# OFA-Sys/OFASys

Measured on AMD Instinct MI355X. Metric: multimodal tokens/sec (enc+dec train step), higher is better.
Workload: dtype bf16

## Files before the change

include/ofasys_amd.h:

```cpp
#ifndef OFASYS_AMD_H
#define OFASYS_AMD_H

#include <stdint.h>

#ifdef __cplusplus
extern "C" {
#endif

typedef enum { OFA_F32 = 0, OFA_BF16 = 1, OFA_F16 = 2 } ofa_dtype;

enum {
  OFA_OK = 0,
  OFA_ERR_INVALID = 1,
  OFA_ERR_UNSUPPORTED = 2,
  OFA_ERR_LAUNCH = 3
};

enum {
  OFA_GEMM_BIAS_COL = 1,
  OFA_GEMM_BIAS_ROW = 2,
  OFA_GEMM_ACCUM = 4,
  OFA_GEMM_FORCE_SIMPLE = 8,
  OFA_GEMM_OUT_F32 = 16,
  OFA_GEMM_A_KPAD_ZERO = 32,
  OFA_GEMM_NO_LDS_DMA = 64,
  OFA_GEMM_DEFER_REDUCE = 128
};

int ofa_version(void);
const char* ofa_last_error(void);

int ofa_layernorm_fwd(const void* x, const void* gamma, const void* beta, void* y, float* mean, float* rstd,
                      int64_t rows, int cols, float eps, int dtype, void* stream);
int ofa_layernorm_bwd_ws_rows(void);
int ofa_layernorm_bwd(const void* dy, const void* x, const void* gamma, const float* mean, const float* rstd,
                      const void* dres, void* dx, void* dgamma, void* dbeta, float* ws, int64_t rows, int cols,
                      int accumulate, int dtype, void* stream);
int ofa_gelu_layernorm_fwd(const void* h, const void* gamma, const void* beta, void* y, float* mean, float* rstd,
                           int64_t rows, int cols, float eps, int dtype, void* stream);
int ofa_gelu_layernorm_bwd(const void* dy, const void* h, const void* gamma, const float* mean, const float* rstd,
                           void* dh, void* dgamma, void* dbeta, void* dbias, float* ws, int64_t rows, int cols,
                           int accumulate, int dtype, void* stream);

int64_t ofa_join_keep_bytes(int64_t rows, int cols, int dtype);
int ofa_join_fwd(const void* x, const void* residual, const void* gamma_a, const void* beta_a, const void* gamma_b,
                 const void* beta_b, void* y, void* z, float* stats, uint8_t* keep_bits, int64_t rows, int cols, float eps, float p,
                 uint64_t seed, uint64_t offset, const int64_t* offset_base, int dtype, void* stream);
int ofa_join_bwd_slots(int64_t rows, int cols, int dtype);
int ofa_join_bwd(const void* dy, const void* dz, const void* x, const void* y, const void* gamma_a, const void* gamma_b,
                 const float* stats, const uint8_t* keep_bits, void* dres, void* dx, float* ws, int64_t rows, int cols, float p,
                 uint64_t seed, uint64_t offset, const int64_t* offset_base, int want_dx_colsum, int dtype, void* stream);

int ofa_gemm(const void* A, const void* B, void* C, const void* bias, int M, int N, int K, int transA, int transB,
             int64_t lda, int64_t ldb, int64_t ldc, int batch, int64_t strideA, int64_t strideB, int64_t strideC,
             int batch_inner, int64_t strideA2, int64_t strideB2, int64_t strideC2,
             float alpha, int flags, int dtype, void* ws, int64_t ws_bytes, void* stream);

int ofa_gemm_colstat(const void* A, const void* B, void* C, const void* bias, int M, int N, int K, int transA, int transB,
                     int64_t lda, int64_t ldb, int64_t ldc, float alpha, int flags, int dtype, void* ws, int64_t ws_bytes,
                     double* partial, int max_groups, int* groups, void* stream);

typedef struct ofa_gemm_group_item {
  const void* a;
  const void* b;
  float* slabs;
  int64_t lda, ldb;
  int32_t m, n, k;
  int32_t splits;
  void* out;
  int64_t ldo;
  float out_alpha;
} ofa_gemm_group_item;
int ofa_gemm_group_plan(ofa_gemm_group_item* items, int n, int dtype);
int ofa_gemm_group_tn(const ofa_gemm_group_item* items, int n, int dtype, void* stream);

int ofa_scaled_softmax_fwd(const void* x, void* y, float scale, int b, int np, int sq, int sk, int dtype, void* stream);
int ofa_scaled_softmax_bwd(const void* dy, const void* y, void* dx, float scale, int b, int np, int sq, int sk,
                           int dtype, void* stream);
int ofa_scaled_masked_softmax_fwd(const void* x, const uint8_t* mask, void* y, float scale, int b, int np, int sq,
                                  int sk, int mask_b, int dtype, void* stream);
int ofa_scaled_masked_softmax_bwd(const void* dy, const void* y, void* dx, float scale, int b, int np, int sq, int sk,
                                  int dtype, void* stream);
int ofa_scaled_upper_triang_masked_softmax_fwd(const void* x, void* y, float scale, int attn_batches, int sq,
                                               int dtype, void* stream);
int ofa_scaled_upper_triang_masked_softmax_bwd(const void* dy, const void* y, void* dx, float scale, int attn_batches,
                                               int sq, int dtype, void* stream);
int ofa_get_batch_per_block(int sq, int sk, int b, int np);

int ofa_attn_softmax_fwd(const void* x, const void* bias, const uint8_t* kpm, void* p, float scale, int BA, int heads,
                         int T, int S, int causal, int dtype, void* stream);

typedef struct ofa_attn_call {
  const void *q, *k, *v, *dout;
  void* out;
  float *lse, *delta;
  void *dq, *dk, *dv;
  const void *bias, *bias_swz_row, *bias_swz_col;
  void* dbias;
  float* ws;
  const uint8_t* kpm;
  const void* c_attn;
  const int32_t* seg;
  float *cs_q, *cs_k, *cs_v, *cs_c;
  int64_t ldq, ldk, ldo, ws_bytes, cs_ldq, cs_ldk;
  int32_t B, heads, T, S, Tpad, Tb, Sb;
  int32_t causal, rows_q, rows_k;
  int32_t dtype, c_attn_dtype, dbias_dtype;
  float scale;
} ofa_attn_call;
int ofa_attn_fwd(const ofa_attn_call* c, void* stream);
int ofa_attn_bwd(const ofa_attn_call* c, void* stream);
int ofa_attn_bwd_prep(const void* dout, const void* out, float* delta, int B, int heads, int T, int Tpad, int64_t ldo,
                      int dtype, void* stream);
int ofa_attn_cs_slots(int B, int rows);
int ofa_attn_sbias_chunks(int B, int heads, int Tb, int Sb);
int ofa_c_attn_grad(const float* delta, const void* c_attn, void* dc, int B, int heads, int T, int64_t ld, int accumulate,
                    int c_attn_dtype, void* stream);
int ofa_attn_decode(const void* q, const void* k, const void* v, const void* bias, const uint8_t* kpm, const void* c_attn,
                    int c_attn_dtype, void* out, void* probs, int B, int heads, int head_dim, int S, int64_t ldk,
                    int64_t k_batch_stride, int64_t kpm_ld, float scale, int dtype, void* stream);
int ofa_mean_heads(const void* p, void* out, int B, int heads, int64_t n, int dtype, void* stream);
int ofa_transpose_heads(const void* x, void* xt, int B, int T, int C, int Tpad, int64_t ld, int dtype, void* stream);

int ofa_gather_rows(const void* src, const int64_t* index, void* out, int64_t n, int D, int64_t src_rows, int dtype,
                    void* stream);
int ofa_gather_rows_parts(const void* const* srcs, const int* lens, int nparts, const int64_t* index, void* out, int64_t n, int D,
                          int64_t batch, int dtype, void* stream);
int ofa_scatter_rows_part(const void* src, const int64_t* inverse, void* out, int64_t batch, int nk, int Ttot, int start, int D,
                          int64_t src_rows, int dtype, void* stream);
int ofa_embedding_fwd(const void* weight, const int64_t* ids, void* out, int64_t n, int D, int64_t V, uint8_t* is_pad, int64_t pad_id,
                      int dtype, void* stream);
int ofa_segment_rowsum(const void* dout, const int32_t* order, const int32_t* seg_off, const int32_t* seg_row, void* dweight, int nseg,
                       int D, int accumulate, int dtype, void* stream);
int ofa_embedding_bwd_slices(int64_t V, int D);
int ofa_embedding_bwd(const void* dout, const int64_t* ids, void* dweight, int64_t n, int D, int64_t V,
                      int64_t padding_idx, uint8_t* present_ws, float* slice_ws, int dtype, void* stream);
#define OFA_EMBEDDING_IDS_MAX 15360
int ofa_embedding_bwd_ids_ok(int64_t n, int D, int64_t V, int dtype);
int ofa_embedding_bwd_ids(const void* dout, const int64_t* ids, void* dweight, int64_t n, int D, int64_t V, int64_t padding_idx,
                          int slices, int dtype, void* stream);
int ofa_embedding_range_bwd(const void* dout, void* dweight, int batch, int64_t T, int D, int64_t V, int64_t r0, int dtype, void* stream);
enum { OFA_EDGE_POS_RANGE = 0, OFA_EDGE_TOKEN_BWD = 1, OFA_EDGE_COLSUM_FOLD = 2, OFA_EDGE_IM2COL = 3 };
int ofa_step_edges_old(int item);

int ofa_gelu_fwd(const void* x, void* y, int64_t n, int dtype, void* stream);
int ofa_gelu_bwd(const void* dy, const void* x, void* dx, int64_t n, int dtype, void* stream);
int ofa_dropout_add_fwd(const void* x, const void* residual, void* y, int64_t n, float p, uint64_t seed,
                        uint64_t offset, const int64_t* offset_base, int dtype, void* stream);
int ofa_dropout_bwd(const void* dy, void* dx, int64_t n, float p, uint64_t seed, uint64_t offset,
                    const int64_t* offset_base, int dtype, void* stream);
int ofa_add_rowvec_mask(const void* a, const void* b, const void* vec, const uint8_t* rowmask, void* y, int64_t rows,
                        int cols, int64_t b_period, int dtype, void* stream);
int ofa_batch_sum(const void* x, void* out, int batch, int64_t n, int accumulate, int dtype, void* stream);

int ofa_colsum_ws_floats(int cols);
int ofa_colsum(const void* x, void* out, float* ws, int64_t rows, int cols, int64_t ld, float alpha, int accumulate,
               int dtype, int out_dtype, void* stream);

int ofa_add_n(const void* const* inputs, int n, void* out, int64_t numel, int dtype, void* stream);
int ofa_mul(const void* a, const void* b, void* y, int64_t rows, int cols, int b_rowvec, int dtype, void* stream);
int ofa_scale_row_groups(const void* x, const float* scale, void* y, int64_t rows, int cols, int64_t group, int dtype,
                         void* stream);
int ofa_reduce_sum_f32(const float* x, float* out, int64_t n, void* stream);
int ofa_head_sum_f32(const float* x, float* out, int B, int heads, int T, int ld, void* stream);

typedef struct ofa_bias_slots {
  const void* values[8];
  const void* values2[8];
  int32_t start[8];
  int32_t n[8];
  int32_t inner[8];
  int32_t count;
} ofa_bias_slots;
int64_t ofa_bias_swz_elems(int heads, int Tb, int Sb);
int ofa_bias_build(const void* abs_bias, const ofa_bias_slots* slots, void* out, void* swz_row, void* swz_col, int heads, int Tb,
                   int Sb, int dtype, void* stream);
int ofa_bias_outer_grad(const void* dbias, void* d_frames, void* d_patches, int heads, int T, int start, int F, int P, int dtype,
                        void* stream);
int ofa_bias_block_add(void* bias, const void* values, int B, int A, int T, int start, int n, int dtype, void* stream);
int ofa_bias_block_grad(const void* dbias, void* dvalues, int B, int A, int T, int start, int n, int dtype, void* stream);
int ofa_bias_block_add_batch(void* bias, const void* values, int B, int A, int T, int start, int n, int dtype, void* stream);
int ofa_bias_block_slice(const void* dbias, void* dvalues, int B, int A, int T, int start, int n, int dtype, void* stream);

int ofa_im2col_patch(const void* img, void* col, int B, int C, int H, int W, int p, int Kpad, int lead, int dtype, void* stream);

int ofa_cross_entropy_fwd(const void* logits, const int64_t* target, float* lse, float* row_loss, int64_t rows,
                          int64_t V, int64_t ld, int64_t ignore_index, int dtype, void* stream);
int ofa_cross_entropy_fwd_grad_ok(int64_t V, int64_t ld, int dtype);
int ofa_cross_entropy_fwd_grad(const void* logits, const int64_t* target, const float* grad_scale, float* lse, float* row_loss,
                               void* dlogits, int64_t rows, int64_t V, int64_t ld, int64_t ignore_index, int dtype, void* stream);
int ofa_cross_entropy_bwd(const void* logits, const int64_t* target, const float* lse, const float* grad_scale,
                          void* dlogits, int64_t rows, int64_t V, int64_t ld, int64_t ignore_index, int dtype,
                          void* stream);

int ofa_ls_cross_entropy_fwd(const void* logits, const int64_t* target, float* lse, float* row_loss, float* row_nll,
                             float* row_cnt, int64_t rows, int64_t V, int64_t ld, int64_t ignore_index, float eps,
                             int64_t cstart, int64_t cend, const uint8_t* cmask, int dtype, void* stream);
int ofa_ls_cross_entropy_bwd(const void* logits, const int64_t* target, const float* lse, const float* row_cnt,
                             const float* row_w, const float* grad_scale, void* dlogits, int64_t rows, int64_t V, int64_t ld,
                             int64_t ignore_index, float eps, int64_t cstart, int64_t cend, const uint8_t* cmask, int dtype,
                             void* stream);
int ofa_scst_loss_fwd_grad(const void* logits, const int64_t* target, const float* reward, const int32_t* row_seq,
                           int64_t rows_per_seq, const float* grad_scale, float* lse, float* row_loss, void* dlogits, int64_t rows,
                           int64_t nseq, int64_t V, int64_t ld, int64_t ignore_index, int64_t cstart, int64_t cend, int dtype,
                           void* stream);
int ofa_probs_fwd(const void* logits, float* out, int64_t rows, int64_t V, int64_t ld, int log_probs, int dtype,
                  void* stream);
int ofa_probs_bwd(const float* dy, const float* y, void* dlogits, int64_t rows, int64_t V, int64_t ld, int log_probs,
                  int dtype, void* stream);

int ofa_sumsq_ws_floats(void);
int ofa_sumsq(const void* x, float* out , float* ws ,
              int64_t n, int dtype, void* stream);
int ofa_step_schedule(const float* gsq, const double* sample_size, double* step, const double* lr, float* sched,
                      float* gnorm, float clip_norm, double beta1, double beta2, void* stream);
int ofa_step_stats_add(double* stats, const float* loss, const int64_t* target, int64_t n, int64_t pad, void* stream);
int ofa_step_schedule_scaled(const float* gsq, const double* sample_size, double* step, const double* lr, float* sched,
                             float* gnorm, double* loss_scaler, float clip_norm, double beta1, double beta2, double scale_factor,
                             double scale_window, double tolerance, double threshold, double min_loss_scale, void* stream);
int ofa_adam_step(float* master, float* exp_avg, float* exp_avg_sq, const void* grad, void* model_param,
                  const float* coef, int64_t n, float lr, float beta1, float beta2, float eps, float weight_decay,
                  int step, int dtype, void* stream);
int ofa_ema_step(void* state, const void* p, void* shadow, int64_t n, const double* step, const float* sched, double decay,
                 int64_t start_update, int64_t update_freq, int dtype, int state_dtype, int max_blocks, void* stream);
int ofa_ema_segments_step(void* state, const void* segments, void* shadow, int64_t n, int64_t state_numel, int64_t max_len,
                          const double* step, const float* sched, double decay, int64_t start_update, int64_t update_freq,
                          int dtype, int state_dtype, int max_blocks, void* stream);

int ofa_conv_out_size(int in, int k, int stride, int pad);
int ofa_im2col(const void* x, void* col, int B, int H, int W, int C, int KH, int KW, int stride, int pad, int Kpad,
               int x_nchw, int dtype, void* stream);
int ofa_col2im(const void* dcol, void* dx, int B, int H, int W, int C, int KH, int KW, int stride, int pad, int Kpad,
               int dtype, void* stream);
int ofa_batchnorm_ws_floats(int C);
int ofa_batchnorm_fwd(const void* x, const void* gamma, const void* beta, const void* residual, void* y, float* mean,
                      float* rstd, float* running_mean, float* running_var, float* ws, int64_t rows, int C, float eps,
                      float momentum, int use_running, int relu, int dtype, void* stream);
int ofa_batchnorm_bwd(const void* dy, const void* y, const void* x, const void* gamma, const float* mean, const float* rstd,
                      void* dx, void* dres, void* dgamma, void* dbeta, float* ws, int64_t rows, int C, int batch_stats,
                      int relu, int accumulate, const void* beta, int dtype, void* stream);
int ofa_batchnorm_fwd_stats(const void* x, double* sums, float* ws, int64_t rows, int C, int dtype, void* stream);
int ofa_batchnorm_fwd_apply(const void* x, const void* gamma, const void* beta, const void* residual, void* y, float* mean,
                            float* rstd, float* running_mean, float* running_var, const double* sums, int groups, int64_t rows,
                            int C, float eps, float momentum, int relu, int dtype, void* stream);
int ofa_batchnorm_bwd_stats(const void* dy, const void* y, const void* x, const void* gamma, const float* mean, const float* rstd,
                            float* sums, void* dgamma, void* dbeta, float* ws, int64_t rows, int C, int relu, int accumulate,
                            const void* beta, int dtype, void* stream);
int ofa_batchnorm_bwd_dx(const void* dy, const void* y, const void* x, const void* gamma, const float* mean, const float* rstd,
                         const float* sums, void* dx, void* dres, int64_t rows, const double* total_rows, int C, int relu,
                         const void* beta, int dtype, void* stream);
int ofa_maxpool_fwd(const void* x, void* y, uint8_t* arg, int B, int H, int W, int C, int K, int stride, int pad, int dtype,
                    void* stream);
int ofa_maxpool_bwd(const void* dy, const uint8_t* arg, void* dx, int B, int H, int W, int C, int K, int stride, int pad,
                    int dtype, void* stream);
int ofa_relu(const void* x, const void* gate, void* y, int64_t n, int dtype, void* stream);

typedef struct ofa_fold_job {
  const float* part;
  void* out;
  int64_t cols;
  int64_t stride;
  int32_t nslots;
  int32_t accumulate;
  float alpha;
  int32_t out_dtype;
} ofa_fold_job;
#define OFA_FOLD_LANES16 4
int ofa_fold_batched(const ofa_fold_job* jobs, int njobs, void* stream);
typedef struct ofa_copy_job {
  const void* src;
  void* dst;
  int64_t bytes;
} ofa_copy_job;
int ofa_copy_batched(const ofa_copy_job* jobs, int njobs, void* stream);
#define OFA_DEFER_FOLD 2
int ofa_layernorm_bwd_slots(int64_t rows, int cols, int dtype, int gelu);
int ofa_colsum_slots(int64_t rows);
int ofa_gemm_splits(int M, int N, int K, int transA, int transB, int batch, int flags, int dtype, int64_t ws_bytes);
enum {
  OFA_GEMM_PLAN_KERNEL = 0,
  OFA_GEMM_PLAN_SIMPLE_WHY,
  OFA_GEMM_PLAN_WAVES_M,
  OFA_GEMM_PLAN_WAVES_N,
  OFA_GEMM_PLAN_WAVE_TM,
  OFA_GEMM_PLAN_WAVE_TN,
  OFA_GEMM_PLAN_TILE_M,
  OFA_GEMM_PLAN_TILE_N,
  OFA_GEMM_PLAN_SPLITS,
  OFA_GEMM_PLAN_KSPLIT,
  OFA_GEMM_PLAN_K,
  OFA_GEMM_PLAN_MIXED_TALL,
  OFA_GEMM_PLAN_MIXED_SHORT,
  OFA_GEMM_PLAN_COLSTAT_ROWS,
  OFA_GEMM_PLAN_REDUCE,
  OFA_GEMM_PLAN_LEN
};
enum {
  OFA_GEMM_KERNEL_SIMPLE = 0,
  OFA_GEMM_KERNEL_REG = 1,
  OFA_GEMM_KERNEL_LDS_DMA = 2,
  OFA_GEMM_KERNEL_RING = 3,
  OFA_GEMM_KERNEL_BIG = 4,
  OFA_GEMM_KERNEL_PP = 5,
  OFA_GEMM_KERNEL_MIXED = 6
};
int ofa_gemm_plan(int M, int N, int K, int transA, int transB, int batch, int flags, int dtype, int64_t ws_bytes, int* plan);

typedef struct ofa_gen_policy {
  float temperature;
  int32_t cstart, cend;
  int32_t step, min_len, max_len;
  int32_t pad, unk, eos;
  float unk_penalty;
  int32_t ngram;
  const int64_t* tokens;
  int64_t tok_ld;
  const int32_t* done;
} ofa_gen_policy;

typedef struct ofa_gen_state {
  int64_t* tokens;
  int64_t tok_ld;
  int32_t tok_cap;
  float* scores;
  int64_t score_ld;
  int32_t *ignore, *done, *nfin;
  int64_t* reorder;
// ... 55 lines not shown
```

ofasys_amd/csrc/elementwise.hip:

```cpp
#include "common.h"

namespace ofa {

template <typename T> __device__ __forceinline__ float round_to(float v);
template <> __device__ __forceinline__ float round_to<float>(float v) { return v; }
template <> __device__ __forceinline__ float round_to<bf16_t>(float v) { return bf2f(f2bf(v)); }
template <> __device__ __forceinline__ float round_to<f16_t>(float v) { return (float)(f16_t)v; }

template <typename T, bool BWD>
__global__ __launch_bounds__(256) void gelu_kernel(const T* __restrict__ dy, const T* __restrict__ x, T* __restrict__ y,
                                                   int64_t nvec, int64_t n) {
  constexpr int N = Vec<T>::N;
  for (int64_t v = (int64_t)blockIdx.x * 256 + threadIdx.x; v < nvec; v += (int64_t)gridDim.x * 256) {
    float a[N], g[N], o[N];
    load_vec<T>(x + v * N, a);
    if (BWD) load_vec<T>(dy + v * N, g);
#pragma unroll
    for (int j = 0; j < N; ++j) o[j] = BWD ? g[j] * gelu_grad_f(a[j]) : gelu_f(a[j]);
    store_vec<T>(y + v * N, o);
  }
  if (blockIdx.x == 0) {
    for (int64_t e = nvec * N + threadIdx.x; e < n; e += 256) {
      const float a = ld1<T>(x + e);
      st1<T>(y + e, BWD ? ld1<T>(dy + e) * gelu_grad_f(a) : gelu_f(a));
// ... 728 lines not shown
  return check_launch("segment_rowsum");
}

extern "C" int ofa_embedding_bwd(const void* dout, const int64_t* ids, void* dweight, int64_t n, int D, int64_t V,
                                 int64_t padding_idx, uint8_t* present_ws, float* slice_ws, int dtype, void* stream) {
  OFA_DT_CHECK("embedding_bwd");
  OFA_REQUIRE(n >= 0 && D > 0 && V > 0 && dout && ids && dweight, OFA_ERR_INVALID, "embedding_bwd: bad argument");
  const int vecn = dt_vecn(dtype);
  OFA_REQUIRE(D <= 2048, OFA_ERR_UNSUPPORTED, "embedding_bwd: D=%d exceeds 2048", D);
  const bool vec_ok = D % vecn == 0 && D <= 64 * vecn * 4 && (((uintptr_t)dout | (uintptr_t)dweight) & 15) == 0;
  if (n == 0) return 0;
  hipStream_t st = (hipStream_t)stream;
  if (present_ws) {
    (void)hipMemsetAsync(present_ws, 0, (size_t)V, st);
    hipLaunchKernelGGL(embedding_mark_kernel, dim3(grid_for(n)), dim3(256), 0, st, ids, present_ws, n, V);
  }
  const int S = slice_ws ? ofa_embedding_bwd_slices(V, D) : 1;
  const int nv = cdiv(D, 64 * vecn);
  dim3 grid((unsigned)((V + 3) / 4), S), block(256);
#define EMB_LAUNCH(T, NV)                                                                                               \
  hipLaunchKernelGGL((embedding_bwd_kernel<T, NV>), grid, block, 0, st, (const T*)dout, ids, (T*)dweight, slice_ws, n, D, V, \
                     padding_idx, (const uint8_t*)present_ws, S)
  if (!vec_ok)
    dispatch_dtype(dtype, [&](auto tag) {
      using T = typename decltype(tag)::type;
      hipLaunchKernelGGL((embedding_bwd_scalar_kernel<T>), grid, block, 0, st, (const T*)dout, ids, (T*)dweight, slice_ws, n, D, V,
                         padding_idx, (const uint8_t*)present_ws, S);
    });
  else
    dispatch_dtype(dtype, [&](auto tag) {
      using T = typename decltype(tag)::type;
      if (nv <= 1) EMB_LAUNCH(T, 1);
      else if (nv <= 2) EMB_LAUNCH(T, 2);
      else EMB_LAUNCH(T, 4);
    });
#undef EMB_LAUNCH
  int rc = check_launch("embedding_bwd");
  if (rc || S == 1) return rc;
  dispatch_dtype(dtype, [&](auto tag) {
    using T = typename decltype(tag)::type;
    hipLaunchKernelGGL((embedding_fold_kernel<T>), dim3((unsigned)V), dim3(256), 0, st, slice_ws, (T*)dweight, D, V, padding_idx,
                       (const uint8_t*)present_ws, S);
  });
  return check_launch("embedding_fold");
}

extern "C" int ofa_step_edges_old(int item) {
#ifdef OFA_DEBUG_SWITCHES
  if (const char* e = getenv("OFA_STEP_EDGES_OLD")) return (atoi(e) >> item) & 1;
#endif
  return 0;
}

extern "C" int ofa_embedding_bwd_ids_ok(int64_t n, int D, int64_t V, int dtype) {
  const int vecn = dt_vecn(dtype);
  return OFA_DT_OK(dtype) && n >= 0 && n <= OFA_EMBEDDING_IDS_MAX && V > 0 && V < ((int64_t)1 << 31) && D > 0 && D % vecn == 0 &&
         D <= 64 * vecn * 4;
}

extern "C" int ofa_embedding_bwd_ids(const void* dout, const int64_t* ids, void* dweight, int64_t n, int D, int64_t V,
                                     int64_t padding_idx, int slices, int dtype, void* stream) {
  OFA_DT_CHECK("embedding_bwd_ids");
  OFA_REQUIRE(n >= 0 && D > 0 && V > 0 && slices >= 1 && dout && ids && dweight, OFA_ERR_INVALID, "embedding_bwd_ids: bad argument");
  OFA_REQUIRE(ofa_embedding_bwd_ids_ok(n, D, V, dtype), OFA_ERR_UNSUPPORTED,
              "embedding_bwd_ids: n=%lld ids (at most %d), D=%d (whole 16-byte vectors, at most 256 of them): use ofa_embedding_bwd",
              (long long)n, OFA_EMBEDDING_IDS_MAX, D);
  OFA_REQUIRE((((uintptr_t)dout | (uintptr_t)dweight) & 15) == 0, OFA_ERR_UNSUPPORTED, "embedding_bwd_ids: buffers not 16-byte aligned");
  if (n == 0) return 0;
  hipStream_t st = (hipStream_t)stream;
  const int vecn = dt_vecn(dtype);
  const int nv = cdiv(D, 64 * vecn);
  const int per = (int)(((n + slices - 1) / slices + 63) / 64 * 64);
  const int blocks = cdiv(n, EMB_IDS_WAVES) < 1024 ? cdiv(n, EMB_IDS_WAVES) : 1024;
  const size_t lds = (size_t)((n + 63) / 64 * 64 + EMB_IDS_WAVES * 64) * sizeof(int);
#define EMB_LAUNCH(T, NV, SL)                                                                                       \
  hipLaunchKernelGGL((embedding_bwd_ids_kernel<T, NV, SL>), dim3(blocks), dim3(EMB_IDS_WAVES * 64), lds, st, (const T*)dout, ids, \
                     (T*)dweight, (int)n, D, V, padding_idx, per)
  if (slices > 1)
    dispatch_dtype(dtype, [&](auto tag) {
      using T = typename decltype(tag)::type;
      if (nv <= 1) EMB_LAUNCH(T, 1, true);
      else if (nv <= 2) EMB_LAUNCH(T, 2, true);
      else EMB_LAUNCH(T, 4, true);
    });
  else
    dispatch_dtype(dtype, [&](auto tag) {
      using T = typename decltype(tag)::type;
      if (nv <= 1) EMB_LAUNCH(T, 1, false);
      else if (nv <= 2) EMB_LAUNCH(T, 2, false);
      else EMB_LAUNCH(T, 4, false);
    });
#undef EMB_LAUNCH
  return check_launch("embedding_bwd_ids");
}

extern "C" int ofa_embedding_range_bwd(const void* dout, void* dweight, int batch, int64_t T, int D, int64_t V, int64_t r0, int dtype,
                                       void* stream) {
  OFA_DT_CHECK("embedding_range_bwd");
  OFA_REQUIRE(dout && dweight && batch >= 1 && T >= 0 && D > 0 && V > 0 && r0 >= 0 && r0 + T <= V, OFA_ERR_INVALID,
              "embedding_range_bwd: bad argument (rows %lld .. %lld of %lld)", (long long)r0, (long long)(r0 + T), (long long)V);
  OFA_REQUIRE(D % dt_vecn(dtype) == 0 && (((uintptr_t)dout | (uintptr_t)dweight) & 15) == 0, OFA_ERR_UNSUPPORTED,
              "embedding_range_bwd: D=%d / buffers not whole 16-byte vectors: use ofa_embedding_bwd", D);
  if (T == 0) return 0;
  hipStream_t st = (hipStream_t)stream;
  const int64_t n = T * D;
  dispatch_dtype(dtype, [&](auto tag) {
// ... 235 lines not shown
```

ofasys_amd/csrc/fold.hip:

```cpp
#include "common.h"

namespace ofa {

constexpr int FOLD_MAX_JOBS = 56;

struct FoldJobs {
  const float* part[FOLD_MAX_JOBS];
  void* out[FOLD_MAX_JOBS];
  int64_t cols[FOLD_MAX_JOBS];
  int64_t stride[FOLD_MAX_JOBS];
  float alpha[FOLD_MAX_JOBS];
  int nslots[FOLD_MAX_JOBS];
  unsigned block0[FOLD_MAX_JOBS + 1];
  unsigned char flags[FOLD_MAX_JOBS];
  int njobs;
};

__device__ __forceinline__ void fold_store(const FoldJobs& J, int j, int64_t c, int64_t cols, const float (&t)[4]) {
  const float alpha = J.alpha[j];
  const bool acc = J.flags[j] & 1, f32 = J.flags[j] & 2, f16 = J.flags[j] & 8;
  if (c + 4 <= cols && (cols & 3) == 0) {
    if (f32) {
      float4* o = reinterpret_cast<float4*>((float*)J.out[j] + c);
      float4 v = make_float4(t[0] * alpha, t[1] * alpha, t[2] * alpha, t[3] * alpha);
// ... 126 lines not shown
      for (; s + 24 < ns; s += 32) {
        const float4 v0 = *reinterpret_cast<const float4*>(r + (int64_t)s * stride);
        const float4 v1 = *reinterpret_cast<const float4*>(r + (int64_t)(s + 8) * stride);
        const float4 v2 = *reinterpret_cast<const float4*>(r + (int64_t)(s + 16) * stride);
        const float4 v3 = *reinterpret_cast<const float4*>(r + (int64_t)(s + 24) * stride);
        a.x = (((a.x + v0.x) + v1.x) + v2.x) + v3.x;
        a.y = (((a.y + v0.y) + v1.y) + v2.y) + v3.y;
        a.z = (((a.z + v0.z) + v1.z) + v2.z) + v3.z;
        a.w = (((a.w + v0.w) + v1.w) + v2.w) + v3.w;
      }
      for (; s < ns; s += 8) {
        const float4 v = *reinterpret_cast<const float4*>(r + (int64_t)s * stride);
        a.x += v.x; a.y += v.y; a.z += v.z; a.w += v.w;
      }
    } else {
      for (int s = sl; s < ns; s += 8) {
        const float* r = p + (int64_t)s * stride + c;
        a.x += r[0];
        if (c + 1 < cols) a.y += r[1];
        if (c + 2 < cols) a.z += r[2];
        if (c + 3 < cols) a.w += r[3];
      }
    }
  }
  red[sl][q] = a;
  if (l16) red[sl + 8][q] = a2;
  __syncthreads();
  if (sl == 0 && c < cols) {
    float t[4] = {0.f, 0.f, 0.f, 0.f};
#pragma unroll
    for (int r = 0; r < 8; ++r) {
      t[0] += red[r][q].x; t[1] += red[r][q].y; t[2] += red[r][q].z; t[3] += red[r][q].w;
    }
    if (l16) {
#pragma unroll
      for (int r = 8; r < 16; ++r) {
        t[0] += red[r][q].x; t[1] += red[r][q].y; t[2] += red[r][q].z; t[3] += red[r][q].w;
      }
    }
    fold_store(J, j, c, cols, t);
  }
}

constexpr int COPY_MAX_JOBS = 96;
constexpr int COPY_CHUNK = 32768;
struct CopyJobs {
  const unsigned char* src[COPY_MAX_JOBS];
  unsigned char* dst[COPY_MAX_JOBS];
  int64_t bytes[COPY_MAX_JOBS];
  unsigned block0[COPY_MAX_JOBS + 1];
  int njobs;
};

__global__ __launch_bounds__(256) void copy_batched_kernel(CopyJobs J) {
  int lo = 0, hi = J.njobs - 1;
  while (lo < hi) {
    const int mid = (lo + hi + 1) >> 1;
    if (J.block0[mid] <= blockIdx.x) lo = mid; else hi = mid - 1;
  }
  const int64_t off = (int64_t)(blockIdx.x - J.block0[lo]) * COPY_CHUNK;
  const int64_t left = J.bytes[lo] - off;
  const int n = (int)(left < COPY_CHUNK ? left : COPY_CHUNK);
  const unsigned char* s = J.src[lo] + off;
  unsigned char* d = J.dst[lo] + off;
  if ((((uintptr_t)s | (uintptr_t)d) & 15) == 0) {
    const int nv = n >> 4;
    for (int i = threadIdx.x; i < nv; i += 256) reinterpret_cast<uint4*>(d)[i] = reinterpret_cast<const uint4*>(s)[i];
    for (int i = (nv << 4) + threadIdx.x; i < n; i += 256) d[i] = s[i];
  } else {
    for (int i = threadIdx.x; i < n; i += 256) d[i] = s[i];
  }
}

}
using namespace ofa;

extern "C" int ofa_copy_batched(const ofa_copy_job* jobs, int njobs, void* stream) {
  OFA_REQUIRE(njobs >= 0 && (njobs == 0 || jobs), OFA_ERR_INVALID, "copy_batched: bad argument");
  hipStream_t st = (hipStream_t)stream;
  for (int base = 0; base < njobs; base += COPY_MAX_JOBS) {
    CopyJobs J;
    const int n = njobs - base < COPY_MAX_JOBS ? njobs - base : COPY_MAX_JOBS;
    int m = 0;
    unsigned blocks = 0;
    for (int i = 0; i < n; ++i) {
      const ofa_copy_job& b = jobs[base + i];
      OFA_REQUIRE(b.bytes >= 0 && (b.bytes == 0 || (b.src && b.dst)), OFA_ERR_INVALID, "copy_batched: bad job %d", base + i);
      if (b.bytes == 0) continue;
      J.src[m] = (const unsigned char*)b.src; J.dst[m] = (unsigned char*)b.dst; J.bytes[m] = b.bytes;
      J.block0[m] = blocks;
      blocks += (unsigned)((b.bytes + COPY_CHUNK - 1) / COPY_CHUNK);
      ++m;
    }
    if (m == 0) continue;
    J.block0[m] = blocks;
    J.njobs = m;
    hipLaunchKernelGGL(copy_batched_kernel, dim3(blocks), dim3(256), 0, st, J);
    int rc = check_launch("copy_batched");
    if (rc) return rc;
  }
  return 0;
}

extern "C" int ofa_fold_batched(const ofa_fold_job* jobs, int njobs, void* stream) {
  OFA_REQUIRE(njobs >= 0 && (njobs == 0 || jobs), OFA_ERR_INVALID, "fold_batched: bad argument");
  hipStream_t st = (hipStream_t)stream;
  for (int base = 0; base < njobs; base += FOLD_MAX_JOBS) {
    FoldJobs J;
    const int n = njobs - base < FOLD_MAX_JOBS ? njobs - base : FOLD_MAX_JOBS;
    J.njobs = n;
    unsigned blocks = 0;
    for (int i = 0; i < n; ++i) {
      const ofa_fold_job& b = jobs[base + i];
      OFA_REQUIRE(b.part && b.out && b.cols > 0 && b.nslots > 0 && b.stride >= b.cols, OFA_ERR_INVALID, "fold_batched: bad job %d", base + i);
      OFA_REQUIRE(OFA_DT_OK(b.out_dtype), OFA_ERR_INVALID, "fold_batched: bad out dtype %d", b.out_dtype);
      J.part[i] = b.part; J.out[i] = b.out; J.cols[i] = b.cols; J.stride[i] = b.stride; J.alpha[i] = b.alpha;
      J.nslots[i] = b.nslots;
      const bool wide = b.nslots <= 16;
      J.flags[i] = (unsigned char)(((b.accumulate & ~OFA_FOLD_LANES16) ? 1 : 0) | (b.out_dtype == OFA_F32 ? 2 : 0) | (wide ? 4 : 0) |
                                   (b.out_dtype == OFA_F16 ? 8 : 0) | ((b.accumulate & OFA_FOLD_LANES16) ? 16 : 0));
      J.block0[i] = blocks;
      blocks += (unsigned)(wide ? (b.cols + 1023) / 1024 : (b.cols + 127) / 128);
    }
    J.block0[n] = blocks;
    if (blocks == 0) continue;
    hipLaunchKernelGGL(fold_batched_kernel, dim3(blocks), dim3(256), 0, st, J);
    int rc = check_launch("fold_batched");
    if (rc) return rc;
  }
  return 0;
}
```

ofasys_amd/csrc/gemm_core.h:

```cpp
#pragma once
#include <stdlib.h>

#include <type_traits>

#include "gemm.h"

namespace ofa {

typedef __attribute__((ext_vector_type(8))) short bf16x8;
template <bool F16> __device__ __forceinline__ float lo16(uint32_t w) {
  if constexpr (F16) return (float)__builtin_bit_cast(f16x2_t, w)[0];
  else return __uint_as_float(w << 16);
}
template <bool F16> __device__ __forceinline__ float hi16(uint32_t w) {
  if constexpr (F16) return (float)__builtin_bit_cast(f16x2_t, w)[1];
  else return __uint_as_float(w & 0xffff0000u);
}
template <bool F16> __device__ __forceinline__ uint32_t enc2(float lo, float hi) {
  if constexpr (F16) return pack_f16x2(lo, hi);
  else return pack_bf16x2(lo, hi);
}
template <bool F16> __device__ __forceinline__ float dec1(uint16_t u) {
  if constexpr (F16) return (float)__builtin_bit_cast(f16_t, u);
  else return bf2f(u);
// ... 405 lines not shown
      for (int j = 0; j < 8; ++j) {
        ps[j] = (double)cs[j];
        ps[g.N + j] = (double)cq[j];
      }
    }
  }
}

template <int I, int N, typename F> __device__ __forceinline__ void static_for(F&& f) {
  if constexpr (I < N) {
    f(std::integral_constant<int, I>{});
    static_for<I + 1, N>(f);
  }
}

template <int R, bool KMAJ> struct BigAddr {
  uint32_t a[4];
  __device__ __forceinline__ void init(uint32_t op0, int rbase, int lane) {
    if (KMAJ) {
      const int row = rbase + (lane & 31), hi = lane >> 5;
#pragma unroll
      for (int kk = 0; kk < 4; ++kk) a[kk] = op0 + (uint32_t)(row * 64 + swz<R, true>(row, kk * 2 + hi) * 8) * 2u;
    } else {
      const int g = lane >> 4, q = lane & 15;
      const int k = (g >> 1) * 8 + (q >> 2);
#pragma unroll
      for (int ti = 0; ti < 4; ++ti) {
        const int col = rbase + ti * 32 + (g & 1) * 16 + 4 * (q & 3);
        a[ti] = op0 + (uint32_t)(k * R + swz<R, false>(k, col >> 3) * 8 + (col & 7)) * 2u;
      }
    }
  }
};

template <int R, bool KMAJ, int KK, int TI, int BUFOFF>
__device__ __forceinline__ void big_frag(u64x2& d, const BigAddr<R, KMAJ>& fa) {
  if constexpr (KMAJ) {
    asm volatile("ds_read_b128 %0, %1 offset:%2" : "=v"(d) : "v"(fa.a[KK]), "i"(BUFOFF + TI * 32 * 128));
  } else {
    unsigned long long lo, hi;
    asm volatile("ds_read_b64_tr_b16 %0, %1 offset:%2" : "=v"(lo) : "v"(fa.a[TI]), "i"(BUFOFF + KK * 16 * R * 2));
    asm volatile("ds_read_b64_tr_b16 %0, %1 offset:%2" : "=v"(hi) : "v"(fa.a[TI]), "i"(BUFOFF + KK * 16 * R * 2 + 4 * R * 2));
    d[0] = lo;
    d[1] = hi;
  }
}

__host__ __device__ constexpr int big_read_after(int t, int nr) { return t < nr ? t : -1; }

constexpr int GROUP_MAX = 16;
struct GroupItem {
  const void* A; const void* B; float* ws;
  void* out; int64_t ldo; float alpha;
  int64_t lda, ldb;
  int M, N, K, krows, ksplit, splits, tiles_m, tiles_n, first;
};
struct GroupArgs { GroupItem it[GROUP_MAX]; int n, total; };

__device__ __forceinline__ const GroupItem* group_enter(const GroupArgs& ga, GemmArgs& g, int& t, int& ks) {
  const int id = xcd_remap((int)blockIdx.x, ga.total);
  int p = 0;
  for (int q = 1; q < ga.n; ++q)
    if (id >= ga.it[q].first) p = q;
  const GroupItem& it = ga.it[p];
  g.A = it.A; g.B = it.B; g.C = it.out; g.bias = nullptr;
  g.M = it.M; g.N = it.N; g.K = it.K; g.transA = 1; g.transB = 0;
  g.lda = it.lda; g.ldb = it.ldb; g.ldc = it.ldo; g.strideA = g.strideB = g.strideC = 0;
  g.alpha = it.out ? it.alpha : 1.f; g.flags = it.out ? OFA_GEMM_ACCUM : 0; g.batch_inner = 1; g.strideA2 = g.strideB2 = g.strideC2 = 0; g.a_krows = g.b_krows = it.krows;
  g.colstat = nullptr; g.colstat_rows = 0;
  const int ntiles = it.tiles_m * it.tiles_n, local = id - it.first;
  ks = local / ntiles;
  t = local - ks * ntiles;
  return &it;
}

bool gemm_group_pp_launch(int variant, const GroupArgs& ga, bool f16, hipStream_t st);

}
```

ofasys_amd/csrc/gemm_mfma.hip:

```cpp
#include <mutex>
#include <utility>
#include <vector>

#include "gemm_core.h"

namespace ofa {


#ifdef OFA_GEMM_TIMELINE
#define OFA_TL(i) do { if (threadIdx.x == 0 && (i) < 24) tl[i] = __builtin_amdgcn_s_memtime(); } while (0)
#define OFA_TL_BEGIN                                                                                                           \
  unsigned long long* tl = (unsigned long long*)ws + 32 * (blockIdx.x + gridDim.x * (blockIdx.y + gridDim.y * blockIdx.z));   \
  int tlk = 8;                                                                                                                 \
  if (threadIdx.x == 0) {                                                                                                      \
    tl[5] = __builtin_amdgcn_s_getreg((31 << 11) | 4);                                                                         \
    tl[6] = __builtin_amdgcn_s_getreg((31 << 11) | 20);                                                                        \
    tl[7] = __builtin_amdgcn_s_memrealtime();                                                                                  \
  }                                                                                                                            \
  OFA_TL(0)
#define OFA_TL_STEP do { OFA_TL(tlk); ++tlk; } while (0)
#define OFA_TL_END                                                        \
  do {                                                                    \
    OFA_TL(3);                                                            \
    asm volatile("s_waitcnt vmcnt(0)" ::: "memory");                      \
// ... 990 lines not shown
  }
  if (len < 0) {
    len = group_plan_len(items, n);
    std::lock_guard<std::mutex> lk(mu);
    if (cache.size() < 512) cache.push_back({key, len});
  }
  for (int p = 0; p < n; ++p) {
    int sp = cdiv(items[p].k, len);
    sp = sp > 32 ? 32 : sp;
    const int ksplit = cdiv(cdiv(items[p].k, BK), sp) * BK;
    items[p].splits = cdiv(items[p].k, ksplit);
  }
}

static int group_plan_len(const ofa_gemm_group_item* items, int n) {
  int kmax = 0;
  for (int p = 0; p < n; ++p) kmax = items[p].k > kmax ? items[p].k : kmax;
  const int tiles = cdiv(kmax, BK);
  int len = tiles * BK;
  double best = group_time_us(items, n, len);
  for (int sp = 2; sp <= 32 && cdiv(tiles, sp) >= 4; ++sp) {
    const int l = cdiv(tiles, sp) * BK;
    const double t = group_time_us(items, n, l);
    if (t < best * 0.97) { best = t; len = l; }
  }
  return len;
}

extern "C" int ofa_gemm_group_plan(ofa_gemm_group_item* items, int n, int dtype) {
  OFA_REQUIRE(dtype == OFA_BF16 || dtype == OFA_F16, OFA_ERR_INVALID, "gemm_group: 16-bit operands only (dtype %d)", dtype);
  OFA_REQUIRE(items && n >= 1 && n <= GROUP_MAX, OFA_ERR_INVALID, "gemm_group: 1..%d products per launch (got %d)", GROUP_MAX, n);
  for (int p = 0; p < n; ++p)
    OFA_REQUIRE(group_item_ok(items[p]), OFA_ERR_INVALID,
                "gemm_group: product %d (m=%d n=%d k=%d lda=%lld ldb=%lld) needs m, n, lda, ldb %% 8 == 0 and 16-byte aligned operands",
                p, items[p].m, items[p].n, items[p].k, (long long)items[p].lda, (long long)items[p].ldb);
  group_plan(items, n);
  return 0;
}

extern "C" int ofa_gemm_group_tn(const ofa_gemm_group_item* items, int n, int dtype, void* stream) {
  OFA_REQUIRE(dtype == OFA_BF16 || dtype == OFA_F16, OFA_ERR_INVALID, "gemm_group: 16-bit operands only (dtype %d)", dtype);
  OFA_REQUIRE(items && n >= 1 && n <= GROUP_MAX, OFA_ERR_INVALID, "gemm_group: 1..%d products per launch (got %d)", GROUP_MAX, n);
  GroupArgs ga;
  int first = 0;
  for (int p = 0; p < n; ++p) {
    const ofa_gemm_group_item& it = items[p];
    const bool direct = it.out != nullptr && it.splits == 1;
    OFA_REQUIRE(group_item_ok(it) && (direct || (it.slabs && !((uintptr_t)it.slabs & 15))), OFA_ERR_INVALID, "gemm_group: product %d is not eligible", p);
    OFA_REQUIRE(!direct || (!((uintptr_t)it.out & 15) && it.ldo >= it.n && !(it.ldo & 7)), OFA_ERR_INVALID,
                "gemm_group: product %d: out must be 16-byte aligned with a row stride that is a multiple of 8 elements", p);
    OFA_REQUIRE(it.splits >= 1 && it.splits <= 32, OFA_ERR_INVALID, "gemm_group: product %d: splits %d (run ofa_gemm_group_plan)", p, it.splits);
    GroupItem& d = ga.it[p];
    d.A = it.a; d.B = it.b; d.ws = it.slabs; d.lda = it.lda; d.ldb = it.ldb;
    d.out = direct ? it.out : nullptr; d.ldo = it.ldo; d.alpha = it.out_alpha;
    d.M = it.m; d.N = it.n; d.K = cdiv(it.k, BK) * BK; d.krows = it.k;
    d.ksplit = cdiv(cdiv(it.k, BK), it.splits) * BK;
    d.splits = it.splits;
    OFA_REQUIRE(cdiv(it.k, d.ksplit) == it.splits, OFA_ERR_INVALID, "gemm_group: product %d: %d slices leave an empty one", p, it.splits);
    d.tiles_m = cdiv(it.m, 256); d.tiles_n = cdiv(it.n, 256);
    d.first = first;
    first += d.tiles_m * d.tiles_n * d.splits;
  }
  for (int p = n; p < GROUP_MAX; ++p) ga.it[p] = ga.it[0];
  ga.n = n; ga.total = first;
  hipStream_t st = (hipStream_t)stream;
  if (const int v = pp_variant(plan_knobs(), true, false, 0)) {
    if (gemm_group_pp_launch(v, ga, dtype == OFA_F16, st)) return check_launch("gemm_group_tn_pp");
  }
  auto kern = dtype == OFA_F16 ? gemm_group_tn_kernel<true> : gemm_group_tn_kernel<false>;
  static uint64_t attr_done[2] = {0, 0};
  (void)gemm_lds_attr((const void*)kern, BIG_LDS, attr_done[dtype == OFA_F16]);
  hipLaunchKernelGGL(kern, dim3(ga.total), dim3(512), BIG_LDS, st, ga);
  return check_launch("gemm_group_tn");
}

extern "C" int ofa_gemm(const void* A, const void* B, void* C, const void* bias, int M, int N, int K, int transA,
                        int transB, int64_t lda, int64_t ldb, int64_t ldc, int batch, int64_t strideA, int64_t strideB,
                        int64_t strideC, int batch_inner, int64_t strideA2, int64_t strideB2, int64_t strideC2,
                        float alpha, int flags, int dtype, void* ws, int64_t ws_bytes, void* stream) {
  OFA_REQUIRE(OFA_DT_OK(dtype), OFA_ERR_INVALID, "gemm: bad dtype %d", dtype);
  OFA_REQUIRE(M >= 0 && N >= 0 && K >= 0 && batch >= 0, OFA_ERR_INVALID, "gemm: negative size");
  if (M == 0 || N == 0 || batch == 0) return 0;
  OFA_REQUIRE(A && B && C, OFA_ERR_INVALID, "gemm: null pointer");
  OFA_REQUIRE(!(flags & (OFA_GEMM_BIAS_COL | OFA_GEMM_BIAS_ROW)) || bias, OFA_ERR_INVALID, "gemm: bias flag without bias");
  OFA_REQUIRE(lda >= (transA ? M : K) && ldb >= (transB ? K : N) && ldc >= N, OFA_ERR_INVALID,
              "gemm: leading dimension too small (lda=%lld ldb=%lld ldc=%lld)", (long long)lda, (long long)ldb,
              (long long)ldc);
  OFA_REQUIRE(!(dtype == OFA_F32 && (flags & OFA_GEMM_OUT_F32)), OFA_ERR_INVALID, "gemm: OUT_F32 is for 16-bit inputs");
  if (batch_inner <= 0 || batch_inner >= batch) { batch_inner = batch; strideA2 = strideB2 = strideC2 = 0; }
  GemmArgs g{A, B, C, bias, M, N, K, transA, transB, lda, ldb, ldc, strideA, strideB, strideC, alpha, flags,
             batch_inner, strideA2, strideB2, strideC2};
  hipStream_t st = (hipStream_t)stream;
  if (dtype != OFA_F32 && !(flags & OFA_GEMM_FORCE_SIMPLE) && K > 0 && gemm_mfma_supported(g))
    return gemm_mfma_launch(g, batch, ws, ws_bytes, st, dtype == OFA_F16);
  return gemm_simple_launch(g, batch, dtype, st);
}

extern "C" int ofa_gemm_colstat(const void* A, const void* B, void* C, const void* bias, int M, int N, int K, int transA, int transB,
                                int64_t lda, int64_t ldb, int64_t ldc, float alpha, int flags, int dtype, void* ws, int64_t ws_bytes,
                                double* partial, int max_groups, int* groups, void* stream) {
  OFA_REQUIRE(groups, OFA_ERR_INVALID, "gemm_colstat: groups must not be NULL");
  *groups = 0;
  OFA_REQUIRE(OFA_DT_OK(dtype), OFA_ERR_INVALID, "gemm_colstat: bad dtype %d", dtype);
  OFA_REQUIRE(M > 0 && N > 0 && K > 0 && A && B && C, OFA_ERR_INVALID, "gemm_colstat: bad argument");
  OFA_REQUIRE(!(flags & (OFA_GEMM_BIAS_COL | OFA_GEMM_BIAS_ROW)) || bias, OFA_ERR_INVALID, "gemm_colstat: bias flag without bias");
  OFA_REQUIRE(lda >= (transA ? M : K) && ldb >= (transB ? K : N) && ldc >= N, OFA_ERR_INVALID, "gemm_colstat: leading dimension too small");
  GemmArgs g{A, B, C, bias, M, N, K, transA, transB, lda, ldb, ldc, 0, 0, 0, alpha, flags, 1, 0, 0, 0};
// ... 12 lines not shown
```

ofasys_amd/csrc/loss_optim.hip:

```cpp
#include "common.h"

namespace ofa {

__device__ __forceinline__ void online_merge(float& m, float& s, float m2, float s2) {
  const float mm = fmaxf(m, m2);
  if (mm == -INFINITY) { m = mm; s = 0.f; return; }
  s = s * expf(m - mm) + s2 * expf(m2 - mm);
  m = mm;
}

struct ExpLib {
  float c;
  __device__ __forceinline__ explicit ExpLib(float centre) : c(centre) {}
  __device__ __forceinline__ float operator()(float v) const { return expf(v - c); }
};
constexpr float L2E = 1.4426950408889634f;
__device__ __forceinline__ float ex2(float v) { return __builtin_amdgcn_exp2f(v); }
struct Exp2Fma {
  float k;
  __device__ __forceinline__ explicit Exp2Fma(float centre) : k(-centre * L2E) {}
  __device__ __forceinline__ float operator()(float v) const { return ex2(fmaf(v, L2E, k)); }
};
template <typename Exp, int N>
__device__ __forceinline__ void vec_merge(float& m, float& s, const float (&a)[N]) {
// ... 26 lines not shown

template <typename T>
__global__ __launch_bounds__(256) void ce_fwd_kernel(const T* __restrict__ logits, const int64_t* __restrict__ target,
                                                     float* __restrict__ lse, float* __restrict__ row_loss, int64_t V,
                                                     int64_t ld, int64_t ignore_index) {
  constexpr int N = Vec<T>::N;
  const int64_t row = blockIdx.x;
  const T* x = logits + row * ld;
  float m = -INFINITY, s = 0.f;
  const int64_t nvec = V / N;
  for (int64_t v = threadIdx.x; v < nvec; v += 256) {
    float a[N];
    load_vec<T>(x + v * N, a);
    vec_merge<ExpLib>(m, s, a);
  }
  for (int64_t e = nvec * N + threadIdx.x; e < V; e += 256) online_merge(m, s, ld1<T>(x + e), 1.f);
  block256_lse(m, s, [&](float l) {
    lse[row] = l;
    const int64_t t = target[row];
    row_loss[row] = (t == ignore_index) ? 0.f : l - ld1<T>(x + t);
  });
}

template <typename T>
__global__ __launch_bounds__(256) void ce_bwd_kernel(const T* __restrict__ logits, const int64_t* __restrict__ target,
                                                     const float* __restrict__ lse, const float* __restrict__ gscale,
                                                     T* __restrict__ dlogits, int64_t V, int64_t ld, int64_t ignore_index) {
  constexpr int N = Vec<T>::N;
  const int64_t row = blockIdx.x;
  const T* x = logits + row * ld;
  T* dx = dlogits + row * ld;
  const int64_t t = target[row];
  const bool ignored = t == ignore_index;
  const float g = gscale ? gscale[0] : 1.0f;
  const float l = lse[row];
  const int64_t nvec = ld / N;
  for (int64_t v = threadIdx.x; v < nvec; v += 256) {
    float a[N], o[N];
    load_vec<T>(x + v * N, a);
#pragma unroll
    for (int j = 0; j < N; ++j) {
      const int64_t c = v * N + j;
      float d = 0.f;
      if (!ignored && c < V) d = (expf(a[j] - l) - (c == t ? 1.f : 0.f)) * g;
      o[j] = d;
    }
    store_vec<T>(dx + v * N, o);
  }
}

template <typename T, int NV>
__global__ __launch_bounds__(1024) __attribute__((amdgpu_waves_per_eu(8))) void ce_fwd_grad_kernel(
    const T* __restrict__ logits, const int64_t* __restrict__ target, const float* __restrict__ gscale, float* __restrict__ lse,
    float* __restrict__ row_loss, T* __restrict__ dlogits, int V, int ld, int64_t ignore_index) {
  constexpr int N = Vec<T>::N;
  static_assert(N == 8, "16-bit element types");
  __shared__ float sm[16], ss[16];
  const int64_t row = blockIdx.x;
  const char* xb = reinterpret_cast<const char*>(logits + row * ld);
  char* db = reinterpret_cast<char*>(dlogits + row * ld);
  const int nvec = ld / N;
  const int tid = threadIdx.x;
  uint4 raw[NV];
#pragma unroll
  for (int i = 0; i < NV; ++i) {
    const int v = tid + i * 1024;
    raw[i] = v < nvec ? *reinterpret_cast<const uint4*>(xb + (uint32_t)v * 16u) : make_uint4(0, 0, 0, 0);
  }
  float m = -INFINITY, s = 0.f;
#pragma unroll
  for (int i = 0; i < NV; ++i) {
    const int c0 = (tid + i * 1024) * N;
    if (c0 >= V) continue;
    float a[N];
    unpack16<T>(raw[i], a);
    if (c0 + N <= V) {
      vec_merge<Exp2Fma>(m, s, a);
    } else {
#pragma unroll
      for (int j = 0; j < N; ++j)
        if (c0 + j < V) online_merge(m, s, a[j], 1.f);
    }
  }
  const float mw = wave_max(m);
  const float sw = wave_sum(mw == -INFINITY ? 0.f : s * ex2((m - mw) * L2E));
  const int wave = tid >> 6;
  if ((tid & 63) == 0) { sm[wave] = mw; ss[wave] = sw; }
  __syncthreads();
  float M = sm[0];
#pragma unroll
  for (int w = 1; w < 16; ++w) M = fmaxf(M, sm[w]);
  float S = 0.f;
#pragma unroll
  for (int w = 0; w < 16; ++w) S += ss[w] * ex2((sm[w] - M) * L2E);
  const float l = M + logf(S);
  const int64_t t64 = target[row];
  const bool ignored = t64 == ignore_index;
  const int t = (t64 >= 0 && t64 < V) ? (int)t64 : -1;
  const bool dead = ignored || t < 0;
  if (tid == 0) {
    lse[row] = l;
    row_loss[row] = ignored ? 0.f : t < 0 ? INFINITY : l - ld1<T>(reinterpret_cast<const T*>(xb) + t);
  }
  const float g = dead ? 0.f : (gscale ? gscale[0] : 1.0f);
  const Exp2Fma prob(l);
#pragma unroll
  for (int i = 0; i < NV; ++i) {
    const int v = tid + i * 1024;
    if (v >= nvec) continue;
    float a[N], o[N];
    unpack16<T>(raw[i], a);
    const int c0 = v * N;
#pragma unroll
    for (int j = 0; j < N; ++j) {
      float d = 0.f;
      if (!dead && c0 + j < V) d = (prob(a[j]) - (c0 + j == t ? 1.f : 0.f)) * g;
      o[j] = d;
    }
    uint4 w;
    w.x = pack2<T>(o[0], o[1]); w.y = pack2<T>(o[2], o[3]); w.z = pack2<T>(o[4], o[5]); w.w = pack2<T>(o[6], o[7]);
    *reinterpret_cast<uint4*>(db + (uint32_t)v * 16u) = w;
  }
}

struct LsCfg { float eps; int64_t cstart, cend; const uint8_t* cmask; };
__device__ __forceinline__ bool ls_allowed(const LsCfg& c, int64_t row, int64_t v, int64_t V) {
  bool ok = c.cstart < 0 || v < 4 || (v >= c.cstart && v < c.cend);
  if (ok && c.cmask) ok = c.cmask[row * V + v] != 0;
  return ok;
}

template <typename T>
__global__ __launch_bounds__(256) void lsce_fwd_kernel(const T* __restrict__ logits, const int64_t* __restrict__ target,
                                                       float* __restrict__ lse, float* __restrict__ row_loss,
                                                       float* __restrict__ row_nll, float* __restrict__ row_cnt, int64_t V,
                                                       int64_t ld, int64_t ignore_index, LsCfg cfg) {
  __shared__ float sx[4], sc[4];
  const int64_t row = blockIdx.x;
  const T* x = logits + row * ld;
  float m = -INFINITY, s = 0.f, sumx = 0.f, cnt = 0.f;
  for (int64_t v = threadIdx.x; v < V; v += 256) {
    if (!ls_allowed(cfg, row, v, V)) continue;
    const float a = ld1<T>(x + v);
    online_merge(m, s, a, 1.f);
    sumx += a;
    cnt += 1.f;
  }
  sumx = wave_sum(sumx);
  cnt = wave_sum(cnt);
  if ((threadIdx.x & 63) == 0) { sx[threadIdx.x >> 6] = sumx; sc[threadIdx.x >> 6] = cnt; }
  block256_lse(m, s, [&](float l) {
    const float X = sx[0] + sx[1] + sx[2] + sx[3], C = sc[0] + sc[1] + sc[2] + sc[3];
    lse[row] = l;
    row_cnt[row] = C;
    const int64_t t = target[row];
    if (t == ignore_index) {
      row_loss[row] = 0.f;
      row_nll[row] = 0.f;
    } else {
      const float nll = l - ld1<T>(x + t);
      const float smooth = C * l - X;
      const float eps_i = cfg.eps / (cfg.cstart < 0 && !cfg.cmask ? (C - 1.f) : (C - 1.f + 1e-6f));
      row_nll[row] = nll;
      row_loss[row] = (1.f - cfg.eps - eps_i) * nll + eps_i * smooth;
    }
  });
}

template <typename T>
__global__ __launch_bounds__(256) void lsce_bwd_kernel(const T* __restrict__ logits, const int64_t* __restrict__ target,
                                                       const float* __restrict__ lse, const float* __restrict__ row_cnt,
                                                       const float* __restrict__ row_w, const float* __restrict__ gscale,
                                                       T* __restrict__ dlogits, int64_t V, int64_t ld, int64_t ignore_index,
                                                       LsCfg cfg) {
// ... 410 lines not shown
        for (int j = 0; j < 4; ++j) e[j] = ema_one<S>(e[j], x[j], d, a);
        if constexpr (S32) {
          const f4v eo = {e[0], e[1], e[2], e[3]};
          __builtin_nontemporal_store(eo, reinterpret_cast<f4v*>(state + i));
        } else {
          u2v o;
          o.x = pack2<S>(e[0], e[1]);
          o.y = pack2<S>(e[2], e[3]);
          *reinterpret_cast<u2v*>(state + i) = o;
        }
        if (shadow) {
          if constexpr (T32) {
            const f4v so = {e[0], e[1], e[2], e[3]};
            *reinterpret_cast<f4v*>(shadow + i) = so;
          } else {
            u2v o;
            o.x = pack2<T>(e[0], e[1]);
            o.y = pack2<T>(e[2], e[3]);
            *reinterpret_cast<u2v*>(shadow + i) = o;
          }
        }
      }
    }
  }
  if (blockIdx.x == 0 && threadIdx.x < (n & 3)) {
    const int64_t i = (nq << 2) + threadIdx.x;
    const float e = ema_one<S>(ld1<S>(state + i), ld1<T>(p + i), d, a);
    st1<S>(state + i, e);
    if (shadow) st1<T>(shadow + i, e);
  }
}

struct EmaSegment {
  const void* src;
  int64_t off, len;
};
template <typename T, typename S>
__global__ __launch_bounds__(256) void ema_segments_kernel(S* __restrict__ state, const EmaSegment* __restrict__ segs,
                                                           T* __restrict__ shadow, int64_t state_numel,
                                                           const double* __restrict__ step, const float* __restrict__ sched,
                                                           EmaRule rule) {
  float d, a;
  if (!ema_decide(step, sched, rule, d, a)) return;
  const EmaSegment sg = segs[blockIdx.y];
  if (sg.off < 0 || sg.len < 0 || sg.off > state_numel - sg.len) return;
  const T* src = static_cast<const T*>(sg.src);
  for (int64_t i = (int64_t)blockIdx.x * 256 + threadIdx.x; i < sg.len; i += (int64_t)gridDim.x * 256) {
    const float e = ema_one<S>(ld1<S>(state + sg.off + i), ld1<T>(src + i), d, a);
    st1<S>(state + sg.off + i, e);
    if (shadow) st1<T>(shadow + sg.off + i, e);
  }
}

__global__ void step_schedule_kernel(const float* __restrict__ gsq, const double* __restrict__ sample_size,
                                     double* __restrict__ step, const double* __restrict__ lr, float* __restrict__ sched,
                                     float* __restrict__ gnorm, float clip_norm, double beta1, double beta2) {
  if (threadIdx.x || blockIdx.x) return;
  const double n = sample_size[0];
  const float inv_n = n > 0.0 ? (float)(1.0 / n) : 0.f;
  const float gn = sqrtf(gsq[0]) * inv_n;
  gnorm[0] = n > 0.0 ? gn : __builtin_nanf("");
  if (!(n > 0.0) || !isfinite(gn)) {
    sched[0] = 0.f;
    sched[1] = 0.f;
    sched[2] = (float)lr[0];
    sched[3] = 1.f;
    sched[4] += 1.f;
    return;
  }
  sched[3] = 0.f;
  float coef = inv_n;
  if (clip_norm > 0.f) coef *= fminf(clip_norm / (gn + 1e-6f), 1.0f);
  const double t = step[0] + 1.0;
  step[0] = t;
  const double bc1 = 1.0 - pow(beta1, t), bc2 = 1.0 - pow(beta2, t);
  sched[0] = coef;
  sched[1] = (float)(lr[0] * sqrt(bc2) / bc1);
  sched[2] = (float)lr[0];
  gnorm[0] = gn;
}

__global__ void step_schedule_scaled_kernel(const float* __restrict__ gsq, const double* __restrict__ sample_size,
                                            double* __restrict__ step, const double* __restrict__ lr, float* __restrict__ sched,
                                            float* __restrict__ gnorm, double* __restrict__ ls, float clip_norm, double beta1,
                                            double beta2, double scale_factor, double scale_window, double tolerance,
                                            double threshold, double min_loss_scale) {
  if (threadIdx.x || blockIdx.x) return;
  const double n = sample_size[0];
  const double scale = ls[0];
  double mf = n > 0.0 ? 1.0 / (scale * n) : 0.0;
  const float gn = (float)(mf * sqrt((double)gsq[0]));
  gnorm[0] = n > 0.0 ? gn : __builtin_nanf("");
  if (!(n > 0.0)) {
    sched[0] = 0.f;
    sched[1] = 0.f;
    sched[2] = (float)lr[0];
    sched[3] = 1.f;
    sched[4] += 1.f;
    return;
  }
  if (!isfinite(gn)) {
    const double it = ls[1];
    const double since = it - ls[3];
    ls[2] = it;
    ls[4] += 1.0;
    const double pct = ls[4] / since;
    if (since <= 0.0 || pct >= tolerance) {
      double dec = scale / scale_factor;
      if (threshold > 0.0 && dec < threshold) dec = threshold;
      ls[0] = dec;
      ls[3] = it;
      ls[4] = 0.0;
    }
    if (ls[0] <= min_loss_scale) {
      ls[0] = scale;
      ls[5] = 1.0;
    } else {
      ls[1] = it + 1.0;
    }
    sched[0] = 0.f;
    sched[1] = 0.f;
    sched[2] = (float)lr[0];
    sched[3] = 1.f;
    sched[4] += 1.f;
    return;
  }
  sched[3] = 0.f;
  if (clip_norm > 0.f && gn > clip_norm) mf *= (double)clip_norm / (double)gn;
  const double t = step[0] + 1.0;
  step[0] = t;
  const double bc1 = 1.0 - pow(beta1, t), bc2 = 1.0 - pow(beta2, t);
  sched[0] = (float)mf;
  sched[1] = (float)(lr[0] * sqrt(bc2) / bc1);
  sched[2] = (float)lr[0];
  const double it = ls[1];
  if (fmod(it - ls[2], scale_window) == 0.0) {
    ls[0] = scale * scale_factor;
    ls[3] = it;
  }
  ls[1] = it + 1.0;
}
}
using namespace ofa;

extern "C" int ofa_cross_entropy_fwd(const void* logits, const int64_t* target, float* lse, float* row_loss, int64_t rows,
                                     int64_t V, int64_t ld, int64_t ignore_index, int dtype, void* stream) {
  OFA_REQUIRE(OFA_DT_OK(dtype), OFA_ERR_INVALID, "cross_entropy_fwd: bad dtype %d", dtype);
  OFA_REQUIRE(rows >= 0 && V > 0 && ld >= V && logits && target && lse && row_loss, OFA_ERR_INVALID, "cross_entropy_fwd: bad argument");
  OFA_REQUIRE(ld % dt_vecn(dtype) == 0, OFA_ERR_INVALID, "cross_entropy_fwd: ld=%lld must be a multiple of the 16-byte vector width", (long long)ld);
  if (rows == 0) return 0;
  hipStream_t st = (hipStream_t)stream;
  dispatch_dtype(dtype, [&](auto tag) {
    using T = typename decltype(tag)::type;
    hipLaunchKernelGGL((ce_fwd_kernel<T>), dim3((unsigned)rows), dim3(256), 0, st, (const T*)logits, target, lse, row_loss, V, ld, ignore_index);
  });
  return check_launch("cross_entropy_fwd");
}

template <typename T>
static bool ce_fwd_grad_launch(const T* logits, const int64_t* target, const float* gs, float* lse, float* row_loss, T* dlogits,
                               int64_t rows, int64_t V, int64_t ld, int64_t ignore_index, hipStream_t st) {
  const int64_t per_thread = (ld / 8 + 1023) / 1024;
#define CE_FG(NV) hipLaunchKernelGGL((ce_fwd_grad_kernel<T, NV>), dim3((unsigned)rows), dim3(1024), 0, st, logits, target, gs, lse, row_loss, dlogits, (int)V, (int)ld, ignore_index)
  if (per_thread <= 1) CE_FG(1);
  else if (per_thread <= 2) CE_FG(2);
  else if (per_thread <= 4) CE_FG(4);
  else if (per_thread <= 7) CE_FG(7);
  else if (per_thread <= 8) CE_FG(8);
  else return false;
#undef CE_FG
  return true;
}

extern "C" int ofa_cross_entropy_fwd_grad_ok(int64_t V, int64_t ld, int dtype) {
  return (dtype == OFA_BF16 || dtype == OFA_F16) && V > 0 && ld >= V && ld % 8 == 0 && ld <= 8 * 1024 * 8;
}

extern "C" int ofa_cross_entropy_fwd_grad(const void* logits, const int64_t* target, const float* grad_scale, float* lse,
                                          float* row_loss, void* dlogits, int64_t rows, int64_t V, int64_t ld, int64_t ignore_index,
                                          int dtype, void* stream) {
  OFA_REQUIRE(ofa_cross_entropy_fwd_grad_ok(V, ld, dtype), OFA_ERR_UNSUPPORTED,
              "cross_entropy_fwd_grad: 16-bit logits of at most 65536 (padded) columns, ld a multiple of 8 (V=%lld ld=%lld dtype=%d)", (long long)V, (long long)ld, dtype);
  OFA_REQUIRE(rows >= 0 && logits && target && lse && row_loss && dlogits, OFA_ERR_INVALID, "cross_entropy_fwd_grad: bad argument");
  if (rows == 0) return 0;
  hipStream_t st = (hipStream_t)stream;
  const bool ok = dispatch_dtype16(dtype, [&](auto tag) {
    using T = typename decltype(tag)::type;
    return ce_fwd_grad_launch<T>((const T*)logits, target, grad_scale, lse, row_loss, (T*)dlogits, rows, V, ld, ignore_index, st);
  });
  OFA_REQUIRE(ok, OFA_ERR_UNSUPPORTED, "cross_entropy_fwd_grad: row too long");
  return check_launch("cross_entropy_fwd_grad");
}

extern "C" int ofa_cross_entropy_bwd(const void* logits, const int64_t* target, const float* lse, const float* grad_scale,
                                     void* dlogits, int64_t rows, int64_t V, int64_t ld, int64_t ignore_index, int dtype,
                                     void* stream) {
  OFA_REQUIRE(OFA_DT_OK(dtype), OFA_ERR_INVALID, "cross_entropy_bwd: bad dtype %d", dtype);
  OFA_REQUIRE(rows >= 0 && V > 0 && ld >= V && logits && target && lse && dlogits, OFA_ERR_INVALID, "cross_entropy_bwd: bad argument");
  OFA_REQUIRE(ld % dt_vecn(dtype) == 0, OFA_ERR_INVALID, "cross_entropy_bwd: ld must be a multiple of the 16-byte vector width");
  if (rows == 0) return 0;
  hipStream_t st = (hipStream_t)stream;
  dispatch_dtype(dtype, [&](auto tag) {
    using T = typename decltype(tag)::type;
    hipLaunchKernelGGL((ce_bwd_kernel<T>), dim3((unsigned)rows), dim3(256), 0, st, (const T*)logits, target, lse, grad_scale, (T*)dlogits, V, ld, ignore_index);
  });
  return check_launch("cross_entropy_bwd");
}

extern "C" int ofa_ls_cross_entropy_fwd(const void* logits, const int64_t* target, float* lse, float* row_loss, float* row_nll,
                                        float* row_cnt, int64_t rows, int64_t V, int64_t ld, int64_t ignore_index, float eps,
                                        int64_t cstart, int64_t cend, const uint8_t* cmask, int dtype, void* stream) {
  OFA_REQUIRE(OFA_DT_OK(dtype), OFA_ERR_INVALID, "ls_cross_entropy_fwd: bad dtype %d", dtype);
  OFA_REQUIRE(rows >= 0 && V > 1 && ld >= V && logits && target && lse && row_loss && row_nll && row_cnt, OFA_ERR_INVALID,
              "ls_cross_entropy_fwd: bad argument");
  OFA_REQUIRE(eps >= 0.f && eps < 1.f && (cstart < 0 || (cstart >= 4 && cend > cstart && cend <= V)), OFA_ERR_INVALID,
              "ls_cross_entropy_fwd: bad eps / constraint range [%lld, %lld)", (long long)cstart, (long long)cend);
  if (rows == 0) return 0;
  hipStream_t st = (hipStream_t)stream;
  const LsCfg cfg{eps, cstart, cend, cmask};
  dispatch_dtype(dtype, [&](auto tag) {
    using T = typename decltype(tag)::type;
    hipLaunchKernelGGL((lsce_fwd_kernel<T>), dim3((unsigned)rows), dim3(256), 0, st, (const T*)logits, target, lse, row_loss, row_nll, row_cnt, V, ld, ignore_index, cfg);
  });
  return check_launch("ls_cross_entropy_fwd");
}

extern "C" int ofa_ls_cross_entropy_bwd(const void* logits, const int64_t* target, const float* lse, const float* row_cnt,
                                        const float* row_w, const float* grad_scale, void* dlogits, int64_t rows, int64_t V,
                                        int64_t ld, int64_t ignore_index, float eps, int64_t cstart, int64_t cend,
                                        const uint8_t* cmask, int dtype, void* stream) {
  OFA_REQUIRE(OFA_DT_OK(dtype), OFA_ERR_INVALID, "ls_cross_entropy_bwd: bad dtype %d", dtype);
  OFA_REQUIRE(rows >= 0 && V > 1 && ld >= V && logits && target && lse && row_cnt && dlogits, OFA_ERR_INVALID,
              "ls_cross_entropy_bwd: bad argument");
  if (rows == 0) return 0;
  hipStream_t st = (hipStream_t)stream;
  const LsCfg cfg{eps, cstart, cend, cmask};
  dispatch_dtype(dtype, [&](auto tag) {
    using T = typename decltype(tag)::type;
    hipLaunchKernelGGL((lsce_bwd_kernel<T>), dim3((unsigned)rows), dim3(256), 0, st, (const T*)logits, target, lse, row_cnt, row_w, grad_scale, (T*)dlogits, V, ld, ignore_index, cfg);
  });
  return check_launch("ls_cross_entropy_bwd");
}

template <typename T>
// ... 31 lines not shown
  hipStream_t st = (hipStream_t)stream;
  dispatch_dtype(dtype, [&](auto tag) {
    using T = typename decltype(tag)::type;
    scst_launch<T>((const T*)logits, target, reward, row_seq, row_seq ? 1 : rows_per_seq, grad_scale, lse, row_loss, (T*)dlogits, rows, nseq,
                   V, ld, ignore_index, cstart < 0 ? 0 : cstart, cstart < 0 ? V : cend, st);
  });
  return check_launch("scst_loss_fwd_grad");
}

extern "C" int ofa_probs_fwd(const void* logits, float* out, int64_t rows, int64_t V, int64_t ld, int log_probs, int dtype,
                             void* stream) {
  OFA_REQUIRE(OFA_DT_OK(dtype), OFA_ERR_INVALID, "probs_fwd: bad dtype %d", dtype);
  OFA_REQUIRE(rows >= 0 && V > 0 && ld >= V && logits && out, OFA_ERR_INVALID, "probs_fwd: bad argument");
  if (rows == 0) return 0;
  hipStream_t st = (hipStream_t)stream;
  dispatch_dtype(dtype, [&](auto tag) {
    using T = typename decltype(tag)::type;
    hipLaunchKernelGGL((probs_fwd_kernel<T>), dim3((unsigned)rows), dim3(256), 0, st, (const T*)logits, out, V, ld, log_probs);
  });
  return check_launch("probs_fwd");
}

extern "C" int ofa_probs_bwd(const float* dy, const float* y, void* dlogits, int64_t rows, int64_t V, int64_t ld,
                             int log_probs, int dtype, void* stream) {
  OFA_REQUIRE(OFA_DT_OK(dtype), OFA_ERR_INVALID, "probs_bwd: bad dtype %d", dtype);
  OFA_REQUIRE(rows >= 0 && V > 0 && ld >= V && dy && y && dlogits, OFA_ERR_INVALID, "probs_bwd: bad argument");
  if (rows == 0) return 0;
  hipStream_t st = (hipStream_t)stream;
  dispatch_dtype(dtype, [&](auto tag) {
    using T = typename decltype(tag)::type;
    hipLaunchKernelGGL((probs_bwd_kernel<T>), dim3((unsigned)rows), dim3(256), 0, st, dy, y, (T*)dlogits, V, ld, log_probs);
  });
  return check_launch("probs_bwd");
}

extern "C" int ofa_sumsq_ws_floats(void) { return 1024; }

extern "C" int ofa_sumsq(const void* x, float* out, float* ws, int64_t n, int dtype, void* stream) {
  OFA_REQUIRE(OFA_DT_OK(dtype), OFA_ERR_INVALID, "sumsq: bad dtype %d", dtype);
  OFA_REQUIRE(n >= 0 && out && ws && (n == 0 || x), OFA_ERR_INVALID, "sumsq: bad argument");
  if (n == 0) return 0;
  hipStream_t st = (hipStream_t)stream;
  const int vecw = dt_vecn(dtype);
  int64_t nbl = (n / vecw + 255) / 256;
  const int nb = (int)(nbl < 1 ? 1 : (nbl > 1024 ? 1024 : nbl));
  dispatch_dtype(dtype, [&](auto tag) {
    using T = typename decltype(tag)::type;
    hipLaunchKernelGGL((sumsq_kernel<T>), dim3(nb), dim3(256), 0, st, (const T*)x, ws, n);
  });
  int rc = check_launch("sumsq");
  if (rc) return rc;
  hipLaunchKernelGGL(sumsq_final_kernel, dim3(1), dim3(256), 0, st, (const float*)ws, out, nb);
  return check_launch("sumsq_final");
}

extern "C" int ofa_adam_step(float* master, float* exp_avg, float* exp_avg_sq, const void* grad, void* model_param,
                             const float* coef, int64_t n, float lr, float beta1, float beta2, float eps,
                             float weight_decay, int step, int dtype, void* stream) {
  OFA_REQUIRE(OFA_DT_OK(dtype), OFA_ERR_INVALID, "adam_step: bad dtype %d", dtype);
  OFA_REQUIRE(n >= 0 && step >= 0 && master && exp_avg && exp_avg_sq && grad && model_param, OFA_ERR_INVALID, "adam_step: bad argument");
  OFA_REQUIRE(step >= 1 || coef, OFA_ERR_INVALID, "adam_step: step == 0 takes the step size and lr from coef[1], coef[2]");
  if (n == 0) return 0;
  const int dev_sched = step == 0;
  const double bc1 = 1.0 - pow((double)beta1, step), bc2 = 1.0 - pow((double)beta2, step);
  const float step_size = dev_sched ? 0.f : (float)(lr * sqrt(bc2) / bc1);
  hipStream_t st = (hipStream_t)stream;
  OFA_REQUIRE(!(((uintptr_t)master | (uintptr_t)exp_avg | (uintptr_t)exp_avg_sq) & 15) && !(((uintptr_t)grad | (uintptr_t)model_param) & 7),
              OFA_ERR_INVALID, "adam_step: arenas must be 16-byte (fp32 state) / 8-byte (grad, model copy) aligned");
  int64_t nbl = (n + 255) / 256;
  const int nb = (int)(nbl > 65536 ? 65536 : nbl);
  dispatch_dtype(dtype, [&](auto tag) {
    using T = typename decltype(tag)::type;
    hipLaunchKernelGGL((adam_kernel<T>), dim3(nb), dim3(256), 0, st, master, exp_avg, exp_avg_sq, (const T*)grad, (T*)model_param, coef, n, lr, beta1, beta2, eps, weight_decay, step_size, dev_sched);
  });
  return check_launch("adam_step");
}

static int ema_rule(const char* who, const void* state, const void* p, const double* step, const float* sched, double decay,
                    int64_t start_update, int64_t update_freq, int dtype, int state_dtype, int max_blocks, EmaRule* rule) {
  OFA_REQUIRE(OFA_DT_OK(dtype), OFA_ERR_INVALID, "%s: bad dtype %d", who, dtype);
  OFA_REQUIRE(state_dtype == OFA_F32 || state_dtype == dtype, OFA_ERR_INVALID,
              "%s: the state is fp32 or of the model dtype (dtype %d, state dtype %d)", who, dtype, state_dtype);
  OFA_REQUIRE(state && p && step && sched && max_blocks >= 0, OFA_ERR_INVALID, "%s: bad argument", who);
  OFA_REQUIRE(decay >= 0.0 && decay <= 1.0 && start_update >= 0 && update_freq >= 1, OFA_ERR_INVALID,
              "%s: decay in [0, 1], start_update >= 0, update_freq >= 1 (got %g, %lld, %lld)", who, decay, (long long)start_update,
              (long long)update_freq);
  float a = (float)(1.0 - decay);
  if (state_dtype == OFA_F16) a = (float)(_Float16)a;
  if (state_dtype == OFA_BF16) {
    uint32_t u;
    memcpy(&u, &a, 4);
    u = (u + 0x7fffu + ((u >> 16) & 1u)) & 0xffff0000u;
    memcpy(&a, &u, 4);
  }
  *rule = EmaRule{(float)decay, a, (double)start_update, update_freq};
  return 0;
}

extern "C" int ofa_ema_step(void* state, const void* p, void* shadow, int64_t n, const double* step, const float* sched,
                            double decay, int64_t start_update, int64_t update_freq, int dtype, int state_dtype, int max_blocks,
                            void* stream) {
  EmaRule rule;
  if (int rc = ema_rule("ema_step", state, p, step, sched, decay, start_update, update_freq, dtype, state_dtype, max_blocks, &rule)) return rc;
  OFA_REQUIRE(n >= 0, OFA_ERR_INVALID, "ema_step: bad argument");
  if (n == 0) return 0;
  const uintptr_t sa = state_dtype == OFA_F32 ? 15 : 7, ta = dtype == OFA_F32 ? 15 : 7;
// ... 78 lines not shown
```

ofasys_amd/kernels.py:

```python
import contextlib
import ctypes

import torch

from .lib import (BF16, F32, GEMM_ACCUM, GEMM_BIAS_COL, GEMM_BIAS_ROW, GEMM_FORCE_SIMPLE, GEMM_OUT_F32, OfaError,
                  dptr, dtype_code, lib, ptr, stream)

_ws_cache = {}


def workspace(nbytes, device, tag="ws"):
    key = (tag, device, torch.cuda.current_stream().cuda_stream if device.type == "cuda" else 0)
    buf = _ws_cache.get(key)
    n = (nbytes + 3) // 4
    if buf is None or buf.numel() < n:
        buf = torch.empty(max(n, 1 << 20), dtype=torch.float32, device=device)
        _ws_cache[key] = buf
    return buf


@contextlib.contextmanager
def capture_workspaces(cache):
    global _ws_cache
    saved, _ws_cache = _ws_cache, dict(cache)
    added = {}
    try:
        yield added
    finally:
        added.update({k: v for k, v in _ws_cache.items() if cache.get(k) is not v})
        cache.update(added)
        _ws_cache = saved


class _FoldJob(ctypes.Structure):
    _fields_ = [("part", ctypes.c_void_p), ("out", ctypes.c_void_p), ("cols", ctypes.c_int64), ("stride", ctypes.c_int64),
                ("nslots", ctypes.c_int32), ("accumulate", ctypes.c_int32), ("alpha", ctypes.c_float),
                ("out_dtype", ctypes.c_int32)]


class _CopyJob(ctypes.Structure):
    _fields_ = [("src", ctypes.c_void_p), ("dst", ctypes.c_void_p), ("bytes", ctypes.c_int64)]


def copy_batched(pairs):
    jobs = []
    for dst, src in pairs:
        if (src.dtype == dst.dtype and src.shape == dst.shape and src.device == dst.device and dst.is_cuda
                and src.is_contiguous() and dst.is_contiguous()):
            jobs.append((dptr(src), dptr(dst), src.numel() * src.element_size()))
        else:
            dst.copy_(src, non_blocking=True)
    if jobs:
        arr = (_CopyJob * len(jobs))()
        for it, (s_, d_, n) in zip(arr, jobs):
            it.src, it.dst, it.bytes = s_, d_, n
        lib().call("ofa_copy_batched", ctypes.addressof(arr), len(jobs), stream())


DEFER_FOLD = 2
FOLD_LANES16 = 4
GEMM_DEFER_REDUCE = 128


class FoldQueue:

    MAX_PENDING_BYTES = 48 << 20

    def __init__(self):
        self.jobs, self.keep, self.bytes, self.outs, self.want_flush = [], [], 0, set(), False

    def add(self, part, part_off, out, cols, stride, nslots, alpha=1.0, accumulate=True, flush_ok=True, lanes16=False):
        assert part.dtype == torch.float32 and out.is_contiguous()
        if out.data_ptr() in self.outs:
            self.flush()
        self.outs.add(out.data_ptr())
        self.jobs.append(_FoldJob(dptr(part) + part_off * 4, dptr(out), cols, stride, nslots,
                                  int(bool(accumulate)) | (FOLD_LANES16 if lanes16 else 0), float(alpha), dtype_code(out)))
        self.keep.append((part, out))
        self.bytes += nslots * stride * 4
        self.want_flush = self.bytes > self.MAX_PENDING_BYTES

    def flush_if_large(self):
        if getattr(self, "want_flush", False):
            self.flush()

    def flush(self):
        if not self.jobs:
            return
        arr = (_FoldJob * len(self.jobs))(*self.jobs)
        lib().call("ofa_fold_batched", ctypes.addressof(arr), len(self.jobs), stream())
        self.jobs, self.keep, self.bytes, self.want_flush = [], [], 0, False
        self.outs = set()


class ImmediateFold:

    def add(self, part, part_off, out, cols, stride, nslots, alpha=1.0, accumulate=True, flush_ok=True, lanes16=False):
        assert part.dtype == torch.float32 and out.is_contiguous()
        job = (_FoldJob * 1)(_FoldJob(dptr(part) + part_off * 4, dptr(out), cols, stride, nslots,
                                      int(bool(accumulate)) | (FOLD_LANES16 if lanes16 else 0), float(alpha), dtype_code(out)))
        lib().call("ofa_fold_batched", ctypes.addressof(job), 1, stream())

    def flush_if_large(self):
        pass


def _u8(mask):
    mask = mask.contiguous()
    return mask.view(torch.uint8) if mask.dtype == torch.bool else mask.to(torch.uint8)


def _rows_cols(x):
    cols = x.shape[-1]
    return x.numel() // cols, cols


def layernorm_fwd(x, gamma, beta, eps=1e-5, fuse_gelu=False):
    x = x.contiguous()
    rows, cols = _rows_cols(x)
    y = torch.empty_like(x)
    mean = torch.empty(rows, dtype=torch.float32, device=x.device)
    rstd = torch.empty(rows, dtype=torch.float32, device=x.device)
    lib().call("ofa_gelu_layernorm_fwd" if fuse_gelu else "ofa_layernorm_fwd", ptr(x), ptr(gamma), ptr(beta), ptr(y),
               ptr(mean), ptr(rstd), rows, cols, eps, dtype_code(x), stream())
    return y, mean, rstd


def layernorm_bwd(dy, x, gamma, mean, rstd, fuse_gelu=False, dgamma=None, dbeta=None, dbias=None, want_dbias=False,
                  fold=None, dres=None):
    dy = dy.contiguous()
    x = x.contiguous()
    rows, cols = _rows_cols(x)
    dx = torch.empty_like(x)
    acc = dgamma is not None
    if not acc:
        dgamma = torch.empty(cols, dtype=gamma.dtype, device=x.device)
        dbeta = torch.empty(cols, dtype=gamma.dtype, device=x.device)
        if want_dbias:
            dbias = torch.empty(cols, dtype=gamma.dtype, device=x.device)
    assert dgamma.dtype == x.dtype and dbeta.dtype == x.dtype and (dbias is None or dbias.dtype == x.dtype)
    wsr = lib().cdll.ofa_layernorm_bwd_ws_rows()
    if fold is not None and acc:
        ns = lib().cdll.ofa_layernorm_bwd_slots(rows, cols, dtype_code(x), int(fuse_gelu))
        nq = 3 if (fuse_gelu and dbias is not None) else 2
        ws = torch.empty(nq * ns * cols, dtype=torch.float32, device=x.device)
        for q, o in enumerate((dgamma, dbeta, dbias)[:nq]):
            fold.add(ws, q * ns * cols, o, cols, cols, ns)
        acc = DEFER_FOLD
    else:
        ws = workspace(wsr * cols * 4, x.device, "ln")
    if fuse_gelu:
        lib().call("ofa_gelu_layernorm_bwd", ptr(dy), ptr(x), ptr(gamma), ptr(mean), ptr(rstd), ptr(dx), ptr(dgamma),
                   ptr(dbeta), ptr(dbias), ptr(ws), rows, cols, int(acc), dtype_code(x), stream())
    else:
        if dres is not None:
            dres = dres.contiguous()
            assert dres.shape == x.shape and dres.dtype == x.dtype
        lib().call("ofa_layernorm_bwd", ptr(dy), ptr(x), ptr(gamma), ptr(mean), ptr(rstd), ptr(dres), ptr(dx), ptr(dgamma),
                   ptr(dbeta), ptr(ws), rows, cols, int(acc), dtype_code(x), stream())
    if acc == DEFER_FOLD:
        fold.flush_if_large()
    return dx, dgamma, dbeta, (dbias if fuse_gelu else None)


def gemm(a, b, trans_a=False, trans_b=False, bias=None, bias_row=False, alpha=1.0, out=None, accumulate=False,
         out_f32=False, force_simple=False, a_kpad_zero=False, fold=None):
    assert a.dim() == b.dim() and a.dim() in (2, 3)
    batched = a.dim() == 3
    if a.stride(-1) != 1:
        a = a.contiguous()
    if b.stride(-1) != 1:
        b = b.contiguous()
    batch = a.shape[0] if batched else 1
    ar, ac = a.shape[-2], a.shape[-1]
    br, bc = b.shape[-2], b.shape[-1]
    M, K = (ac, ar) if trans_a else (ar, ac)
    N, Kb = (br, bc) if trans_b else (bc, br)
    if K != Kb:
        raise OfaError(f"gemm: inner dimensions differ ({K} vs {Kb})")
    dt = dtype_code(a)
    if b.dtype != a.dtype:
        raise OfaError("gemm: operand dtypes differ")
    if out is None:
        odt = torch.float32 if (out_f32 or a.dtype == torch.float32) else a.dtype
        out = torch.empty((batch, M, N) if batched else (M, N), dtype=odt, device=a.device)
    flags = 0
    if bias is not None:
        flags |= GEMM_BIAS_ROW if bias_row else GEMM_BIAS_COL
    if accumulate:
        flags |= GEMM_ACCUM
    if force_simple:
        flags |= GEMM_FORCE_SIMPLE
    if dt != F32 and out.dtype == torch.float32:
        flags |= GEMM_OUT_F32
    if a_kpad_zero:
        flags |= 32
    lda, ldb, ldc = a.stride(-2), b.stride(-2), out.stride(-2)
    sa = a.stride(0) if batched else 0
    sb = b.stride(0) if batched else 0
    sc = out.stride(0) if batched else 0
    ws = None
    if fold is not None and bias is None and not batched and ldc == N and N % 4 == 0 and _prof is None:
        nsp = lib().cdll.ofa_gemm_splits(M, N, K, int(trans_a), int(trans_b), 1, flags, dt, 256 << 20)
        if nsp > 1:
            ws = torch.empty(nsp * M * N, dtype=torch.float32, device=a.device)
            fold.add(ws, 0, out, M * N, M * N, nsp, alpha, accumulate)
            flags |= GEMM_DEFER_REDUCE
            ws_bytes = 256 << 20
    if ws is None:
        ws = workspace(256 << 20, a.device, "gemm")
        ws_bytes = ws.numel() * 4
    args = ("ofa_gemm", ptr(a), ptr(b), ptr(out), ptr(bias), M, N, K, int(trans_a), int(trans_b), lda, ldb, ldc, batch,
            sa, sb, sc, 0, 0, 0, 0, float(alpha), flags, dt, ptr(ws), ws_bytes, stream())
    if _prof is not None:
        e0 = torch.cuda.Event(enable_timing=True)
        e1 = torch.cuda.Event(enable_timing=True)
        e0.record()
        lib().call(*args)
        e1.record()
        _prof.append((2.0 * M * N * K * batch, e0, e1, batch * ((M * K + K * N) * a.element_size() + M * N * out.element_size())))
    else:
        lib().call(*args)
    if flags & GEMM_DEFER_REDUCE:
        fold.flush_if_large()
    return out


def gemm_colstat(a, b, bias=None, max_groups=512):
    assert a.dim() == 2 and b.dim() == 2 and a.shape[1] == b.shape[1] and a.dtype == b.dtype
    if a.stride(-1) != 1:
        a = a.contiguous()
    if b.stride(-1) != 1:
        b = b.contiguous()
    M, Kd, N = a.shape[0], a.shape[1], b.shape[0]
    out = torch.empty(M, N, dtype=a.dtype, device=a.device)
    if a.dtype == torch.float32 or N % 8:
        return gemm(a, b, False, True, bias=bias, out=out), None
    flags = GEMM_BIAS_COL if bias is not None else 0
    ws = workspace(256 << 20, a.device, "gemm")
    cap = min(max_groups, (M + 31) // 32)
    partial = torch.empty(cap, 2, N, dtype=torch.float64, device=a.device)
    groups = ctypes.c_int(0)
    args = ("ofa_gemm_colstat", ptr(a), ptr(b), ptr(out), ptr(bias), M, N, Kd, 0, 1, a.stride(0), b.stride(0), out.stride(0), 1.0,
            flags, dtype_code(a), ptr(ws), ws.numel() * 4, ptr(partial), cap, ctypes.addressof(groups), stream())
    if _prof is not None:
        e0 = torch.cuda.Event(enable_timing=True)
        e1 = torch.cuda.Event(enable_timing=True)
        e0.record()
        lib().call(*args)
        e1.record()
        _prof.append((2.0 * M * N * Kd, e0, e1, (M * Kd + Kd * N + M * N) * a.element_size()))
    else:
        lib().call(*args)
    return out, (partial[:groups.value] if groups.value > 0 else None)


class _GroupItem(ctypes.Structure):
    _fields_ = [("a", ctypes.c_void_p), ("b", ctypes.c_void_p), ("slabs", ctypes.c_void_p), ("lda", ctypes.c_int64),
                ("ldb", ctypes.c_int64), ("m", ctypes.c_int32), ("n", ctypes.c_int32), ("k", ctypes.c_int32),
                ("splits", ctypes.c_int32), ("out", ctypes.c_void_p), ("ldo", ctypes.c_int64), ("out_alpha", ctypes.c_float)]


GROUP_MAX = 16
GROUP_DIRECT = True


def gemm_group_ok(dy, x, out):
    return (dy.dim() == 2 and x.dim() == 2 and dy.dtype in (torch.bfloat16, torch.float16) and x.dtype == dy.dtype
            and dy.stride(1) == 1 and x.stride(1) == 1 and dy.shape[0] == x.shape[0] and dy.shape[0] >= 1
            and dy.shape[1] % 8 == 0 and x.shape[1] % 8 == 0 and dy.stride(0) % 8 == 0 and x.stride(0) % 8 == 0
            and dy.data_ptr() % 16 == 0 and x.data_ptr() % 16 == 0 and out.is_contiguous())


def gemm_group_tn(products, fold):
    assert 1 <= len(products) <= GROUP_MAX
    arr = (_GroupItem * len(products))()
    for it, (dy, x, out, alpha) in zip(arr, products):
        it.a, it.b, it.lda, it.ldb = dptr(dy), dptr(x), dy.stride(0), x.stride(0)
        it.m, it.n, it.k = dy.shape[1], x.shape[1], dy.shape[0]
    dt = dtype_code(products[0][0])
    lib().call("ofa_gemm_group_plan", ctypes.addressof(arr), len(products), dt)
    slabs, direct_outs = [], set()
    for it, (dy, x, out, alpha) in zip(arr, products):
        direct = (GROUP_DIRECT and it.splits == 1 and out.dtype == dy.dtype and out.dim() == 2 and out.stride(1) == 1 and out.stride(0) % 8 == 0
                  and out.data_ptr() % 16 == 0 and out.data_ptr() not in direct_outs)
        if direct:
            direct_outs.add(out.data_ptr())
            it.out, it.ldo, it.out_alpha = dptr(out), out.stride(0), float(alpha)
            slabs.append(None)
        else:
            sl = torch.empty(it.splits * it.m * it.n, dtype=torch.float32, device=dy.device)
            it.slabs = dptr(sl)
            slabs.append(sl)
    if _prof is not None:
        e0 = torch.cuda.Event(enable_timing=True)
        e1 = torch.cuda.Event(enable_timing=True)
        e0.record()
        lib().call("ofa_gemm_group_tn", ctypes.addressof(arr), len(products), dt, stream())
        e1.record()
        es = products[0][0].element_size()
        _prof.append((sum(2.0 * it.m * it.n * it.k for it in arr), e0, e1,
                      sum((it.m + it.n) * it.k * es + (it.splits * it.m * it.n * 4 if sl is not None else 2 * it.m * it.n * es)
                          for it, sl in zip(arr, slabs))))
    else:
        lib().call("ofa_gemm_group_tn", ctypes.addressof(arr), len(products), dt, stream())
    for it, sl, (dy, x, out, alpha) in zip(arr, slabs, products):
        if sl is not None:
            fold.add(sl, 0, out, it.m * it.n, it.m * it.n, it.splits, alpha, True)


_prof = None
_PROF_REPS = 1


def gemm_profile_begin():
    global _prof
    _prof = []


def gemm_profile_end():
    global _prof
    torch.cuda.synchronize()
    rec, _prof = _prof, None
    return {"launches": len(rec), "flops": sum(r[0] for r in rec), "bytes": sum(r[3] for r in rec),
            "time_ms": sum(r[1].elapsed_time(r[2]) for r in rec) / _PROF_REPS, "reps": _PROF_REPS}


def gemm_heads(a, b, out, M, N, K, trans_a, trans_b, lda, ldb, ldc, B, heads, sa, sa2, sb, sb2, sc, sc2, alpha=1.0,
               accumulate=False):
    dt = dtype_code(a)
    flags = GEMM_ACCUM if accumulate else 0
    if dt != F32 and out.dtype == torch.float32:
        flags |= GEMM_OUT_F32
    ws = workspace(256 << 20, a.device, "gemm")
    lib().call("ofa_gemm", ptr(a), ptr(b), ptr(out), None, M, N, K, int(trans_a), int(trans_b), lda, ldb, ldc, B * heads,
               sa, sb, sc, heads, sa2, sb2, sc2, float(alpha), flags, dt, ptr(ws), ws.numel() * 4, stream())
    return out


def scaled_softmax(x, scale):
    x = x.contiguous()
# ... 55 lines not shown

def attn_softmax(x, bias, kpm, scale, heads, causal):
    x = x.contiguous()
    BA, T, S = x.shape
    if bias is not None:
        bias = bias.contiguous()
    if kpm is not None:
        kpm = _u8(kpm)
    p = torch.empty_like(x)
    lib().call("ofa_attn_softmax_fwd", ptr(x), ptr(bias), ptr(kpm), ptr(p), float(scale), BA, heads, T, S, int(causal),
               dtype_code(x), stream())
    return p


def pad32(n):
    return (n + 31) // 32 * 32


def transpose_heads(x, T_pad):
    B, T, C = x.shape
    if x.stride(-1) != 1 or x.stride(0) != T * x.stride(1):
        x = x.contiguous()
    xt = torch.empty(B, C, T_pad, dtype=x.dtype, device=x.device)
    lib().call("ofa_transpose_heads", ptr(x), ptr(xt), B, T, C, T_pad, x.stride(1), dtype_code(x), stream())
    return xt


def _rows3(x):
    if x.stride(-1) != 1 or x.stride(0) != x.shape[1] * x.stride(1):
        x = x.contiguous()
    return x, x.stride(1)


def _same_ld(k, v):
    k, ldk = _rows3(k)
    v, ldv = _rows3(v)
    if ldv != ldk:
        k, v = k.contiguous(), v.contiguous()
        ldk = k.stride(1)
    return k, v, ldk


def _c_dtype(c_attn):
    if c_attn is None:
        return dtype_code(torch.empty(0, dtype=torch.float32))
    assert c_attn.is_contiguous()
    return dtype_code(c_attn)


def c_attn_grad(delta, c_attn, B, heads, T, out=None, accumulate=False):
    if out is None:
        out = torch.empty_like(c_attn)
        accumulate = False
    lib().call("ofa_c_attn_grad", ptr(delta), ptr(c_attn), ptr(out), B, heads, T, delta.stride(0), int(accumulate),
               dtype_code(c_attn), stream())
    return out


def _shared_bias(bias, heads, q):
    assert bias.dim() == 3 and bias.shape[0] == heads, (tuple(bias.shape), heads)
    if bias.dtype != q.dtype:
        bias = bias.to(q.dtype)
    return bias.contiguous()


class _BiasSlots(ctypes.Structure):
    _fields_ = [("values", ctypes.c_void_p * 8), ("values2", ctypes.c_void_p * 8), ("start", ctypes.c_int32 * 8), ("n", ctypes.c_int32 * 8),
                ("inner", ctypes.c_int32 * 8), ("count", ctypes.c_int32)]


def bias_build(abs_bias, starts=(), values=(), heads=None, want_out=True):
    live = [(s, v) for s, v in zip(starts, values) if v is not None]
    ref = abs_bias if abs_bias is not None else (live[0][1][0] if isinstance(live[0][1], tuple) else live[0][1])
    slots = _BiasSlots()
    assert len(live) <= 8, "at most 8 slots per bias"
    keep, ends = [], []
    for i, (s, v) in enumerate(live):
        if isinstance(v, tuple):
            vf, vi = (t.to(ref.dtype).contiguous() for t in v)
            keep += [vf, vi]
            n = vf.shape[0] * vi.shape[0]
            slots.values[i], slots.values2[i], slots.inner[i] = dptr(vf), dptr(vi), vi.shape[0]
        else:
            v = v.to(ref.dtype).contiguous()
            keep.append(v)
            n = v.shape[0]
            slots.values[i], slots.values2[i], slots.inner[i] = dptr(v), None, 0
        slots.start[i], slots.n[i] = int(s), n
        ends.append(int(s) + n)
    slots.count = len(live)
    if abs_bias is not None:
        abs_bias = abs_bias.contiguous()
        A, Tb, Sb = abs_bias.shape
    else:
        A = heads
        Tb = Sb = max(ends)
    n = lib().cdll.ofa_bias_swz_elems(A, Tb, Sb)
    swz = torch.empty(2, n, dtype=ref.dtype, device=ref.device)
    out = torch.empty(A, Tb, Sb, dtype=ref.dtype, device=ref.device) if want_out else None
    lib().call("ofa_bias_build", ptr(abs_bias), ctypes.addressof(slots), ptr(out), ptr(swz[0]), ptr(swz[1]), A, Tb, Sb,
               dtype_code(ref), stream())
    return out, (swz[0], swz[1])


def _shared_swz(bias, bias_shared):
    if isinstance(bias_shared, tuple):
        return bias_shared
# ... 133 lines not shown
    y = torch.empty_like(x)
    lib().call("ofa_gelu_fwd", ptr(x), ptr(y), x.numel(), dtype_code(x), stream())
    return y


def gelu_bwd(dy, x):
    dy, x = dy.contiguous(), x.contiguous()
    dx = torch.empty_like(x)
    lib().call("ofa_gelu_bwd", ptr(dy), ptr(x), ptr(dx), x.numel(), dtype_code(x), stream())
    return dx


def dropout_add(x, residual, p, seed, offset, offset_base=None):
    x = x.contiguous()
    if residual is not None:
        residual = residual.contiguous()
    y = torch.empty_like(x)
    lib().call("ofa_dropout_add_fwd", ptr(x), ptr(residual), ptr(y), x.numel(), float(p), seed, offset, ptr(offset_base),
               dtype_code(x), stream())
    return y


def dropout_bwd(dy, p, seed, offset, offset_base=None):
    dy = dy.contiguous()
    dx = torch.empty_like(dy)
    lib().call("ofa_dropout_bwd", ptr(dy), ptr(dx), dy.numel(), float(p), seed, offset, ptr(offset_base), dtype_code(dy),
               stream())
    return dx


def add_rowvec_mask(a, b=None, vec=None, rowmask=None):
    a = a.contiguous()
    rows, cols = _rows_cols(a)
    period = 0
    if b is not None:
        b = b.contiguous()
        brows = b.numel() // cols
        if brows != rows:
            assert brows > 0 and rows % brows == 0, (rows, brows)
            period = brows
    if rowmask is not None:
        rowmask = _u8(rowmask)
    y = torch.empty_like(a)
    lib().call("ofa_add_rowvec_mask", ptr(a), ptr(b), ptr(vec), ptr(rowmask), ptr(y), rows, cols, period, dtype_code(a), stream())
    return y


def batch_sum(x, batch, out=None, accumulate=False):
    x = x.contiguous()
    n = x.numel() // batch
    if out is None:
        out = torch.empty(n, dtype=x.dtype, device=x.device)
        accumulate = False
    lib().call("ofa_batch_sum", ptr(x), ptr(out), int(batch), n, int(bool(accumulate)), dtype_code(x), stream())
    return out


def embedding_fwd(weight, ids, pad_mask_of=None):
    ids = ids.contiguous()
    V, D = weight.shape
    out = torch.empty(*ids.shape, D, dtype=weight.dtype, device=weight.device)
    mask = None
    if pad_mask_of is not None and D % (4 if weight.dtype == torch.float32 else 8) == 0:
        mask = torch.empty(ids.shape, dtype=torch.bool, device=weight.device)
    lib().call("ofa_embedding_fwd", ptr(weight), ptr(ids), ptr(out), ids.numel(), D, V, ptr(mask), int(pad_mask_of) if mask is not None else 0,
               dtype_code(weight), stream())
    if pad_mask_of is None:
        return out
    return out, (mask if mask is not None else ids.eq(pad_mask_of))


def gather_rows(src2d, index):
    assert src2d.dim() == 2 and src2d.is_contiguous() and index.dtype == torch.int64 and index.is_contiguous()
    out = torch.empty(index.numel(), src2d.shape[1], dtype=src2d.dtype, device=src2d.device)
    lib().call("ofa_gather_rows", ptr(src2d), ptr(index), ptr(out), index.numel(), src2d.shape[1], src2d.shape[0],
               dtype_code(src2d), stream())
    return out


def gather_rows_parts(parts, index):
    assert 1 <= len(parts) <= 8 and index.dtype == torch.int64 and index.is_contiguous()
    B, D = parts[0].shape[0], parts[0].shape[2]
    assert all(t.dim() == 3 and t.is_contiguous() and t.shape[0] == B and t.shape[2] == D and t.dtype == parts[0].dtype for t in parts)
    out = torch.empty(index.numel(), D, dtype=parts[0].dtype, device=parts[0].device)
    srcs = (ctypes.c_void_p * len(parts))(*[dptr(t) for t in parts])
    lens = (ctypes.c_int * len(parts))(*[int(t.shape[1]) for t in parts])
    lib().call("ofa_gather_rows_parts", ctypes.addressof(srcs), ctypes.addressof(lens), len(parts), ptr(index), ptr(out), index.numel(), D, B,
               dtype_code(parts[0]), stream())
    return out


def scatter_rows_part(dpacked, inverse, B, nk, Ttot, start):
    assert dpacked.dim() == 2 and dpacked.is_contiguous() and inverse.dtype == torch.int64 and inverse.is_contiguous()
    D = dpacked.shape[1]
    out = torch.empty(B, nk, D, dtype=dpacked.dtype, device=dpacked.device)
    lib().call("ofa_scatter_rows_part", ptr(dpacked), ptr(inverse), ptr(out), B, nk, Ttot, start, D, dpacked.shape[0], dtype_code(dpacked), stream())
    return out


EDGE_POS_RANGE, EDGE_TOKEN_BWD, EDGE_COLSUM_FOLD, EDGE_IM2COL = 0, 1, 2, 3


def edge_old(item):
    return bool(lib().cdll.ofa_step_edges_old(int(item)))


def embedding_bwd(dout, ids, V, padding_idx=-1, dweight=None, id_major=None):
    dout = dout.contiguous()
    ids = ids.contiguous()
    D = dout.shape[-1]
    if dweight is None:
        dweight = torch.zeros(V, D, dtype=dout.dtype, device=dout.device)
    S = lib().cdll.ofa_embedding_bwd_slices(V, D)
    pad = -1 if padding_idx is None else padding_idx
    if id_major is None:
        id_major = S == 1 and not edge_old(EDGE_TOKEN_BWD)
    if (id_major and lib().cdll.ofa_embedding_bwd_ids_ok(ids.numel(), D, V, dtype_code(dout))
            and (dout.data_ptr() | dweight.data_ptr()) % 16 == 0):
        lib().call("ofa_embedding_bwd_ids", ptr(dout), ptr(ids), ptr(dweight), ids.numel(), D, V, pad, S, dtype_code(dout), stream())
        return dweight
    present = workspace(V, dout.device, "embed_present") if V > 4096 else None
    slices = workspace(S * V * D * 4, dout.device, "embed_slices") if S > 1 else None
    lib().call("ofa_embedding_bwd", ptr(dout), ptr(ids), ptr(dweight), ids.numel(), D, V,
               pad, ptr(present), ptr(slices), dtype_code(dout), stream())
    return dweight


def embedding_range_ok(x):
    return x.shape[-1] % (4 if x.dtype == torch.float32 else 8) == 0 and not edge_old(EDGE_POS_RANGE)


def embedding_range_bwd(dout, dweight, r0, T):
    dout = dout.contiguous()
    V, D = dweight.shape
    batch = dout.numel() // (T * D)
    assert dweight.is_contiguous() and dweight.dtype == dout.dtype and batch * T * D == dout.numel()
    lib().call("ofa_embedding_range_bwd", ptr(dout), ptr(dweight), batch, T, D, V, int(r0), dtype_code(dout), stream())
    return dweight


def segment_rowsum(dout2d, plan, dweight, accumulate):
    assert dout2d.dim() == 2 and dout2d.is_contiguous() and dweight.is_contiguous() and dout2d.dtype == dweight.dtype
    lib().call("ofa_segment_rowsum", ptr(dout2d), ptr(plan.order), ptr(plan.seg_off), ptr(plan.seg_row), ptr(dweight), plan.nseg,
               dout2d.shape[1], int(accumulate), dtype_code(dout2d), stream())
    return dweight


def im2col_patch(img, p, Kpad, lead=0):
    img = img.contiguous()
    B, C, H, W = img.shape
    col = torch.empty(B * (lead + (H // p) * (W // p)), Kpad, dtype=img.dtype, device=img.device)
    lib().call("ofa_im2col_patch", ptr(img), ptr(col), B, C, H, W, p, Kpad, int(lead), dtype_code(img), stream())
    return col


def step_stats_add(stats, loss, target, pad):
    assert stats.dtype == torch.float64 and stats.numel() >= 3 and loss.dtype == torch.float32 and loss.numel() == 1
    t = target.reshape(-1)
    assert t.dtype == torch.int64 and t.is_contiguous()
    lib().call("ofa_step_stats_add", ptr(stats), ptr(loss), ptr(t), t.numel(), int(pad), stream())


def cross_entropy_fwd(logits2d, target, V, ignore_index):
    rows, ld = logits2d.shape[0], logits2d.stride(0)
    lse = torch.empty(rows, dtype=torch.float32, device=logits2d.device)
    row_loss = torch.empty(rows, dtype=torch.float32, device=logits2d.device)
    lib().call("ofa_cross_entropy_fwd", ptr(logits2d), ptr(target), ptr(lse), ptr(row_loss), rows, V, ld, ignore_index,
               dtype_code(logits2d), stream())
    return lse, row_loss


def cross_entropy_fwd_grad_ok(logits2d, V):
    return logits2d.is_cuda and bool(lib().cdll.ofa_cross_entropy_fwd_grad_ok(int(V), int(logits2d.stride(0)), dtype_code(logits2d)))


def cross_entropy_fwd_grad(logits2d, target, grad_scale, V, ignore_index):
    rows, ld = logits2d.shape[0], logits2d.stride(0)
    lse = torch.empty(rows, dtype=torch.float32, device=logits2d.device)
    row_loss = torch.empty(rows, dtype=torch.float32, device=logits2d.device)
    dlogits = torch.empty(rows, ld, dtype=logits2d.dtype, device=logits2d.device)
    lib().call("ofa_cross_entropy_fwd_grad", ptr(logits2d), ptr(target), ptr(grad_scale), ptr(lse), ptr(row_loss), ptr(dlogits), rows, V,
               ld, ignore_index, dtype_code(logits2d), stream())
    return lse, row_loss, dlogits


def cross_entropy_bwd(logits2d, target, lse, grad_scale, V, ignore_index, dlogits=None):
    rows, ld = logits2d.shape[0], logits2d.stride(0)
    if dlogits is None:
        dlogits = torch.empty(rows, ld, dtype=logits2d.dtype, device=logits2d.device)
    lib().call("ofa_cross_entropy_bwd", ptr(logits2d), ptr(target), ptr(lse), ptr(grad_scale), ptr(dlogits), rows, V, ld,
               ignore_index, dtype_code(logits2d), stream())
    return dlogits


def ls_cross_entropy_fwd(logits2d, target, V, ignore_index, eps, cstart=-1, cend=-1, cmask=None):
    rows, ld = logits2d.shape[0], logits2d.stride(0)
    out = [torch.empty(rows, dtype=torch.float32, device=logits2d.device) for _ in range(4)]
    if cmask is not None:
        cmask = _u8(cmask)
    lib().call("ofa_ls_cross_entropy_fwd", ptr(logits2d), ptr(target), *[ptr(o) for o in out], rows, V, ld, ignore_index,
               float(eps), int(cstart), int(cend), ptr(cmask), dtype_code(logits2d), stream())
    return out


def ls_cross_entropy_bwd(logits2d, target, lse, row_cnt, row_w, grad_scale, V, ignore_index, eps, cstart=-1, cend=-1,
                         cmask=None):
    rows, ld = logits2d.shape[0], logits2d.stride(0)
    dlogits = torch.empty(rows, ld, dtype=logits2d.dtype, device=logits2d.device)
    if cmask is not None:
        cmask = _u8(cmask)
    lib().call("ofa_ls_cross_entropy_bwd", ptr(logits2d), ptr(target), ptr(lse), ptr(row_cnt), ptr(row_w), ptr(grad_scale),
               ptr(dlogits), rows, V, ld, ignore_index, float(eps), int(cstart), int(cend), ptr(cmask),
               dtype_code(logits2d), stream())
    return dlogits


def scst_loss_fwd_grad(logits2d, target, reward, grad_scale, V, ignore_index, rows_per_seq=1, row_seq=None, cstart=-1, cend=-1,
                       dlogits=None):
    rows, ld = logits2d.shape[0], logits2d.stride(0)
    assert reward.dtype == torch.float32 and reward.is_contiguous() and target.dtype == torch.int64 and target.is_contiguous()
    assert target.numel() == rows, (target.shape, rows)
    if row_seq is not None:
        assert row_seq.dtype == torch.int32 and row_seq.is_contiguous() and row_seq.numel() == rows, (row_seq.dtype, row_seq.shape)
    else:
        assert rows <= reward.numel() * int(rows_per_seq), (rows, reward.numel(), rows_per_seq)
    lse = torch.empty(rows, dtype=torch.float32, device=logits2d.device)
    row_loss = torch.empty(rows, dtype=torch.float32, device=logits2d.device)
    if dlogits is None:
        dlogits = torch.empty(rows, ld, dtype=logits2d.dtype, device=logits2d.device)
    lib().call("ofa_scst_loss_fwd_grad", ptr(logits2d), ptr(target), ptr(reward), ptr(row_seq), int(rows_per_seq), ptr(grad_scale),
               ptr(lse), ptr(row_loss), ptr(dlogits), rows, reward.numel(), V, ld, ignore_index, int(cstart), int(cend),
               dtype_code(logits2d), stream())
    return lse, row_loss, dlogits


def probs_fwd(logits2d, V, ld, log_probs):
    rows = logits2d.shape[0]
    y = torch.empty(rows, V, dtype=torch.float32, device=logits2d.device)
    lib().call("ofa_probs_fwd", ptr(logits2d), ptr(y), rows, V, ld, int(log_probs), dtype_code(logits2d), stream())
    return y


def probs_bwd(dy, y, V, dtype, log_probs):
    rows = y.shape[0]
    ld = (V + 7) // 8 * 8
    d = torch.empty(rows, ld, dtype=dtype, device=y.device)
    lib().call("ofa_probs_bwd", ptr(dy), ptr(y), ptr(d), rows, V, ld, int(log_probs), dtype_code(d), stream())
    return d


def sumsq(x, out):
    x = x.contiguous()
    ws = workspace(lib().cdll.ofa_sumsq_ws_floats() * 4, x.device, "sumsq")
    lib().call("ofa_sumsq", ptr(x), ptr(out), ptr(ws), x.numel(), dtype_code(x), stream())
    return out


def step_schedule(gsq, sample_size, step, lr, sched, gnorm, clip_norm, beta1, beta2):
    lib().call("ofa_step_schedule", ptr(gsq), ptr(sample_size), ptr(step), ptr(lr), ptr(sched), ptr(gnorm), float(clip_norm),
               float(beta1), float(beta2), stream())


def step_schedule_scaled(gsq, sample_size, step, lr, sched, gnorm, loss_scaler, clip_norm, beta1, beta2, scale_factor=2.0,
                         scale_window=2000, tolerance=0.0, threshold=None, min_loss_scale=1e-4):
    lib().call("ofa_step_schedule_scaled", ptr(gsq), ptr(sample_size), ptr(step), ptr(lr), ptr(sched), ptr(gnorm), ptr(loss_scaler),
               float(clip_norm), float(beta1), float(beta2), float(scale_factor), float(scale_window), float(tolerance),
               float(threshold or 0.0), float(min_loss_scale), stream())


def adam_step(master, exp_avg, exp_avg_sq, grad, model_param, coef, lr, beta1, beta2, eps, weight_decay, step):
    lib().call("ofa_adam_step", ptr(master), ptr(exp_avg), ptr(exp_avg_sq), ptr(grad), ptr(model_param), ptr(coef),
               master.numel(), float(lr), float(beta1), float(beta2), float(eps), float(weight_decay), int(step),
               dtype_code(grad), stream())


class _EmaSegment(ctypes.Structure):
    _fields_ = [("src", ctypes.c_void_p), ("off", ctypes.c_int64), ("len", ctypes.c_int64)]


def ema_step(state, p, shadow, step, sched, decay, start_update=0, update_freq=1, max_blocks=0):
    assert state.is_contiguous() and p.is_contiguous() and state.numel() == p.numel() and step.dtype == torch.float64
    assert shadow is None or (shadow.is_contiguous() and shadow.dtype == p.dtype and shadow.numel() == p.numel())
    lib().call("ofa_ema_step", ptr(state), ptr(p), ptr(shadow), p.numel(), ptr(step), ptr(sched), float(decay), int(start_update),
               int(update_freq), dtype_code(p), dtype_code(state), int(max_blocks), stream())


def ema_segment_table(sources, offsets, device):
    arr = (_EmaSegment * max(len(sources), 1))()
    for it, s, o in zip(arr, sources, offsets):
        assert s.is_contiguous()
        it.src, it.off, it.len = dptr(s), int(o), s.numel()
    raw = torch.frombuffer(bytearray(bytes(arr)), dtype=torch.int64).clone()
    return raw.to(device), max([s.numel() for s in sources], default=0)


def ema_segments_step(state, table, nseg, max_len, shadow, model_dtype, step, sched, decay, start_update=0, update_freq=1,
                      max_blocks=0):
    code = dtype_code(torch.empty(0, dtype=model_dtype))
    assert state.is_contiguous() and step.dtype == torch.float64 and table.dtype == torch.int64 and table.numel() >= 3 * nseg
    assert shadow is None or (shadow.is_contiguous() and shadow.numel() == state.numel() and shadow.dtype == model_dtype)
    lib().call("ofa_ema_segments_step", ptr(state), ptr(table), ptr(shadow), int(nseg), state.numel(), int(max_len), ptr(step),
               ptr(sched), float(decay), int(start_update), int(update_freq), code, dtype_code(state), int(max_blocks), stream())


def colsum(x, alpha=1.0, out=None, accumulate=False, out_dtype=torch.float32, fold=None, same_bits=False):
    if x.stride(-1) != 1:
        x = x.contiguous()
    rows, cols = x.shape
    if out is None:
        out = torch.empty(cols, dtype=out_dtype, device=x.device)
        fold = None
    if fold is not None and out.is_contiguous():
        ns = lib().cdll.ofa_colsum_slots(rows)
        ws = torch.empty(ns * cols, dtype=torch.float32, device=x.device)
        fold.add(ws, 0, out, cols, cols, ns, alpha, accumulate, lanes16=same_bits)
        lib().call("ofa_colsum", ptr(x), ptr(out), ptr(ws), rows, cols, x.stride(0), float(alpha), DEFER_FOLD,
                   dtype_code(x), dtype_code(out), stream())
        fold.flush_if_large()
        return out
    ws = workspace(lib().cdll.ofa_colsum_ws_floats(cols) * 4, x.device, "colsum")
    lib().call("ofa_colsum", ptr(x), ptr(out), ptr(ws), rows, cols, x.stride(0), float(alpha), int(accumulate),
               dtype_code(x), dtype_code(out), stream())
    return out


def mul(a, b):
    a, b = a.contiguous(), b.contiguous()
    rows, cols = _rows_cols(a)
    y = torch.empty_like(a)
    lib().call("ofa_mul", ptr(a), ptr(b), ptr(y), rows, cols, 0, dtype_code(a), stream())
    return y


def add_n(tensors):
    ts = [t.contiguous() for t in tensors]
    assert 1 <= len(ts) <= 16 and all(t.shape == ts[0].shape and t.dtype == ts[0].dtype for t in ts)
    if len(ts) == 1:
        return ts[0]
    out = torch.empty_like(ts[0])
    arr = (ctypes.c_void_p * len(ts))(*[dptr(t) for t in ts])
    lib().call("ofa_add_n", ctypes.addressof(arr), len(ts), ptr(out), out.numel(), dtype_code(out), stream())
    return out


def mul_rowvec(a, vec):
    a, vec = a.contiguous(), vec.contiguous()
    rows, cols = _rows_cols(a)
    y = torch.empty_like(a)
    lib().call("ofa_mul", ptr(a), ptr(vec), ptr(y), rows, cols, 1, dtype_code(a), stream())
    return y


def scale_row_groups(x, scale, group):
    x = x.contiguous()
    rows, cols = _rows_cols(x)
    assert scale.dtype == torch.float32 and scale.numel() * group == rows
    y = torch.empty_like(x)
    lib().call("ofa_scale_row_groups", ptr(x), ptr(scale.contiguous()), ptr(y), rows, cols, group, dtype_code(x), stream())
    return y


def sum_f32(x):
    x = x.contiguous()
    out = torch.empty((), dtype=torch.float32, device=x.device)
    lib().call("ofa_reduce_sum_f32", ptr(x), ptr(out), x.numel(), stream())
    return out


def bias_block_add_(bias, values, start):
    B, A, T, _ = bias.shape
    n = values.shape[0]
    values = values.contiguous()
    assert bias.is_contiguous() and values.dtype == bias.dtype
    lib().call("ofa_bias_block_add", ptr(bias), ptr(values), B, A, T, start, n, dtype_code(bias), stream())
    return bias
# ... 44 lines not shown

def head_sum(x, B, heads, T):
    out = torch.empty(heads, dtype=torch.float32, device=x.device)
    lib().call("ofa_head_sum_f32", ptr(x), ptr(out), B, heads, T, x.stride(0), stream())
    return out


def conv_out_size(n, k, stride, pad):
    return (n + 2 * pad - k) // stride + 1


def im2col(x, B, H, W, C, kh, kw, stride, pad, nchw=False):
    x = x.contiguous()
    Ho, Wo = conv_out_size(H, kh, stride, pad), conv_out_size(W, kw, stride, pad)
    K = kh * kw * C
    Kpad = (K + 7) // 8 * 8
    col = torch.empty(B * Ho * Wo, Kpad, dtype=x.dtype, device=x.device)
    lib().call("ofa_im2col", ptr(x), ptr(col), B, H, W, C, kh, kw, stride, pad, Kpad, int(nchw), dtype_code(x), stream())
    return col, Ho, Wo


def col2im(dcol, B, H, W, C, kh, kw, stride, pad):
    dcol = dcol.contiguous()
    dx = torch.empty(B * H * W, C, dtype=dcol.dtype, device=dcol.device)
    lib().call("ofa_col2im", ptr(dcol), ptr(dx), B, H, W, C, kh, kw, stride, pad, dcol.shape[1], dtype_code(dcol), stream())
    return dx


def batchnorm_fwd(x, gamma, beta, running_mean, running_var, training, momentum, eps, relu=False, residual=None):
    x = x.contiguous()
    rows, C = x.shape
    y = torch.empty_like(x)
    mean = torch.empty(C, dtype=torch.float32, device=x.device)
    rstd = torch.empty(C, dtype=torch.float32, device=x.device)
    ws = workspace(lib().cdll.ofa_batchnorm_ws_floats(C) * 4, x.device, "bn")
    if residual is not None:
        residual = residual.contiguous()
    lib().call("ofa_batchnorm_fwd", ptr(x), ptr(gamma), ptr(beta), ptr(residual), ptr(y), ptr(mean), ptr(rstd),
               ptr(running_mean), ptr(running_var), ptr(ws), rows, C, float(eps), float(momentum), int(not training),
               int(relu), dtype_code(x), stream())
    return y, mean, rstd


def batchnorm_bwd(dy, y, x, gamma, mean, rstd, batch_stats, relu, want_dres=False, dgamma=None, dbeta=None, beta=None):
    dy = dy.contiguous()
    rows, C = x.shape
    dx = torch.empty_like(x)
    dres = torch.empty_like(x) if want_dres else None
    acc = dgamma is not None
    if not acc:
        dgamma = torch.empty(C, dtype=gamma.dtype, device=x.device)
        dbeta = torch.empty(C, dtype=gamma.dtype, device=x.device)
    ws = workspace(lib().cdll.ofa_batchnorm_ws_floats(C) * 4, x.device, "bn")
    lib().call("ofa_batchnorm_bwd", ptr(dy), ptr(y), ptr(x), ptr(gamma), ptr(mean), ptr(rstd), ptr(dx), ptr(dres), ptr(dgamma),
               ptr(dbeta), ptr(ws), rows, C, int(batch_stats), int(relu), int(acc), ptr(beta) if (relu and not want_dres) else None,
               dtype_code(x), stream())
    return dx, dres, dgamma, dbeta


def batchnorm_fwd_stats(x):
    x = x.contiguous()
    rows, C = x.shape
    sums = torch.empty(2 * C + 1, dtype=torch.float64, device=x.device)
    ws = workspace(lib().cdll.ofa_batchnorm_ws_floats(C) * 4, x.device, "bn")
    lib().call("ofa_batchnorm_fwd_stats", ptr(x), ptr(sums), ptr(ws), rows, C, dtype_code(x), stream())
    return sums


def batchnorm_fwd_apply(x, gamma, beta, running_mean, running_var, sums, momentum, eps, relu=False, residual=None, groups=0):
    x = x.contiguous()
    rows, C = x.shape
    y = torch.empty_like(x)
    mean = torch.empty(C, dtype=torch.float32, device=x.device)
    rstd = torch.empty(C, dtype=torch.float32, device=x.device)
    if residual is not None:
        residual = residual.contiguous()
    lib().call("ofa_batchnorm_fwd_apply", ptr(x), ptr(gamma), ptr(beta), ptr(residual), ptr(y), ptr(mean), ptr(rstd),
               ptr(running_mean), ptr(running_var), ptr(sums), int(groups), rows, C, float(eps), float(momentum), int(relu),
               dtype_code(x), stream())
    return y, mean, rstd


def batchnorm_bwd_stats(dy, y, x, gamma, mean, rstd, relu, regate_beta=None, dgamma=None, dbeta=None):
    dy = dy.contiguous()
    rows, C = x.shape
    acc = dgamma is not None
    if not acc:
        dgamma = torch.empty(C, dtype=gamma.dtype, device=x.device)
        dbeta = torch.empty(C, dtype=gamma.dtype, device=x.device)
    sums = torch.empty(2, C, dtype=torch.float32, device=x.device)
    ws = workspace(lib().cdll.ofa_batchnorm_ws_floats(C) * 4, x.device, "bn")
    lib().call("ofa_batchnorm_bwd_stats", ptr(dy), ptr(y), ptr(x), ptr(gamma), ptr(mean), ptr(rstd), ptr(sums), ptr(dgamma), ptr(dbeta),
               ptr(ws), rows, C, int(relu), int(acc), ptr(regate_beta), dtype_code(x), stream())
    return sums, dgamma, dbeta


def batchnorm_bwd_dx(dy, y, x, gamma, mean, rstd, sums, total_rows, relu, want_dres=False, regate_beta=None):
    dy = dy.contiguous()
    rows, C = x.shape
    dx = torch.empty_like(x)
    dres = torch.empty_like(x) if want_dres else None
    assert total_rows.dtype == torch.float64 and total_rows.numel() == 1
    lib().call("ofa_batchnorm_bwd_dx", ptr(dy), ptr(y), ptr(x), ptr(gamma), ptr(mean), ptr(rstd), ptr(sums), ptr(dx), ptr(dres), rows,
               ptr(total_rows), C, int(relu), ptr(regate_beta), dtype_code(x), stream())
    return dx, dres


def maxpool_fwd(x, B, H, W, C, k, stride, pad):
    x = x.contiguous()
    Ho, Wo = conv_out_size(H, k, stride, pad), conv_out_size(W, k, stride, pad)
    y = torch.empty(B * Ho * Wo, C, dtype=x.dtype, device=x.device)
    arg = torch.empty(B * Ho * Wo, C, dtype=torch.uint8, device=x.device)
    lib().call("ofa_maxpool_fwd", ptr(x), ptr(y), ptr(arg), B, H, W, C, k, stride, pad, dtype_code(x), stream())
    return y, arg, Ho, Wo


def maxpool_bwd(dy, arg, B, H, W, C, k, stride, pad):
    dy = dy.contiguous()
    dx = torch.empty(B * H * W, C, dtype=dy.dtype, device=dy.device)
    lib().call("ofa_maxpool_bwd", ptr(dy), ptr(arg), ptr(dx), B, H, W, C, k, stride, pad, dtype_code(dy), stream())
    return dx


def relu(x, gate=None):
    x = x.contiguous()
    y = torch.empty_like(x)
    lib().call("ofa_relu", ptr(x), ptr(gate), ptr(y), x.numel(), dtype_code(x), stream())
    return y


def join_fwd(x, residual, ln_a, ln_b, eps, p, seed, offset, offset_base):
    x = x.contiguous()
    residual = residual.contiguous() if residual is not None else None
    rows, cols = _rows_cols(x)
    y = torch.empty_like(x)
    z = torch.empty_like(x) if ln_b is not None else None
    stats = torch.empty(4, rows, dtype=torch.float32, device=x.device)
    nkeep = lib().cdll.ofa_join_keep_bytes(rows, cols, dtype_code(x)) if p > 0 else 0
    keep = torch.empty(nkeep, dtype=torch.uint8, device=x.device) if nkeep else None
    ga, ba = ln_a if ln_a is not None else (None, None)
    gb, bb = ln_b if ln_b is not None else (None, None)
    lib().call("ofa_join_fwd", ptr(x), ptr(residual), ptr(ga), ptr(ba), ptr(gb), ptr(bb), ptr(y), ptr(z), ptr(stats), ptr(keep), rows, cols,
               float(eps), float(p), seed, offset, ptr(offset_base), dtype_code(x), stream())
    return y, z, stats, keep
# ... 204 lines not shown
```

ofasys_amd/ops.py:

```python

import weakref

import torch

from . import kernels as K
from .lib import OfaError


def rows_view(x):
    C = x.shape[-1]
    if x.is_contiguous():
        lead = x.shape[:-1]
        return x.view(-1, C), lambda y: y.view(*lead, y.shape[-1])
    if x.dim() == 3:
        xt = x.transpose(0, 1)
        if xt.is_contiguous():
            b, t = xt.shape[0], xt.shape[1]
            return xt.view(-1, C), lambda y: y.view(b, t, y.shape[-1]).transpose(0, 1)
    xc = x.contiguous()
    lead = xc.shape[:-1]
    return xc.view(-1, C), lambda y: y.view(*lead, y.shape[-1])


def like_layout(x, ref):
    if x.dim() != 3 or x.shape != ref.shape:
        return x
    ref_bm = ref.transpose(0, 1).is_contiguous() and not ref.is_contiguous()
    x_bm = x.transpose(0, 1).is_contiguous() and not x.is_contiguous()
    if ref_bm == x_bm and (x_bm or x.is_contiguous() == ref.is_contiguous()):
        return x
    if ref_bm:
        return x.transpose(0, 1).contiguous().transpose(0, 1)
    return x.contiguous()


def batch_major(x):
    xt = x.transpose(0, 1)
    return xt if xt.is_contiguous() else xt.contiguous()


class _Rng:
    seed = 0x5EED0FA
    offset = 0
    base = {}

    @classmethod
    def manual_seed(cls, seed):
        cls.seed, cls.offset = int(seed) & (2 ** 63 - 1), 0
        for b in cls.base.values():
            b.zero_()

    @classmethod
    def reserve(cls, n, device):
        o = cls.offset
        cls.offset += (n + 3) // 4 + 1
        b = cls.base.get(device)
        if b is None:
            b = cls.base[device] = torch.zeros(1, dtype=torch.int64, device=device)
        return cls.seed, o, b

    @classmethod
    def advance(cls):
        if cls.offset:
            for b in cls.base.values():
                b.add_(cls.offset)
            cls.offset = 0


manual_seed = _Rng.manual_seed
rng_advance = _Rng.advance


def _sink(param):
    return getattr(param, "_ofa_grad", None) if param is not None else None


def _sink_done(param):
    cb = getattr(param, "_ofa_grad_ready", None)
    if cb is not None:
        cb()


class _Fold:
    queue = None
    queued = False


def defer_reductions(flag):
    if flag and _Fold.queue is None:
        _Fold.queue = K.FoldQueue()
    elif not flag and _Fold.queue is not None:
        flush_folds()
        _Fold.queue = None


def drop_pending():
    _Wgrads.items, _Wgrads.fillers, _Wgrads.queued, _Fold.queued = [], [], False, False
    if _Fold.queue is not None:
        _Fold.queue.__init__()


def flush_folds():
    flush_wgrads()
    _Fold.queued = False
    if _Fold.queue is not None:
        _Fold.queue.flush()


def _fold():
    q = _Fold.queue
    if q is not None and not _Fold.queued:
        try:
            torch.autograd.Variable._execution_engine.queue_callback(flush_folds)
            _Fold.queued = True
        except RuntimeError:
            return None
    return q


def _edge_fold():
    return None if K.edge_old(K.EDGE_COLSUM_FOLD) else _fold()


class _Wgrads:
    enabled = True
    items = []
    fillers = []
    queued = False
    FLUSH_TILES = 128
    FILLER_TILES = 40
    use_fillers = True


# ... 1383 lines not shown
                    K.colsum(first, alpha=-1.0, out=gb, accumulate=True, fold=_edge_fold(), same_bits=True)
                _sink_done(bias)
            else:
                db = K.colsum(d2, out_dtype=dout.dtype)
                if lead:
                    db = db - K.colsum(first, out_dtype=dout.dtype)
        return None, dw, db, dcls, None


def patch_embed(img, weight, bias, p, cls_token=None):
    return PatchEmbedFn.apply(img, weight, bias, cls_token, p)


def _ce_rows(logits):
    V = logits.shape[-1]
    if logits.is_contiguous():
        l2d = logits.reshape(-1, V)
    else:
        try:
            l2d = logits.view(-1, V)
        except RuntimeError:
            l2d = logits.contiguous().view(-1, V)
    if l2d.stride(1) != 1 or l2d.stride(0) % (4 if l2d.dtype == torch.float32 else 8) != 0:
        pad = (-V) % 8
        store = torch.zeros(l2d.shape[0], V + pad, dtype=l2d.dtype, device=l2d.device)
        store[:, :V].copy_(l2d)
        l2d = store[:, :V]
    return l2d


class _SeededGrad:

    @staticmethod
    def usable(seed, device):
        return seed is not None and seed.dtype == torch.float32 and seed.numel() == 1 and seed.device == device

    def __init__(self, seed=None, pre=None):
        self.seed, self.version, self.pre = seed, None if seed is None else seed._version, pre

    def take(self, dloss):
        seed = self.seed
        if self.pre is None or dloss.data_ptr() != seed.data_ptr() or dloss.dtype != seed.dtype or seed._version != self.version:
            return None
        return self.spare()

    def spare(self):
        d, self.pre = self.pre, None
        return d


class CrossEntropyFn(torch.autograd.Function):

    @staticmethod
    def forward(ctx, logits, target, ignore_index, seed=None):
        V = logits.shape[-1]
        l2d = _ce_rows(logits)
        t = target.reshape(-1).contiguous()
        ctx.ignore_index, ctx.shape = ignore_index, logits.shape
        ctx.seeded = _SeededGrad()
        if ctx.needs_input_grad[0] and _SeededGrad.usable(seed, l2d.device) and K.cross_entropy_fwd_grad_ok(l2d, V):
            lse, row_loss, d = K.cross_entropy_fwd_grad(l2d, t, seed, V, ignore_index)
            ctx.seeded = _SeededGrad(seed, d)
        else:
            lse, row_loss = K.cross_entropy_fwd(l2d, t, V, ignore_index)
        ctx.save_for_backward(l2d, t, lse)
        return K.sum_f32(row_loss)

    @staticmethod
    def backward(ctx, dloss):
        l2d, t, lse = ctx.saved_tensors
        V = l2d.shape[1]
        d = ctx.seeded.take(dloss)
        if d is None:
            gs = dloss.reshape(1).float().contiguous()
            d = K.cross_entropy_bwd(l2d, t, lse, gs, V, ctx.ignore_index, dlogits=ctx.seeded.spare())
        return d[:, :V].view(ctx.shape), None, None, None


def cross_entropy_sum(logits, target, ignore_index, seed=None):
    return CrossEntropyFn.apply(logits, target, ignore_index, seed)


class LabelSmoothedCrossEntropyFn(torch.autograd.Function):

    @staticmethod
    def forward(ctx, logits, target, ignore_index, eps, constraint_range, constraint_masks, drop_worst_ratio):
        V = logits.shape[-1]
        l2d = _ce_rows(logits)
        t = target.reshape(-1).contiguous()
        cs, ce = constraint_range if constraint_range is not None else (-1, -1)
        cm = constraint_masks.reshape(-1, V).contiguous() if constraint_masks is not None else None
        lse, row_loss, row_nll, row_cnt = K.ls_cross_entropy_fwd(l2d, t, V, ignore_index, eps, cs, ce, cm)
        valid = t.ne(ignore_index)
        row_w = None
        if drop_worst_ratio > 0:
            n = valid.sum()
            k = (n.double() * (1 - drop_worst_ratio)).floor().long()
            key = torch.where(valid, row_loss, torch.full_like(row_loss, float("inf")))
            order = torch.argsort(key, stable=True)
            rank = torch.empty_like(order)
            rank[order] = torch.arange(order.numel(), device=order.device)
            row_w = (rank < k).float()
            row_loss, row_nll = row_loss * row_w, row_nll * row_w
            ntok = k
        else:
            ntok = valid.sum()
        ctx.save_for_backward(l2d, t, lse, row_cnt, row_w, cm)
        ctx.cfg = (ignore_index, eps, cs, ce, logits.shape)
        ctx.mark_non_differentiable(ntok)
        return K.sum_f32(row_loss), K.sum_f32(row_nll).detach(), ntok

    @staticmethod
    def backward(ctx, dloss, dnll, dntok):
        l2d, t, lse, row_cnt, row_w, cm = ctx.saved_tensors
        ignore_index, eps, cs, ce, shape = ctx.cfg
        V = l2d.shape[1]
        gs = dloss.reshape(1).float().contiguous()
        d = K.ls_cross_entropy_bwd(l2d, t, lse, row_cnt, row_w, gs, V, ignore_index, eps, cs, ce, cm)
        return d[:, :V].view(shape), None, None, None, None, None, None


def label_smoothed_cross_entropy(logits, target, ignore_index, eps, constraint_range=None, constraint_masks=None,
                                 drop_worst_ratio=0.0):
    return LabelSmoothedCrossEntropyFn.apply(logits, target, ignore_index, eps, constraint_range, constraint_masks,
                                             drop_worst_ratio)


class ScstLossFn(torch.autograd.Function):

    @staticmethod
    def forward(ctx, logits, target, reward, ignore_index, constraint_range, row_seq, seed):
        V = logits.shape[-1]
        l2d = _ce_rows(logits)
# ... 341 lines not shown
```

ofasys_amd/trainer.py:

```python
import os
import warnings
from typing import List

import torch
import torch.utils._python_dispatch

from . import kernels as K
from . import ops
from .distributed import GradBucketReducer, all_reduce_scalars
from .ema import EMA, as_config
from .lib import capture_audit


class FlatParams:

    def __init__(self, model: torch.nn.Module):
        from .module.multihead_attention import MultiheadAttention
        mha_of, mhas = {}, []
        for m in model.modules():
            if isinstance(m, MultiheadAttention) and m.q_proj.bias is not None:
                mhas.append(m)
                for p in (m.k_proj.weight, m.v_proj.weight, m.q_proj.weight, m.k_proj.bias, m.v_proj.bias, m.q_proj.bias):
                    mha_of[id(p)] = m
        cross = [m for m in mhas if getattr(m, "encoder_decoder_attention", False) and not m.self_attention]
        cross_ok = len(cross) > 1 and len({tuple(m.k_proj.weight.shape) for m in cross}) == 1 and \
            all(m.kdim == m.vdim and m.k_proj.weight.shape == m.v_proj.weight.shape for m in cross) and \
            all(q.requires_grad for m in cross for q in (m.k_proj.weight, m.v_proj.weight, m.k_proj.bias, m.v_proj.bias))
        cross_group = []
        if cross_ok:
            cross_group = [w for m in cross for w in (m.k_proj.weight, m.v_proj.weight)] + \
                [b for m in cross for b in (m.k_proj.bias, m.v_proj.bias)]
        cross_ids = {id(q) for q in cross_group}
        seen, params = set(), []
        for p in model.parameters():
            if not p.requires_grad or id(p) in seen:
                continue
            m = mha_of.get(id(p))
            group = [p]
            if id(p) in cross_ids:
                group = cross_group
            elif m is not None:
                if m.self_attention:
                    group = [m.k_proj.weight, m.v_proj.weight, m.q_proj.weight, m.k_proj.bias, m.v_proj.bias, m.q_proj.bias]
                elif cross_ok and m in cross:
                    group = [m.q_proj.weight, m.q_proj.bias]
                else:
                    group = [m.k_proj.weight, m.v_proj.weight, m.k_proj.bias, m.v_proj.bias, m.q_proj.weight, m.q_proj.bias]
                if not all(g.requires_grad for g in group):
                    group = [p]
            for g in group:
                if id(g) not in seen:
                    seen.add(id(g))
                    params.append(g)
        assert params, "no trainable parameters"
        self.params = params
        self._plain4d = {id(w) for m in model.modules() for w in getattr(m, "_ofa_plain_conv_weights", lambda: ())()}
        dtype, device = params[0].dtype, params[0].device
        self.offsets, off = [], 0
        for p in params:
            assert p.dtype == dtype and p.device == device
            self.offsets.append(off)
            off += (p.numel() + 7) // 8 * 8
        self.numel = off
        self.flat = torch.zeros(off, dtype=dtype, device=device)
        self.grad = torch.zeros(off, dtype=dtype, device=device)
        with torch.no_grad():
            for p, o in zip(params, self.offsets):
                self._view(self.flat, o, p).copy_(p.data)
                p.data = self._view(self.flat, o, p)
                p.grad = self._view(self.grad, o, p)
                p._ofa_grad = p.grad
        off_of = {id(p): o for p, o in zip(params, self.offsets)}
        for m in mhas:
            n = 3 if m.self_attention else 2
            kw, kb = m.k_proj.weight, m.k_proj.bias
            if id(kw) not in off_of or kw.shape[0] != kw.shape[1] and not m.self_attention and m.kdim != m.embed_dim:
                continue
            D, Kin = kw.shape
            ow, ob = off_of[id(kw)], off_of[id(kb)]
            ws = [m.k_proj.weight, m.v_proj.weight, m.q_proj.weight][:n]
            bs = [m.k_proj.bias, m.v_proj.bias, m.q_proj.bias][:n]
            ok = all(off_of.get(id(w)) == ow + i * D * Kin for i, w in enumerate(ws)) and \
                all(off_of.get(id(b)) == ob + i * D for i, b in enumerate(bs)) and (D * Kin) % 8 == 0 and D % 8 == 0
            if ok:
                m._pack = {"w": self.flat[ow:ow + n * D * Kin].view(n * D, Kin), "b": self.flat[ob:ob + n * D],
                           "gw": self.grad[ow:ow + n * D * Kin].view(n * D, Kin), "gb": self.grad[ob:ob + n * D]}
        if cross_ok:
            L = len(cross)
            D, Kin = cross[0].k_proj.weight.shape
            ow, ob = off_of[id(cross[0].k_proj.weight)], off_of[id(cross[0].k_proj.bias)]
            ok = all(off_of.get(id(w)) == ow + i * D * Kin for i, w in enumerate(cross_group[:2 * L])) and \
                all(off_of.get(id(b)) == ob + i * D for i, b in enumerate(cross_group[2 * L:])) and (D * Kin) % 8 == 0 and D % 8 == 0
            if ok:
                pack = {"w": self.flat[ow:ow + 2 * L * D * Kin].view(2 * L * D, Kin), "b": self.flat[ob:ob + 2 * L * D],
                        "gw": self.grad[ow:ow + 2 * L * D * Kin].view(2 * L * D, Kin), "gb": self.grad[ob:ob + 2 * L * D],
                        "params": tuple(cross_group), "layers": L, "D": D}
                for i, m in enumerate(cross):
                    m._cross_all = (pack, i)

    def _view(self, buf, o, p):
        n = p.numel()
        if p.dim() == 4 and p.shape[2] * p.shape[3] > 1 and (p.shape[1] * p.shape[2] * p.shape[3]) % 8 == 0 \
                and id(p) not in self._plain4d:
            Cout, Cin, kh, kw = p.shape
            return buf[o:o + n].view(Cout, kh, kw, Cin).permute(0, 3, 1, 2)
        return buf[o:o + n].view(p.shape)

    def zero_grad(self):
        self.grad.zero_()
        for p, o in zip(self.params, self.offsets):
            if p.grad is None or p.grad.data_ptr() != self.grad.data_ptr() + o * self.grad.element_size():
                p.grad = self._view(self.grad, o, p)
                p._ofa_grad = p.grad


class _AtenAudit(torch.utils._python_dispatch.TorchDispatchMode):

    def __init__(self, audit):
        super().__init__()
        self.audit = audit

    def __torch_dispatch__(self, func, types, args=(), kwargs=None):
        for a in args:
            if torch.is_tensor(a):
                if a.is_cuda:
                    self.audit.see(a)
            elif isinstance(a, (list, tuple)):
                for b in a:
                    if torch.is_tensor(b) and b.is_cuda:
                        self.audit.see(b)
        self.audit.label("aten::" + getattr(func, "__name__", str(func)))
        return func(*args, **(kwargs or {}))


_CAPTURE_MODE = "thread_local"


_KEEP_ALIVE = []


class _Uncapturable(Exception):
    """A sample holds something the static-input walker does not understand: the step must stay eager."""


def _walk(obj, path, out):
    if torch.is_tensor(obj):
        out.append((path, obj))
    elif isinstance(obj, dict):
        for k in obj:
            _walk(obj[k], path + (k,), out)
    elif isinstance(obj, (list, tuple)):
        for i, v in enumerate(obj):
            _walk(v, path + (i,), out)
    elif hasattr(obj, "modality") and hasattr(obj, "is_src"):
        _walk(obj.value, path + ("value",), out)
    elif hasattr(obj, "tensors") and hasattr(obj, "structure"):
        for i, t in enumerate(obj.tensors()):
            out.append((path + (i,), t))
    elif obj is None or isinstance(obj, (str, int, float, bool)):
        pass
    else:
        raise _Uncapturable(f"{'/'.join(map(str, path))}: {type(obj).__name__}")
# ... 21 lines not shown

class TrainStep:

    def __init__(self, model, lr=1e-4, betas=(0.9, 0.999), eps=1e-8, weight_decay=0.0, clip_norm=1.0, process_group=None,
                 bucket_bytes: int = 64 << 20, use_graph: bool = False, graph_warmup: int = 2,
                 label_smoothing: float = 0.0, constraint_range=None, drop_worst_ratio: float = 0.0, dp_graph: str = None,
                 loss_scale=None, max_graphs: int = 16, shard_optimizer: bool = False, ema=None):
        self.model = model
        self.fp = FlatParams(model)
        dev = self.fp.flat.device
        self.master = self.fp.flat.float().clone() if self.fp.flat.dtype != torch.float32 else self.fp.flat
        self.exp_avg = torch.zeros(self.fp.numel, dtype=torch.float32, device=dev)
        self.exp_avg_sq = torch.zeros(self.fp.numel, dtype=torch.float32, device=dev)
        self.betas, self.eps, self.weight_decay, self.clip_norm = betas, eps, weight_decay, clip_norm
        self.num_updates = 0
        self.group = process_group
        self.shard_optimizer = bool(shard_optimizer)
        self.reducer = GradBucketReducer(self.fp.params, self.fp.grad, self.fp.offsets, process_group, bucket_bytes,
                                         shard=self.shard_optimizer)
        self.world = self.reducer.world
        self.pad = model.global_dict.pad()
        self.label_smoothing, self.constraint_range, self.drop_worst_ratio = label_smoothing, constraint_range, drop_worst_ratio
        self._stats = torch.zeros(3, dtype=torch.float64, device=dev)
        self._gsq = torch.zeros(1, dtype=torch.float32, device=dev)
        self._gnorm_t = torch.zeros(1, dtype=torch.float32, device=dev)
        self._step_t = torch.zeros(1, dtype=torch.float64, device=dev)
        self._lr_t = torch.full((1,), float(lr), dtype=torch.float64, device=dev)
        self._sched = torch.zeros(5, dtype=torch.float32, device=dev)
        self._lr = float(lr)
        self.use_graph = bool(use_graph) and dev.type == "cuda"
        self.dynamic_autograd = any(float(getattr(m, "layerdrop", 0.0) or 0.0) > 0.0 for m in model.modules())
        if self.use_graph and self.dynamic_autograd:
            warnings.warn("ofasys_amd.TrainStep: LayerDrop draws the kept layers on the host every step; the step is not captured")
            self.use_graph = False
        self.sync_collectives = any(getattr(m, "_ofa_sync", None) not in (None, False) for m in model.modules())
        if self.sync_collectives and self.world > 1 and any(getattr(m, "_ofa_sync", None) is True for m in model.modules()):
            ops.sync_bn_process_group()
        self.graph_warmup = graph_warmup
        default_dp = "full"
        if self.world > 1:
            import torch.distributed as dist
            if dist.get_backend(process_group) != "nccl":
                default_dp = "split"
        self.dp_graph = dp_graph or os.environ.get("OFA_DP_GRAPH") or default_dp
        assert self.dp_graph in ("full", "split"), self.dp_graph
        self.loss_scale_cfg = None
        if loss_scale is not None:
            cfg = {"init_scale": 2.0 ** 7, "scale_factor": 2.0, "scale_window": 2000, "tolerance": 0.0, "threshold": None,
                   "min_loss_scale": 1e-4}
            cfg.update(loss_scale if isinstance(loss_scale, dict) else {})
            self.loss_scale_cfg = cfg
            self._ls = torch.tensor([cfg["init_scale"], 0, -1, -1, 0, 0, 0, 0], dtype=torch.float64, device=dev)
        self._graphs = {}
        self.max_graphs = int(max_graphs)
        self._pool = None
        self._warned_cap = False
        self._skipped_seen = 0.0
        self._seed = torch.ones((), dtype=torch.float32, device=dev)
        self.last = {}
        ema_cfg = as_config(ema)
        self.ema = EMA(model, self.fp, ema_cfg, step_t=self._step_t) if ema_cfg is not None else None

    @property
    def lr(self):
        return self._lr

    @lr.setter
    def lr(self, value):
        self._lr = float(value)
        self._lr_t.fill_(self._lr)

    def _fwd_bwd(self, samples, overlap_reduce, structure=None):
        model = self.model
        model.train()
        ops.drop_pending()
        self.fp.zero_grad()
        self._stats.zero_()
        self.reducer.overlap = overlap_reduce
        ops.defer_reductions(self.world == 1 or not overlap_reduce)
        self.reducer.begin_step(structure, dynamic=self.dynamic_autograd or self.sync_collectives)
        for s in samples:
            plan = s.get("pack")
            target = s["target"]
            if plan is None:
                logits = model(s["slots"])[0]
            else:
                logits = model(s["slots"], pack=plan)[0]
                target = s.get("target_packed")
                if target is None:
                    idx = plan.dec_index
                    target = s["target"].reshape(-1)[idx.clamp_min(0)].masked_fill(idx < 0, self.pad).view(1, -1)
            cm = s.get("constraint_masks")
            if plan is not None and cm is not None:
                raise NotImplementedError("constraint masks are laid out by padded position: run such samples without a pack plan")
            counted = False
            size = None
            if s.get("reward") is not None:
                if cm is not None:
                    raise NotImplementedError("an SCST micro-batch (reward) cannot carry constraint_masks: its criterion takes a "
                                              "constraint range only (engine/criterion/scst_loss.py:214-217)")
                row_seq = None
                if plan is not None:
                    row_seq = torch.div(plan.dec_index, s["target"].shape[1], rounding_mode="floor").to(torch.int32)
                cr = s.get("constraint_range")
                cr = tuple(int(v) for v in cr.split(",")) if cr is not None else self.constraint_range
                if self.loss_scale_cfg is None and (self._seed is None or self._seed.device != logits.device):
                    self._seed = torch.ones((), dtype=torch.float32, device=logits.device)
                loss, n = ops.scst_loss(logits, target, s["reward"], self.pad, cr, row_seq,
                                        seed=self._seed if self.loss_scale_cfg is None else None)
                if s.get("sentence_avg"):
                    size = s["reward"].numel()
            elif self.label_smoothing > 0 or self.constraint_range is not None or self.drop_worst_ratio > 0 or cm is not None:
                loss, _, n = ops.label_smoothed_cross_entropy(logits, target, self.pad, self.label_smoothing,
                                                              self.constraint_range, cm, self.drop_worst_ratio)
            else:
                if self.loss_scale_cfg is None and (self._seed is None or self._seed.device != logits.device):
                    self._seed = torch.ones((), dtype=torch.float32, device=logits.device)
                loss = ops.cross_entropy_sum(logits, target, self.pad, seed=self._seed if self.loss_scale_cfg is None else None)
                n = None
                if loss.is_cuda and loss.dtype == torch.float32 and target.is_contiguous() and target.dtype == torch.int64:
                    K.step_stats_add(self._stats, loss.detach(), target, self.pad)
                    counted = True
                else:
                    n = target.ne(self.pad).sum()
            if self.loss_scale_cfg is None:
                if self._seed is None or self._seed.shape != loss.shape or self._seed.dtype != loss.dtype or self._seed.device != loss.device:
                    self._seed = torch.ones_like(loss)
                loss.backward(self._seed)
            else:
                loss.backward(self._ls[0].to(loss.dtype))
            if not counted:
                self._stats[0] += n if size is None else size
                self._stats[1] += loss.detach().double()
                self._stats[2] += n
        ops.flush_folds()
        ops.rng_advance()

    def _reduce(self):
        self.reducer.finish()
        all_reduce_scalars(self._stats, self.group)

    def _update(self):
        self._gsq.zero_()
        owned = self.reducer.owned_ranges()
        for lo, hi, counted in owned:
            if counted:
                K.sumsq(self.fp.grad[lo:hi], self._gsq)
        if self.shard_optimizer and self.world > 1:
            import torch.distributed as dist
            dist.all_reduce(self._gsq, op=dist.ReduceOp.SUM, group=self.group)
        if self.loss_scale_cfg is None:
            K.step_schedule(self._gsq, self._stats, self._step_t, self._lr_t, self._sched, self._gnorm_t, self.clip_norm,
                            self.betas[0], self.betas[1])
        else:
            c = self.loss_scale_cfg
            K.step_schedule_scaled(self._gsq, self._stats, self._step_t, self._lr_t, self._sched, self._gnorm_t, self._ls,
                                   self.clip_norm, self.betas[0], self.betas[1], c["scale_factor"], c["scale_window"],
                                   c["tolerance"], c["threshold"], c["min_loss_scale"])
        for lo, hi, _ in owned:
            K.adam_step(self.master[lo:hi], self.exp_avg[lo:hi], self.exp_avg_sq[lo:hi], self.fp.grad[lo:hi], self.fp.flat[lo:hi],
                        self._sched, 0.0, self.betas[0], self.betas[1], self.eps, self.weight_decay, 0)
        self.reducer.gather_params(self.fp.flat)
        self._gnorm = self._gnorm_t
        if self.ema is not None:
            self.ema._enqueue(self._step_t, self._sched)

    def check(self):
        if self.loss_scale_cfg is not None:
            if float(self._ls[5]) != 0.0:
                raise FloatingPointError(f"Minimum loss scale reached ({self.loss_scale_cfg['min_loss_scale']}). Your loss is "
                                         "probably exploding. Try lowering the learning rate, using gradient clipping or "
                                         "increasing the batch size.")
            return
        skipped = float(self._sched[4])
        if skipped > self._skipped_seen:
            n = int(skipped - self._skipped_seen)
            self._skipped_seen = skipped
            raise FloatingPointError(f"gradients are Nan/Inf (or sample_size == 0) in {n} update(s): skipped on the device")

    def captured_graphs(self):
        return sum(1 for e in self._graphs.values() if "graphs" in e)

    def _capture(self, samples, structure, mode):
        import gc
        gc.collect()
        if self._pool is None:
            self._pool = torch.cuda.graph_pool_handle()
        pool = self._pool
        entry = {"static": samples, "graphs": [], "mode": mode}
        with capture_audit() as audit, _AtenAudit(audit):
            if self.world == 1 or mode == "full":
                g = torch.cuda.CUDAGraph()
                _KEEP_ALIVE.append(g)
                with torch.cuda.graph(g, pool=pool, capture_error_mode=_CAPTURE_MODE):
                    self._fwd_bwd(samples, overlap_reduce=self.world > 1, structure=structure)
                    if self.world > 1:
                        self._reduce()
                    self._update()
                entry["graphs"] = [g]
            else:
                ga, gb = torch.cuda.CUDAGraph(), torch.cuda.CUDAGraph()
                _KEEP_ALIVE.extend((ga, gb))
                with torch.cuda.graph(ga, pool=pool, capture_error_mode=_CAPTURE_MODE):
                    self._fwd_bwd(samples, overlap_reduce=False)
                with torch.cuda.graph(gb, pool=pool, capture_error_mode=_CAPTURE_MODE):
                    self._update()
                entry["graphs"] = [ga, gb]
        entry["audit"] = audit
        if os.environ.get("OFA_CAPTURE_PINS", "1") != "0":
            entry["pins"] = audit.tensors()
        return entry
# ... 82 lines not shown
```

Measured before the change: 1.413 million.

## Fuse training step tail: CE stats, sumsq+schedule, and first-touch grad zeroing

Cross-entropy forward+grad now accumulates loss and token-count stats inside the kernel, using a last-block ticket. This removes the separate step_stats_add launch. Gradient sum-of-squares and the LR/clip schedule are fused into a single ticketed kernel that also applies the deferred RNG counter advance. The full gradient-buffer zero is replaced by first-touch tracking: GEMMs store instead of accumulate, and only demanded regions are pre-zeroed with a batched zero kernel. This cuts launches and memory traffic in the step tail, but adds complexity around per-structure demand caching and atomic ticket correctness.

```diff
diff --git a/include/ofasys_amd.h b/include/ofasys_amd.h
--- a/include/ofasys_amd.h
+++ b/include/ofasys_amd.h
@@ -70,6 +70,7 @@
   void* out;
   int64_t ldo;
   float out_alpha;
+  int32_t store;
 } ofa_gemm_group_item;
 int ofa_gemm_group_plan(ofa_gemm_group_item* items, int n, int dtype);
 int ofa_gemm_group_tn(const ofa_gemm_group_item* items, int n, int dtype, void* stream);
@@ -142,6 +143,8 @@
 int ofa_embedding_range_bwd(const void* dout, void* dweight, int batch, int64_t T, int D, int64_t V, int64_t r0, int dtype, void* stream);
 enum { OFA_EDGE_POS_RANGE = 0, OFA_EDGE_TOKEN_BWD = 1, OFA_EDGE_COLSUM_FOLD = 2, OFA_EDGE_IM2COL = 3 };
 int ofa_step_edges_old(int item);
+enum { OFA_TAIL_FIRST_TOUCH = 0, OFA_TAIL_NORM_SCHEDULE = 1, OFA_TAIL_CRITERION_STATS = 2 };
+int ofa_step_tail_old(int item);
 
 int ofa_gelu_fwd(const void* x, void* y, int64_t n, int dtype, void* stream);
 int ofa_gelu_bwd(const void* dy, const void* x, void* dx, int64_t n, int dtype, void* stream);
@@ -189,6 +192,9 @@
 int ofa_cross_entropy_fwd_grad_ok(int64_t V, int64_t ld, int dtype);
 int ofa_cross_entropy_fwd_grad(const void* logits, const int64_t* target, const float* grad_scale, float* lse, float* row_loss,
                                void* dlogits, int64_t rows, int64_t V, int64_t ld, int64_t ignore_index, int dtype, void* stream);
+int ofa_cross_entropy_fwd_grad_stats(const void* logits, const int64_t* target, const float* grad_scale, float* lse, float* row_loss,
+                                     void* dlogits, int64_t rows, int64_t V, int64_t ld, int64_t ignore_index, int dtype, float* loss,
+                                     double* stats, unsigned int* ticket, void* stream);
 int ofa_cross_entropy_bwd(const void* logits, const int64_t* target, const float* lse, const float* grad_scale,
                           void* dlogits, int64_t rows, int64_t V, int64_t ld, int64_t ignore_index, int dtype,
                           void* stream);
@@ -214,6 +220,10 @@
               int64_t n, int dtype, void* stream);
 int ofa_step_schedule(const float* gsq, const double* sample_size, double* step, const double* lr, float* sched,
                       float* gnorm, float clip_norm, double beta1, double beta2, void* stream);
+int ofa_sumsq_schedule(const void* x, float* gsq, float* ws, unsigned int* ticket, int64_t n, int dtype, const double* sample_size,
+                       double* step, const double* lr, float* sched, float* gnorm, double* loss_scaler, int64_t* counter,
+                       int64_t counter_add, float clip_norm, double beta1, double beta2, double scale_factor, double scale_window,
+                       double tolerance, double threshold, double min_loss_scale, void* stream);
 int ofa_step_stats_add(double* stats, const float* loss, const int64_t* target, int64_t n, int64_t pad, void* stream);
 int ofa_step_schedule_scaled(const float* gsq, const double* sample_size, double* step, const double* lr, float* sched,
                              float* gnorm, double* loss_scaler, float clip_norm, double beta1, double beta2, double scale_factor,
@@ -273,6 +283,7 @@
   int64_t bytes;
 } ofa_copy_job;
 int ofa_copy_batched(const ofa_copy_job* jobs, int njobs, void* stream);
+int ofa_zero_batched(const ofa_copy_job* jobs, int njobs, void* stream);
 #define OFA_DEFER_FOLD 2
 int ofa_layernorm_bwd_slots(int64_t rows, int cols, int dtype, int gelu);
 int ofa_colsum_slots(int64_t rows);
diff --git a/ofasys_amd/csrc/elementwise.hip b/ofasys_amd/csrc/elementwise.hip
--- a/ofasys_amd/csrc/elementwise.hip
+++ b/ofasys_amd/csrc/elementwise.hip
@@ -804,6 +804,13 @@
   return 0;
 }
 
+extern "C" int ofa_step_tail_old(int item) {
+#ifdef OFA_DEBUG_SWITCHES
+  if (const char* e = getenv("OFA_STEP_TAIL_OLD")) return (atoi(e) >> item) & 1;
+#endif
+  return 0;
+}
+
 extern "C" int ofa_embedding_bwd_ids_ok(int64_t n, int D, int64_t V, int dtype) {
   const int vecn = dt_vecn(dtype);
   return OFA_DT_OK(dtype) && n >= 0 && n <= OFA_EMBEDDING_IDS_MAX && V > 0 && V < ((int64_t)1 << 31) && D > 0 && D % vecn == 0 &&
diff --git a/ofasys_amd/csrc/fold.hip b/ofasys_amd/csrc/fold.hip
--- a/ofasys_amd/csrc/fold.hip
+++ b/ofasys_amd/csrc/fold.hip
@@ -202,15 +202,22 @@
   int njobs;
 };
 
-__global__ __launch_bounds__(256) void copy_batched_kernel(CopyJobs J) {
+__device__ __forceinline__ int copy_job_of(const CopyJobs& J, int64_t& off, int& n) {
   int lo = 0, hi = J.njobs - 1;
   while (lo < hi) {
     const int mid = (lo + hi + 1) >> 1;
     if (J.block0[mid] <= blockIdx.x) lo = mid; else hi = mid - 1;
   }
-  const int64_t off = (int64_t)(blockIdx.x - J.block0[lo]) * COPY_CHUNK;
+  off = (int64_t)(blockIdx.x - J.block0[lo]) * COPY_CHUNK;
   const int64_t left = J.bytes[lo] - off;
-  const int n = (int)(left < COPY_CHUNK ? left : COPY_CHUNK);
+  n = (int)(left < COPY_CHUNK ? left : COPY_CHUNK);
+  return lo;
+}
+
+__global__ __launch_bounds__(256) void copy_batched_kernel(CopyJobs J) {
+  int64_t off;
+  int n;
+  const int lo = copy_job_of(J, off, n);
   const unsigned char* s = J.src[lo] + off;
   unsigned char* d = J.dst[lo] + off;
   if ((((uintptr_t)s | (uintptr_t)d) & 15) == 0) {
@@ -222,11 +229,26 @@
   }
 }
 
+__global__ __launch_bounds__(256) void zero_batched_kernel(CopyJobs J) {
+  int64_t off;
+  int n;
+  const int lo = copy_job_of(J, off, n);
+  unsigned char* d = J.dst[lo] + off;
+  int head = (int)((16 - ((uintptr_t)d & 15)) & 15);
+  head = head < n ? head : n;
+  for (int i = threadIdx.x; i < head; i += 256) d[i] = 0;
+  const int nv = (n - head) >> 4;
+  uint4* v = reinterpret_cast<uint4*>(d + head);
+  for (int i = threadIdx.x; i < nv; i += 256) v[i] = make_uint4(0, 0, 0, 0);
+  for (int i = head + (nv << 4) + threadIdx.x; i < n; i += 256) d[i] = 0;
+}
+
 }
 using namespace ofa;
 
-extern "C" int ofa_copy_batched(const ofa_copy_job* jobs, int njobs, void* stream) {
-  OFA_REQUIRE(njobs >= 0 && (njobs == 0 || jobs), OFA_ERR_INVALID, "copy_batched: bad argument");
+template <bool ZERO>
+static int copy_jobs_launch(const ofa_copy_job* jobs, int njobs, void* stream, const char* what) {
+  OFA_REQUIRE(njobs >= 0 && (njobs == 0 || jobs), OFA_ERR_INVALID, "%s: bad argument", what);
   hipStream_t st = (hipStream_t)stream;
   for (int base = 0; base < njobs; base += COPY_MAX_JOBS) {
     CopyJobs J;
@@ -235,9 +257,9 @@
     unsigned blocks = 0;
     for (int i = 0; i < n; ++i) {
       const ofa_copy_job& b = jobs[base + i];
-      OFA_REQUIRE(b.bytes >= 0 && (b.bytes == 0 || (b.src && b.dst)), OFA_ERR_INVALID, "copy_batched: bad job %d", base + i);
+      OFA_REQUIRE(b.bytes >= 0 && (b.bytes == 0 || (b.dst && (ZERO || b.src))), OFA_ERR_INVALID, "%s: bad job %d", what, base + i);
       if (b.bytes == 0) continue;
-      J.src[m] = (const unsigned char*)b.src; J.dst[m] = (unsigned char*)b.dst; J.bytes[m] = b.bytes;
+      J.src[m] = ZERO ? nullptr : (const unsigned char*)b.src; J.dst[m] = (unsigned char*)b.dst; J.bytes[m] = b.bytes;
       J.block0[m] = blocks;
       blocks += (unsigned)((b.bytes + COPY_CHUNK - 1) / COPY_CHUNK);
       ++m;
@@ -245,11 +267,20 @@
     if (m == 0) continue;
     J.block0[m] = blocks;
     J.njobs = m;
-    hipLaunchKernelGGL(copy_batched_kernel, dim3(blocks), dim3(256), 0, st, J);
-    int rc = check_launch("copy_batched");
+    if (ZERO) hipLaunchKernelGGL(zero_batched_kernel, dim3(blocks), dim3(256), 0, st, J);
+    else hipLaunchKernelGGL(copy_batched_kernel, dim3(blocks), dim3(256), 0, st, J);
+    int rc = check_launch(what);
     if (rc) return rc;
   }
   return 0;
+}
+
+extern "C" int ofa_zero_batched(const ofa_copy_job* jobs, int njobs, void* stream) {
+  return copy_jobs_launch<true>(jobs, njobs, stream, "zero_batched");
+}
+
+extern "C" int ofa_copy_batched(const ofa_copy_job* jobs, int njobs, void* stream) {
+  return copy_jobs_launch<false>(jobs, njobs, stream, "copy_batched");
 }
 
 extern "C" int ofa_fold_batched(const ofa_fold_job* jobs, int njobs, void* stream) {
diff --git a/ofasys_amd/csrc/gemm_core.h b/ofasys_amd/csrc/gemm_core.h
--- a/ofasys_amd/csrc/gemm_core.h
+++ b/ofasys_amd/csrc/gemm_core.h
@@ -481,6 +481,7 @@
 struct GroupItem {
   const void* A; const void* B; float* ws;
   void* out; int64_t ldo; float alpha;
+  int store;
   int64_t lda, ldb;
   int M, N, K, krows, ksplit, splits, tiles_m, tiles_n, first;
 };
@@ -495,7 +496,7 @@
   g.A = it.A; g.B = it.B; g.C = it.out; g.bias = nullptr;
   g.M = it.M; g.N = it.N; g.K = it.K; g.transA = 1; g.transB = 0;
   g.lda = it.lda; g.ldb = it.ldb; g.ldc = it.ldo; g.strideA = g.strideB = g.strideC = 0;
-  g.alpha = it.out ? it.alpha : 1.f; g.flags = it.out ? OFA_GEMM_ACCUM : 0; g.batch_inner = 1; g.strideA2 = g.strideB2 = g.strideC2 = 0; g.a_krows = g.b_krows = it.krows;
+  g.alpha = it.out ? it.alpha : 1.f; g.flags = (it.out && !it.store) ? OFA_GEMM_ACCUM : 0; g.batch_inner = 1; g.strideA2 = g.strideB2 = g.strideC2 = 0; g.a_krows = g.b_krows = it.krows;
   g.colstat = nullptr; g.colstat_rows = 0;
   const int ntiles = it.tiles_m * it.tiles_n, local = id - it.first;
   ks = local / ntiles;
diff --git a/ofasys_amd/csrc/gemm_mfma.hip b/ofasys_amd/csrc/gemm_mfma.hip
--- a/ofasys_amd/csrc/gemm_mfma.hip
+++ b/ofasys_amd/csrc/gemm_mfma.hip
@@ -1066,7 +1066,7 @@
     OFA_REQUIRE(it.splits >= 1 && it.splits <= 32, OFA_ERR_INVALID, "gemm_group: product %d: splits %d (run ofa_gemm_group_plan)", p, it.splits);
     GroupItem& d = ga.it[p];
     d.A = it.a; d.B = it.b; d.ws = it.slabs; d.lda = it.lda; d.ldb = it.ldb;
-    d.out = direct ? it.out : nullptr; d.ldo = it.ldo; d.alpha = it.out_alpha;
+    d.out = direct ? it.out : nullptr; d.ldo = it.ldo; d.alpha = it.out_alpha; d.store = it.store != 0;
     d.M = it.m; d.N = it.n; d.K = cdiv(it.k, BK) * BK; d.krows = it.k;
     d.ksplit = cdiv(cdiv(it.k, BK), it.splits) * BK;
     d.splits = it.splits;
diff --git a/ofasys_amd/csrc/loss_optim.hip b/ofasys_amd/csrc/loss_optim.hip
--- a/ofasys_amd/csrc/loss_optim.hip
+++ b/ofasys_amd/csrc/loss_optim.hip
@@ -102,10 +102,11 @@
 template <typename T, int NV>
 __global__ __launch_bounds__(1024) __attribute__((amdgpu_waves_per_eu(8))) void ce_fwd_grad_kernel(
     const T* __restrict__ logits, const int64_t* __restrict__ target, const float* __restrict__ gscale, float* __restrict__ lse,
-    float* __restrict__ row_loss, T* __restrict__ dlogits, int V, int ld, int64_t ignore_index) {
+    float* __restrict__ row_loss, T* __restrict__ dlogits, int V, int ld, int64_t ignore_index, float* __restrict__ loss_out,
+    double* __restrict__ stats, unsigned* __restrict__ ticket) {
   constexpr int N = Vec<T>::N;
   static_assert(N == 8, "16-bit element types");
-  __shared__ float sm[16], ss[16];
+  __shared__ float sm[17], ss[16];
   const int64_t row = blockIdx.x;
   const char* xb = reinterpret_cast<const char*>(logits + row * ld);
   char* db = reinterpret_cast<char*>(dlogits + row * ld);
@@ -150,7 +151,14 @@
   const bool dead = ignored || t < 0;
   if (tid == 0) {
     lse[row] = l;
-    row_loss[row] = ignored ? 0.f : t < 0 ? INFINITY : l - ld1<T>(reinterpret_cast<const T*>(xb) + t);
+    const float rl = ignored ? 0.f : t < 0 ? INFINITY : l - ld1<T>(reinterpret_cast<const T*>(xb) + t);
+    if (ticket) {
+      __hip_atomic_store(row_loss + row, rl, __ATOMIC_RELAXED, __HIP_MEMORY_SCOPE_AGENT);
+      asm volatile("s_waitcnt vmcnt(0)" ::: "memory");
+      sm[16] = __hip_atomic_fetch_add(ticket, 1u, __ATOMIC_RELAXED, __HIP_MEMORY_SCOPE_AGENT) == gridDim.x - 1 ? 1.f : 0.f;
+    } else {
+      row_loss[row] = rl;
+    }
   }
   const float g = dead ? 0.f : (gscale ? gscale[0] : 1.0f);
   const Exp2Fma prob(l);
@@ -170,6 +178,31 @@
     uint4 w;
     w.x = pack2<T>(o[0], o[1]); w.y = pack2<T>(o[2], o[3]); w.z = pack2<T>(o[4], o[5]); w.w = pack2<T>(o[6], o[7]);
     *reinterpret_cast<uint4*>(db + (uint32_t)v * 16u) = w;
+  }
+  if (!ticket) return;
+  __syncthreads();
+  if (sm[16] == 0.f) return;
+  const int64_t rows = gridDim.x;
+  float ls_ = 0.f;
+  int cnt = 0;
+  if (tid < 256)
+    for (int64_t i = tid; i < rows; i += 256) {
+      ls_ += __hip_atomic_load(row_loss + i, __ATOMIC_RELAXED, __HIP_MEMORY_SCOPE_AGENT);
+      cnt += target[i] != ignore_index;
+    }
+  ls_ = wave_sum(ls_);
+#pragma unroll
+  for (int o = 32; o > 0; o >>= 1) cnt += __shfl_xor(cnt, o, 64);
+  if (tid < 256 && (tid & 63) == 0) { ss[tid >> 6] = ls_; sm[tid >> 6] = __int_as_float(cnt); }
+  __syncthreads();
+  if (tid == 0) {
+    const float loss = ss[0] + ss[1] + ss[2] + ss[3];
+    const double c = (double)(__float_as_int(sm[0]) + __float_as_int(sm[1]) + __float_as_int(sm[2]) + __float_as_int(sm[3]));
+    loss_out[0] = loss;
+    stats[0] += c;
+    stats[1] += (double)loss;
+    stats[2] += c;
+    *ticket = 0u;
   }
 }
 
@@ -686,13 +719,12 @@
   }
 }
 
-__global__ void step_schedule_kernel(const float* __restrict__ gsq, const double* __restrict__ sample_size,
-                                     double* __restrict__ step, const double* __restrict__ lr, float* __restrict__ sched,
-                                     float* __restrict__ gnorm, float clip_norm, double beta1, double beta2) {
-  if (threadIdx.x || blockIdx.x) return;
+__device__ __forceinline__ void step_schedule_one(float gsq0, const double* __restrict__ sample_size, double* __restrict__ step,
+                                                  const double* __restrict__ lr, float* __restrict__ sched, float* __restrict__ gnorm,
+                                                  float clip_norm, double beta1, double beta2) {
   const double n = sample_size[0];
   const float inv_n = n > 0.0 ? (float)(1.0 / n) : 0.f;
-  const float gn = sqrtf(gsq[0]) * inv_n;
+  const float gn = sqrtf(gsq0) * inv_n;
   gnorm[0] = n > 0.0 ? gn : __builtin_nanf("");
   if (!(n > 0.0) || !isfinite(gn)) {
     sched[0] = 0.f;
@@ -713,17 +745,22 @@
   sched[2] = (float)lr[0];
   gnorm[0] = gn;
 }
-
-__global__ void step_schedule_scaled_kernel(const float* __restrict__ gsq, const double* __restrict__ sample_size,
-                                            double* __restrict__ step, const double* __restrict__ lr, float* __restrict__ sched,
-                                            float* __restrict__ gnorm, double* __restrict__ ls, float clip_norm, double beta1,
-                                            double beta2, double scale_factor, double scale_window, double tolerance,
-                                            double threshold, double min_loss_scale) {
+__global__ void step_schedule_kernel(const float* __restrict__ gsq, const double* __restrict__ sample_size,
+                                     double* __restrict__ step, const double* __restrict__ lr, float* __restrict__ sched,
+                                     float* __restrict__ gnorm, float clip_norm, double beta1, double beta2) {
   if (threadIdx.x || blockIdx.x) return;
+  step_schedule_one(gsq[0], sample_size, step, lr, sched, gnorm, clip_norm, beta1, beta2);
+}
+
+__device__ __forceinline__ void step_schedule_scaled_one(float gsq0, const double* __restrict__ sample_size, double* __restrict__ step,
+                                                         const double* __restrict__ lr, float* __restrict__ sched,
+                                                         float* __restrict__ gnorm, double* __restrict__ ls, float clip_norm,
+                                                         double beta1, double beta2, double scale_factor, double scale_window,
+                                                         double tolerance, double threshold, double min_loss_scale) {
   const double n = sample_size[0];
   const double scale = ls[0];
   double mf = n > 0.0 ? 1.0 / (scale * n) : 0.0;
-  const float gn = (float)(mf * sqrt((double)gsq[0]));
+  const float gn = (float)(mf * sqrt((double)gsq0));
   gnorm[0] = n > 0.0 ? gn : __builtin_nanf("");
   if (!(n > 0.0)) {
     sched[0] = 0.f;
@@ -774,6 +811,65 @@
   }
   ls[1] = it + 1.0;
 }
+__global__ void step_schedule_scaled_kernel(const float* __restrict__ gsq, const double* __restrict__ sample_size,
+                                            double* __restrict__ step, const double* __restrict__ lr, float* __restrict__ sched,
+                                            float* __restrict__ gnorm, double* __restrict__ ls, float clip_norm, double beta1,
+                                            double beta2, double scale_factor, double scale_window, double tolerance,
+                                            double threshold, double min_loss_scale) {
+  if (threadIdx.x || blockIdx.x) return;
+  step_schedule_scaled_one(gsq[0], sample_size, step, lr, sched, gnorm, ls, clip_norm, beta1, beta2, scale_factor, scale_window,
+                           tolerance, threshold, min_loss_scale);
+}
+
+struct SchedArgs {
+  const double* sample_size; double* step; const double* lr; float* sched; float* gnorm; double* ls;
+  int64_t* counter; int64_t counter_add;
+  float clip_norm; double beta1, beta2, scale_factor, scale_window, tolerance, threshold, min_loss_scale;
+};
+template <typename T>
+__global__ __launch_bounds__(256) void sumsq_schedule_kernel(const T* __restrict__ x, float* __restrict__ partial,
+                                                             float* __restrict__ gsq, unsigned* __restrict__ ticket, int64_t n,
+                                                             SchedArgs a) {
+  constexpr int N = Vec<T>::N;
+  __shared__ float sw[4];
+  __shared__ float fin[4];
+  float s = 0.f;
+  const int64_t nvec = n / N;
+  for (int64_t v = (int64_t)blockIdx.x * 256 + threadIdx.x; v < nvec; v += (int64_t)gridDim.x * 256) {
+    float e[N];
+    load_vec<T>(x + v * N, e);
+#pragma unroll
+    for (int j = 0; j < N; ++j) s += e[j] * e[j];
+  }
+  if (blockIdx.x == 0)
+    for (int64_t e = nvec * N + threadIdx.x; e < n; e += 256) { const float q = ld1<T>(x + e); s += q * q; }
+  s = wave_sum(s);
+  if ((threadIdx.x & 63) == 0) sw[threadIdx.x >> 6] = s;
+  __syncthreads();
+  if (threadIdx.x == 0) {
+    __hip_atomic_store(partial + blockIdx.x, sw[0] + sw[1] + sw[2] + sw[3], __ATOMIC_RELAXED, __HIP_MEMORY_SCOPE_AGENT);
+    asm volatile("s_waitcnt vmcnt(0)" ::: "memory");
+    const bool last = __hip_atomic_fetch_add(ticket, 1u, __ATOMIC_RELAXED, __HIP_MEMORY_SCOPE_AGENT) == gridDim.x - 1;
+    fin[0] = last ? 1.f : 0.f;
+  }
+  __syncthreads();
+  if (fin[0] == 0.f) return;
+  const int nb = (int)gridDim.x;
+  float t = 0.f;
+  for (int i = threadIdx.x; i < nb; i += 256) t += __hip_atomic_load(partial + i, __ATOMIC_RELAXED, __HIP_MEMORY_SCOPE_AGENT);
+  t = wave_sum(t);
+  if ((threadIdx.x & 63) == 0) sw[threadIdx.x >> 6] = t;
+  __syncthreads();
+  if (threadIdx.x == 0) {
+    const float total = 0.f + (sw[0] + sw[1] + sw[2] + sw[3]);
+    gsq[0] = total;
+    if (a.ls) step_schedule_scaled_one(total, a.sample_size, a.step, a.lr, a.sched, a.gnorm, a.ls, a.clip_norm, a.beta1, a.beta2,
+                                       a.scale_factor, a.scale_window, a.tolerance, a.threshold, a.min_loss_scale);
+    else step_schedule_one(total, a.sample_size, a.step, a.lr, a.sched, a.gnorm, a.clip_norm, a.beta1, a.beta2);
+    if (a.counter) a.counter[0] += a.counter_add;
+    *ticket = 0u;
+  }
+}
 }
 using namespace ofa;
 
@@ -793,9 +889,10 @@
 
 template <typename T>
 static bool ce_fwd_grad_launch(const T* logits, const int64_t* target, const float* gs, float* lse, float* row_loss, T* dlogits,
-                               int64_t rows, int64_t V, int64_t ld, int64_t ignore_index, hipStream_t st) {
+                               int64_t rows, int64_t V, int64_t ld, int64_t ignore_index, hipStream_t st, float* loss_out = nullptr,
+                               double* stats = nullptr, unsigned* ticket = nullptr) {
   const int64_t per_thread = (ld / 8 + 1023) / 1024;
-#define CE_FG(NV) hipLaunchKernelGGL((ce_fwd_grad_kernel<T, NV>), dim3((unsigned)rows), dim3(1024), 0, st, logits, target, gs, lse, row_loss, dlogits, (int)V, (int)ld, ignore_index)
+#define CE_FG(NV) hipLaunchKernelGGL((ce_fwd_grad_kernel<T, NV>), dim3((unsigned)rows), dim3(1024), 0, st, logits, target, gs, lse, row_loss, dlogits, (int)V, (int)ld, ignore_index, loss_out, stats, ticket)
   if (per_thread <= 1) CE_FG(1);
   else if (per_thread <= 2) CE_FG(2);
   else if (per_thread <= 4) CE_FG(4);
@@ -824,6 +921,24 @@
   });
   OFA_REQUIRE(ok, OFA_ERR_UNSUPPORTED, "cross_entropy_fwd_grad: row too long");
   return check_launch("cross_entropy_fwd_grad");
+}
+
+extern "C" int ofa_cross_entropy_fwd_grad_stats(const void* logits, const int64_t* target, const float* grad_scale, float* lse,
+                                                float* row_loss, void* dlogits, int64_t rows, int64_t V, int64_t ld,
+                                                int64_t ignore_index, int dtype, float* loss, double* stats, unsigned int* ticket,
+                                                void* stream) {
+  OFA_REQUIRE(ofa_cross_entropy_fwd_grad_ok(V, ld, dtype), OFA_ERR_UNSUPPORTED,
+              "cross_entropy_fwd_grad_stats: 16-bit logits of at most 65536 (padded) columns, ld a multiple of 8 (V=%lld ld=%lld dtype=%d)", (long long)V, (long long)ld, dtype);
+  OFA_REQUIRE(rows >= 1 && logits && target && lse && row_loss && dlogits && loss && stats && ticket, OFA_ERR_INVALID,
+              "cross_entropy_fwd_grad_stats: bad argument");
+  hipStream_t st = (hipStream_t)stream;
+  const bool ok = dispatch_dtype16(dtype, [&](auto tag) {
+    using T = typename decltype(tag)::type;
+    return ce_fwd_grad_launch<T>((const T*)logits, target, grad_scale, lse, row_loss, (T*)dlogits, rows, V, ld, ignore_index, st, loss,
+                                 stats, ticket);
+  });
+  OFA_REQUIRE(ok, OFA_ERR_UNSUPPORTED, "cross_entropy_fwd_grad_stats: row too long");
+  return check_launch("cross_entropy_fwd_grad_stats");
 }
 
 extern "C" int ofa_cross_entropy_bwd(const void* logits, const int64_t* target, const float* lse, const float* grad_scale,
@@ -961,6 +1076,29 @@
   if (rc) return rc;
   hipLaunchKernelGGL(sumsq_final_kernel, dim3(1), dim3(256), 0, st, (const float*)ws, out, nb);
   return check_launch("sumsq_final");
+}
+
+extern "C" int ofa_sumsq_schedule(const void* x, float* gsq, float* ws, unsigned int* ticket, int64_t n, int dtype,
+                                  const double* sample_size, double* step, const double* lr, float* sched, float* gnorm,
+                                  double* loss_scaler, int64_t* counter, int64_t counter_add, float clip_norm, double beta1,
+                                  double beta2, double scale_factor, double scale_window, double tolerance, double threshold,
+                                  double min_loss_scale, void* stream) {
+  OFA_REQUIRE(OFA_DT_OK(dtype), OFA_ERR_INVALID, "sumsq_schedule: bad dtype %d", dtype);
+  OFA_REQUIRE(n >= 1 && x && gsq && ws && ticket && sample_size && step && lr && sched && gnorm, OFA_ERR_INVALID,
+              "sumsq_schedule: bad argument");
+  OFA_REQUIRE(!loss_scaler || (scale_factor > 1.0 && scale_window >= 1.0 && min_loss_scale >= 0.0), OFA_ERR_INVALID,
+              "sumsq_schedule: bad scaler configuration");
+  hipStream_t st = (hipStream_t)stream;
+  const int vecw = dt_vecn(dtype);
+  int64_t nbl = (n / vecw + 255) / 256;
+  const int nb = (int)(nbl < 1 ? 1 : (nbl > 1024 ? 1024 : nbl));
+  SchedArgs a{sample_size, step, lr, sched, gnorm, loss_scaler, counter, counter_add, clip_norm, beta1, beta2,
+              scale_factor, scale_window, tolerance, threshold, min_loss_scale};
+  dispatch_dtype(dtype, [&](auto tag) {
+    using T = typename decltype(tag)::type;
+    hipLaunchKernelGGL((sumsq_schedule_kernel<T>), dim3(nb), dim3(256), 0, st, (const T*)x, ws, gsq, ticket, n, a);
+  });
+  return check_launch("sumsq_schedule");
 }
 
 extern "C" int ofa_adam_step(float* master, float* exp_avg, float* exp_avg_sq, const void* grad, void* model_param,
diff --git a/ofasys_amd/kernels.py b/ofasys_amd/kernels.py
--- a/ofasys_amd/kernels.py
+++ b/ofasys_amd/kernels.py
@@ -57,6 +57,38 @@
         lib().call("ofa_copy_batched", ctypes.addressof(arr), len(jobs), stream())
 
 
+def zero_batched(bufs):
+    if bufs:
+        arr = (_CopyJob * len(bufs))()
+        for it, (d_, n) in zip(arr, bufs):
+            it.src, it.dst, it.bytes = None, d_, n
+        lib().call("ofa_zero_batched", ctypes.addressof(arr), len(bufs), stream())
+
+
+grad_mode = None
+
+
+def _accum(out, accumulate, full=True):
+    if grad_mode is None:
+        return bool(accumulate)
+    if accumulate:
+        return bool(grad_mode(out, full))
+    grad_mode(out, full, store=True)
+    return False
+
+
+def _accum_all(outs):
+    if grad_mode is None:
+        return True
+    if all(grad_mode(o, True, peek=True) is False for o in outs):
+        for o in outs:
+            grad_mode(o, True)
+        return False
+    for o in outs:
+        grad_mode(o, False)
+    return True
+
+
 DEFER_FOLD = 2
 FOLD_LANES16 = 4
 GEMM_DEFER_REDUCE = 128
@@ -68,6 +100,7 @@
 
     def __init__(self):
         self.jobs, self.keep, self.bytes, self.outs, self.want_flush = [], [], 0, set(), False
+        self.modes = []
 
     def add(self, part, part_off, out, cols, stride, nslots, alpha=1.0, accumulate=True, flush_ok=True, lanes16=False):
         assert part.dtype == torch.float32 and out.is_contiguous()
@@ -76,6 +109,7 @@
         self.outs.add(out.data_ptr())
         self.jobs.append(_FoldJob(dptr(part) + part_off * 4, dptr(out), cols, stride, nslots,
                                   int(bool(accumulate)) | (FOLD_LANES16 if lanes16 else 0), float(alpha), dtype_code(out)))
+        self.modes.append((bool(accumulate), FOLD_LANES16 if lanes16 else 0))
         self.keep.append((part, out))
         self.bytes += nslots * stride * 4
         self.want_flush = self.bytes > self.MAX_PENDING_BYTES
@@ -87,9 +121,12 @@
     def flush(self):
         if not self.jobs:
             return
+        for job, (_, out), (want, bits) in zip(self.jobs, self.keep, self.modes):
+            job.accumulate = int(_accum(out, want)) | bits
         arr = (_FoldJob * len(self.jobs))(*self.jobs)
         lib().call("ofa_fold_batched", ctypes.addressof(arr), len(self.jobs), stream())
         self.jobs, self.keep, self.bytes, self.want_flush = [], [], 0, False
+        self.modes = []
         self.outs = set()
 
 
@@ -98,7 +135,7 @@
     def add(self, part, part_off, out, cols, stride, nslots, alpha=1.0, accumulate=True, flush_ok=True, lanes16=False):
         assert part.dtype == torch.float32 and out.is_contiguous()
         job = (_FoldJob * 1)(_FoldJob(dptr(part) + part_off * 4, dptr(out), cols, stride, nslots,
-                                      int(bool(accumulate)) | (FOLD_LANES16 if lanes16 else 0), float(alpha), dtype_code(out)))
+                                      int(_accum(out, accumulate)) | (FOLD_LANES16 if lanes16 else 0), float(alpha), dtype_code(out)))
         lib().call("ofa_fold_batched", ctypes.addressof(job), 1, stream())
 
     def flush_if_large(self):
@@ -149,6 +186,8 @@
         acc = DEFER_FOLD
     else:
         ws = workspace(wsr * cols * 4, x.device, "ln")
+        if acc:
+            acc = _accum_all([o for o in (dgamma, dbeta, dbias if fuse_gelu else None) if o is not None])
     if fuse_gelu:
         lib().call("ofa_gelu_layernorm_bwd", ptr(dy), ptr(x), ptr(gamma), ptr(mean), ptr(rstd), ptr(dx), ptr(dgamma),
                    ptr(dbeta), ptr(dbias), ptr(ws), rows, cols, int(acc), dtype_code(x), stream())
@@ -210,6 +249,8 @@
     if ws is None:
         ws = workspace(256 << 20, a.device, "gemm")
         ws_bytes = ws.numel() * 4
+        if not _accum(out, accumulate, full=ldc == N and (not batched or sc == M * N)):
+            flags &= ~GEMM_ACCUM
     args = ("ofa_gemm", ptr(a), ptr(b), ptr(out), ptr(bias), M, N, K, int(trans_a), int(trans_b), lda, ldb, ldc, batch,
             sa, sb, sc, 0, 0, 0, 0, float(alpha), flags, dt, ptr(ws), ws_bytes, stream())
     if _prof is not None:
@@ -258,7 +299,8 @@
 class _GroupItem(ctypes.Structure):
     _fields_ = [("a", ctypes.c_void_p), ("b", ctypes.c_void_p), ("slabs", ctypes.c_void_p), ("lda", ctypes.c_int64),
                 ("ldb", ctypes.c_int64), ("m", ctypes.c_int32), ("n", ctypes.c_int32), ("k", ctypes.c_int32),
-                ("splits", ctypes.c_int32), ("out", ctypes.c_void_p), ("ldo", ctypes.c_int64), ("out_alpha", ctypes.c_float)]
+                ("splits", ctypes.c_int32), ("out", ctypes.c_void_p), ("ldo", ctypes.c_int64), ("out_alpha", ctypes.c_float),
+                ("store", ctypes.c_int32)]
 
 
 GROUP_MAX = 16
@@ -287,6 +329,7 @@
         if direct:
             direct_outs.add(out.data_ptr())
             it.out, it.ldo, it.out_alpha = dptr(out), out.stride(0), float(alpha)
+            it.store = int(not _accum(out, True, full=out.is_contiguous()))
             slabs.append(None)
         else:
             sl = torch.empty(it.splits * it.m * it.n, dtype=torch.float32, device=dy.device)
@@ -448,7 +491,7 @@
     if out is None:
         out = torch.empty_like(c_attn)
         accumulate = False
-    lib().call("ofa_c_attn_grad", ptr(delta), ptr(c_attn), ptr(out), B, heads, T, delta.stride(0), int(accumulate),
+    lib().call("ofa_c_attn_grad", ptr(delta), ptr(c_attn), ptr(out), B, heads, T, delta.stride(0), int(_accum(out, accumulate)),
                dtype_code(c_attn), stream())
     return out
 
@@ -688,7 +731,7 @@
     if out is None:
         out = torch.empty(n, dtype=x.dtype, device=x.device)
         accumulate = False
-    lib().call("ofa_batch_sum", ptr(x), ptr(out), int(batch), n, int(bool(accumulate)), dtype_code(x), stream())
+    lib().call("ofa_batch_sum", ptr(x), ptr(out), int(batch), n, int(_accum(out, accumulate)), dtype_code(x), stream())
     return out
 
 
@@ -734,6 +777,13 @@
     return out
 
 
+TAIL_FIRST_TOUCH, TAIL_NORM_SCHEDULE, TAIL_CRITERION_STATS = 0, 1, 2
+
+
+def tail_old(item):
+    return bool(lib().cdll.ofa_step_tail_old(int(item)))
+
+
 EDGE_POS_RANGE, EDGE_TOKEN_BWD, EDGE_COLSUM_FOLD, EDGE_IM2COL = 0, 1, 2, 3
 
 
@@ -747,6 +797,8 @@
     D = dout.shape[-1]
     if dweight is None:
         dweight = torch.zeros(V, D, dtype=dout.dtype, device=dout.device)
+    else:
+        _accum(dweight, True, full=False)
     S = lib().cdll.ofa_embedding_bwd_slices(V, D)
     pad = -1 if padding_idx is None else padding_idx
     if id_major is None:
@@ -771,12 +823,15 @@
     V, D = dweight.shape
     batch = dout.numel() // (T * D)
     assert dweight.is_contiguous() and dweight.dtype == dout.dtype and batch * T * D == dout.numel()
+    _accum(dweight, True, full=False)
     lib().call("ofa_embedding_range_bwd", ptr(dout), ptr(dweight), batch, T, D, V, int(r0), dtype_code(dout), stream())
     return dweight
 
 
 def segment_rowsum(dout2d, plan, dweight, accumulate):
     assert dout2d.dim() == 2 and dout2d.is_contiguous() and dweight.is_contiguous() and dout2d.dtype == dweight.dtype
+    if accumulate:
+        _accum(dweight, True, full=False)
     lib().call("ofa_segment_rowsum", ptr(dout2d), ptr(plan.order), ptr(plan.seg_off), ptr(plan.seg_row), ptr(dweight), plan.nseg,
                dout2d.shape[1], int(accumulate), dtype_code(dout2d), stream())
     return dweight
@@ -810,11 +865,18 @@
     return logits2d.is_cuda and bool(lib().cdll.ofa_cross_entropy_fwd_grad_ok(int(V), int(logits2d.stride(0)), dtype_code(logits2d)))
 
 
-def cross_entropy_fwd_grad(logits2d, target, grad_scale, V, ignore_index):
+def cross_entropy_fwd_grad(logits2d, target, grad_scale, V, ignore_index, stats=None, ticket=None):
     rows, ld = logits2d.shape[0], logits2d.stride(0)
     lse = torch.empty(rows, dtype=torch.float32, device=logits2d.device)
     row_loss = torch.empty(rows, dtype=torch.float32, device=logits2d.device)
     dlogits = torch.empty(rows, ld, dtype=logits2d.dtype, device=logits2d.device)
+    if stats is not None:
+        assert stats.dtype == torch.float64 and stats.numel() >= 3 and ticket.dtype == torch.int32 and rows >= 1
+        assert target.dtype == torch.int64 and target.is_contiguous() and target.numel() == rows
+        loss = torch.empty((), dtype=torch.float32, device=logits2d.device)
+        lib().call("ofa_cross_entropy_fwd_grad_stats", ptr(logits2d), ptr(target), ptr(grad_scale), ptr(lse), ptr(row_loss), ptr(dlogits),
+                   rows, V, ld, ignore_index, dtype_code(logits2d), ptr(loss), ptr(stats), ptr(ticket), stream())
+        return lse, row_loss, dlogits, loss
     lib().call("ofa_cross_entropy_fwd_grad", ptr(logits2d), ptr(target), ptr(grad_scale), ptr(lse), ptr(row_loss), ptr(dlogits), rows, V,
                ld, ignore_index, dtype_code(logits2d), stream())
     return lse, row_loss, dlogits
@@ -892,6 +954,16 @@
     return out
 
 
+def sumsq_schedule(x, gsq, ticket, sample_size, step, lr, sched, gnorm, clip_norm, beta1, beta2, loss_scaler=None, scale_factor=2.0,
+                   scale_window=2000, tolerance=0.0, threshold=None, min_loss_scale=1e-4, counter=None, counter_add=0):
+    assert x.is_contiguous() and x.numel() >= 1 and ticket.dtype == torch.int32 and (counter is None or counter.dtype == torch.int64)
+    ws = workspace(lib().cdll.ofa_sumsq_ws_floats() * 4, x.device, "sumsq")
+    lib().call("ofa_sumsq_schedule", ptr(x), ptr(gsq), ptr(ws), ptr(ticket), x.numel(), dtype_code(x), ptr(sample_size), ptr(step),
+               ptr(lr), ptr(sched), ptr(gnorm), ptr(loss_scaler), ptr(counter), int(counter_add), float(clip_norm), float(beta1),
+               float(beta2), float(scale_factor), float(scale_window), float(tolerance), float(threshold or 0.0), float(min_loss_scale),
+               stream())
+
+
 def step_schedule(gsq, sample_size, step, lr, sched, gnorm, clip_norm, beta1, beta2):
     lib().call("ofa_step_schedule", ptr(gsq), ptr(sample_size), ptr(step), ptr(lr), ptr(sched), ptr(gnorm), float(clip_norm),
                float(beta1), float(beta2), stream())
@@ -955,8 +1027,8 @@
         fold.flush_if_large()
         return out
     ws = workspace(lib().cdll.ofa_colsum_ws_floats(cols) * 4, x.device, "colsum")
-    lib().call("ofa_colsum", ptr(x), ptr(out), ptr(ws), rows, cols, x.stride(0), float(alpha), int(accumulate),
-               dtype_code(x), dtype_code(out), stream())
+    lib().call("ofa_colsum", ptr(x), ptr(out), ptr(ws), rows, cols, x.stride(0), float(alpha),
+               int(_accum(out, accumulate, full=out.is_contiguous())), dtype_code(x), dtype_code(out), stream())
     return out
 
 
@@ -1107,6 +1179,8 @@
         dgamma = torch.empty(C, dtype=gamma.dtype, device=x.device)
         dbeta = torch.empty(C, dtype=gamma.dtype, device=x.device)
     ws = workspace(lib().cdll.ofa_batchnorm_ws_floats(C) * 4, x.device, "bn")
+    if acc:
+        acc = _accum_all([dgamma, dbeta])
     lib().call("ofa_batchnorm_bwd", ptr(dy), ptr(y), ptr(x), ptr(gamma), ptr(mean), ptr(rstd), ptr(dx), ptr(dres), ptr(dgamma),
                ptr(dbeta), ptr(ws), rows, C, int(batch_stats), int(relu), int(acc), ptr(beta) if (relu and not want_dres) else None,
                dtype_code(x), stream())
@@ -1145,6 +1219,8 @@
         dbeta = torch.empty(C, dtype=gamma.dtype, device=x.device)
     sums = torch.empty(2, C, dtype=torch.float32, device=x.device)
     ws = workspace(lib().cdll.ofa_batchnorm_ws_floats(C) * 4, x.device, "bn")
+    if acc:
+        acc = _accum_all([dgamma, dbeta])
     lib().call("ofa_batchnorm_bwd_stats", ptr(dy), ptr(y), ptr(x), ptr(gamma), ptr(mean), ptr(rstd), ptr(sums), ptr(dgamma), ptr(dbeta),
                ptr(ws), rows, C, int(relu), int(acc), ptr(regate_beta), dtype_code(x), stream())
     return sums, dgamma, dbeta
diff --git a/ofasys_amd/ops.py b/ofasys_amd/ops.py
--- a/ofasys_amd/ops.py
+++ b/ofasys_amd/ops.py
@@ -67,8 +67,19 @@
             cls.offset = 0
 
 
+    @classmethod
+    def defer(cls):
+        if cls.offset and len(cls.base) == 1:
+            (b,) = cls.base.values()
+            o, cls.offset = cls.offset, 0
+            return b, o
+        cls.advance()
+        return None
+
+
 manual_seed = _Rng.manual_seed
 rng_advance = _Rng.advance
+rng_defer = _Rng.defer
 
 
 def _sink(param):
@@ -79,6 +90,115 @@
     cb = getattr(param, "_ofa_grad_ready", None)
     if cb is not None:
         cb()
+
+
+class _Touched:
+    arena = None
+    spans = []
+    demand = []
+    unused = []
+
+
+def _zero_ranges(arena, ranges, also=()):
+    es = arena.element_size()
+    K.zero_batched([(K.dptr(arena) + lo * es, (hi - lo) * es) for lo, hi in ranges] +
+                   [(K.dptr(t), t.numel() * t.element_size()) for t in also])
+
+
+def _span_gaps(lo, hi):
+    import bisect
+    spans, gaps = _Touched.spans, []
+    i = bisect.bisect_right(spans, (lo, float("inf"))) - 1
+    if i >= 0 and spans[i][1] > lo:
+        lo = spans[i][1]
+    i += 1
+    while lo < hi:
+        if i < len(spans) and spans[i][0] < hi:
+            if spans[i][0] > lo:
+                gaps.append((lo, spans[i][0]))
+            lo = max(lo, spans[i][1])
+            i += 1
+        else:
+            gaps.append((lo, hi))
+            break
+    return gaps
+
+
+def _span_mark(lo, hi):
+    import bisect
+    spans = _Touched.spans
+    i = bisect.bisect_left(spans, (lo, lo))
+    if i > 0 and spans[i - 1][1] >= lo:
+        i -= 1
+    j = i
+    while j < len(spans) and spans[j][0] <= hi:
+        lo, hi = min(lo, spans[j][0]), max(hi, spans[j][1])
+        j += 1
+    spans[i:j] = [(lo, hi)]
+
+
+def grad_begin(arena, prezero=(), also=()):
+    _Touched.arena, _Touched.spans, _Touched.demand, _Touched.unused = arena, [], [], []
+    prezero = [(max(0, lo), min(arena.numel(), hi)) for lo, hi in prezero if lo < hi]
+    if prezero or also:
+        _zero_ranges(arena, prezero, also)
+        for lo, hi in prezero:
+            _span_mark(lo, hi)
+
+
+def _dense(t):
+    want = 1
+    for n, st in sorted(((n, st) for n, st in zip(t.shape, t.stride()) if n > 1), key=lambda p: p[1]):
+        if st != want:
+            return False
+        want *= n
+    return True
+
+
+def grad_mode(out, full=True, peek=False, store=False):
+    arena = _Touched.arena
+    if arena is None or out.dtype != arena.dtype or out.device != arena.device:
+        return True
+    es = arena.element_size()
+    off = out.data_ptr() - arena.data_ptr()
+    if off < 0 or off >= arena.numel() * es or out.numel() == 0:
+        return True
+    lo = off // es
+    reach = 1 + sum((n - 1) * st for n, st in zip(out.shape, out.stride()))
+    hi = lo + reach
+    gaps = _span_gaps(lo, hi)
+    if store and not peek and full and _dense(out):
+        _span_mark(lo, hi)
+        return False
+    if full and _dense(out) and gaps == [(lo, hi)]:
+        if not peek:
+            _span_mark(lo, hi)
+        return False
+    if peek:
+        return True
+    if gaps:
+        _zero_ranges(arena, gaps)
+        _Touched.demand.extend(gaps)
+        _span_mark(lo, hi)
+    return True
+
+
+def grad_end():
+    arena = _Touched.arena
+    if arena is None:
+        return [], []
+    _Touched.unused = _span_gaps(0, arena.numel())
+    if _Touched.unused:
+        _zero_ranges(arena, _Touched.unused)
+    _Touched.arena = None
+    return list(_Touched.demand), list(_Touched.unused)
+
+
+def grad_abort():
+    _Touched.arena = None
+
+
+K.grad_mode = grad_mode
 
 
 class _Fold:
@@ -1568,13 +1688,19 @@
 class CrossEntropyFn(torch.autograd.Function):
 
     @staticmethod
-    def forward(ctx, logits, target, ignore_index, seed=None):
+    def forward(ctx, logits, target, ignore_index, seed=None, stats=None):
         V = logits.shape[-1]
         l2d = _ce_rows(logits)
         t = target.reshape(-1).contiguous()
         ctx.ignore_index, ctx.shape = ignore_index, logits.shape
         ctx.seeded = _SeededGrad()
         if ctx.needs_input_grad[0] and _SeededGrad.usable(seed, l2d.device) and K.cross_entropy_fwd_grad_ok(l2d, V):
+            if stats is not None and t.dtype == torch.int64 and t.numel() >= 1:
+                lse, row_loss, d, loss = K.cross_entropy_fwd_grad(l2d, t, seed, V, ignore_index, stats.stats, stats.ticket)
+                stats.done = True
+                ctx.seeded = _SeededGrad(seed, d)
+                ctx.save_for_backward(l2d, t, lse)
+                return loss
             lse, row_loss, d = K.cross_entropy_fwd_grad(l2d, t, seed, V, ignore_index)
             ctx.seeded = _SeededGrad(seed, d)
         else:
@@ -1590,11 +1716,19 @@
         if d is None:
             gs = dloss.reshape(1).float().contiguous()
             d = K.cross_entropy_bwd(l2d, t, lse, gs, V, ctx.ignore_index, dlogits=ctx.seeded.spare())
-        return d[:, :V].view(ctx.shape), None, None, None
-
-
-def cross_entropy_sum(logits, target, ignore_index, seed=None):
-    return CrossEntropyFn.apply(logits, target, ignore_index, seed)
+        return d[:, :V].view(ctx.shape), None, None, None, None
+
+
+class StepStats:
+
+    def __init__(self, stats, ticket):
+        self.stats, self.ticket, self.done = stats, ticket, False
+
+
+def cross_entropy_sum(logits, target, ignore_index, seed=None, stats=None):
+    if stats is not None:
+        stats.done = False
+    return CrossEntropyFn.apply(logits, target, ignore_index, seed, stats)
 
 
 class LabelSmoothedCrossEntropyFn(torch.autograd.Function):
diff --git a/ofasys_amd/trainer.py b/ofasys_amd/trainer.py
--- a/ofasys_amd/trainer.py
+++ b/ofasys_amd/trainer.py
@@ -70,6 +70,10 @@
                 p.data = self._view(self.flat, o, p)
                 p.grad = self._view(self.grad, o, p)
                 p._ofa_grad = p.grad
+                old = getattr(p, "_ofa_grad_hook", None)
+                if old is not None:
+                    old.remove()
+                p._ofa_grad_hook = p.register_hook(lambda g, v=p._ofa_grad: None if g is None else (ops.grad_mode(v, False) and None))
         off_of = {id(p): o for p, o in zip(params, self.offsets)}
         for m in mhas:
             n = 3 if m.self_attention else 2
@@ -108,6 +112,9 @@
 
     def zero_grad(self):
         self.grad.zero_()
+        self.repoint()
+
+    def repoint(self):
         for p, o in zip(self.params, self.offsets):
             if p.grad is None or p.grad.data_ptr() != self.grad.data_ptr() + o * self.grad.element_size():
                 p.grad = self._view(self.grad, o, p)
@@ -235,6 +242,11 @@
             self.loss_scale_cfg = cfg
             self._ls = torch.tensor([cfg["init_scale"], 0, -1, -1, 0, 0, 0, 0], dtype=torch.float64, device=dev)
         self._graphs = {}
+        self._gsq_cleared = False
+        self._rng_pending = None
+        self._tail_ticket = torch.zeros(2, dtype=torch.int32, device=dev)
+        self._ce_stats = ops.StepStats(self._stats, self._tail_ticket[1:2])
+        self._prezero = {}
         self.max_graphs = int(max_graphs)
         self._pool = None
         self._warned_cap = False
@@ -257,11 +269,40 @@
         model = self.model
         model.train()
         ops.drop_pending()
-        self.fp.zero_grad()
-        self._stats.zero_()
+        if self._rng_pending:
+            self._rng_pending[0].add_(self._rng_pending[1])
+            self._rng_pending = None
+        first_touch = self.world == 1 and not K.tail_old(K.TAIL_FIRST_TOUCH)
+        if first_touch:
+            self.fp.repoint()
+            ops.grad_begin(self.fp.grad, self._prezero.get(structure, ()), also=(self._stats, self._gsq))
+            self._gsq_cleared = True
+        else:
+            ops.grad_abort()
+            self.fp.zero_grad()
+            self._stats.zero_()
         self.reducer.overlap = overlap_reduce
         ops.defer_reductions(self.world == 1 or not overlap_reduce)
         self.reducer.begin_step(structure, dynamic=self.dynamic_autograd or self.sync_collectives)
+        try:
+            self._micro_batches(samples)
+            ops.flush_folds()
+        except BaseException:
+            ops.grad_abort()
+            raise
+        if first_touch:
+            demand, _ = ops.grad_end()
+            if demand:
+                if len(self._prezero) >= 256 and structure not in self._prezero:
+                    self._prezero.clear()
+                self._prezero[structure] = sorted(set(self._prezero.get(structure, ())) | set(demand))
+        self._rng_pending = ops.rng_defer() if self._fused_norm() else ops.rng_advance()
+
+    def _fused_norm(self):
+        return self.world == 1 and not K.tail_old(K.TAIL_NORM_SCHEDULE)
+
+    def _micro_batches(self, samples):
+        model = self.model
         for s in samples:
             plan = s.get("pack")
             target = s["target"]
@@ -299,9 +340,13 @@
             else:
                 if self.loss_scale_cfg is None and (self._seed is None or self._seed.device != logits.device):
                     self._seed = torch.ones((), dtype=torch.float32, device=logits.device)
-                loss = ops.cross_entropy_sum(logits, target, self.pad, seed=self._seed if self.loss_scale_cfg is None else None)
+                fused = self._ce_stats if (logits.is_cuda and not K.tail_old(K.TAIL_CRITERION_STATS)) else None
+                loss = ops.cross_entropy_sum(logits, target, self.pad, seed=self._seed if self.loss_scale_cfg is None else None,
+                                             stats=fused)
                 n = None
-                if loss.is_cuda and loss.dtype == torch.float32 and target.is_contiguous() and target.dtype == torch.int64:
+                if fused is not None and fused.done:
+                    counted = True
+                elif loss.is_cuda and loss.dtype == torch.float32 and target.is_contiguous() and target.dtype == torch.int64:
                     K.step_stats_add(self._stats, loss.detach(), target, self.pad)
                     counted = True
                 else:
@@ -316,16 +361,31 @@
                 self._stats[0] += n if size is None else size
                 self._stats[1] += loss.detach().double()
                 self._stats[2] += n
-        ops.flush_folds()
-        ops.rng_advance()
 
     def _reduce(self):
         self.reducer.finish()
         all_reduce_scalars(self._stats, self.group)
 
     def _update(self):
-        self._gsq.zero_()
         owned = self.reducer.owned_ranges()
+        pending, self._rng_pending = self._rng_pending, None
+        if self._fused_norm() and len(owned) == 1 and owned[0][2] and owned[0][1] > owned[0][0]:
+            lo, hi, _ = owned[0]
+            c = self.loss_scale_cfg or {}
+            K.sumsq_schedule(self.fp.grad[lo:hi], self._gsq, self._tail_ticket[0:1], self._stats, self._step_t, self._lr_t, self._sched,
+                             self._gnorm_t, self.clip_norm, self.betas[0], self.betas[1],
+                             loss_scaler=self._ls if self.loss_scale_cfg is not None else None,
+                             scale_factor=c.get("scale_factor", 2.0), scale_window=c.get("scale_window", 2000),
+                             tolerance=c.get("tolerance", 0.0), threshold=c.get("threshold"), min_loss_scale=c.get("min_loss_scale", 1e-4),
+                             counter=pending[0] if pending else None, counter_add=pending[1] if pending else 0)
+            self._gsq_cleared = False
+            self._finish_update(owned)
+            return
+        if pending:
+            pending[0].add_(pending[1])
+        if not self._gsq_cleared:
+            self._gsq.zero_()
+        self._gsq_cleared = False
         for lo, hi, counted in owned:
             if counted:
                 K.sumsq(self.fp.grad[lo:hi], self._gsq)
@@ -340,6 +400,9 @@
             K.step_schedule_scaled(self._gsq, self._stats, self._step_t, self._lr_t, self._sched, self._gnorm_t, self._ls,
                                    self.clip_norm, self.betas[0], self.betas[1], c["scale_factor"], c["scale_window"],
                                    c["tolerance"], c["threshold"], c["min_loss_scale"])
+        self._finish_update(owned)
+
+    def _finish_update(self, owned):
         for lo, hi, _ in owned:
             K.adam_step(self.master[lo:hi], self.exp_avg[lo:hi], self.exp_avg_sq[lo:hi], self.fp.grad[lo:hi], self.fp.flat[lo:hi],
                         self._sched, 0.0, self.betas[0], self.betas[1], self.eps, self.weight_decay, 0)
```

Measured after the change: 1.433 million (median of 6 runs). 1.01x the previous value.
